# mojing1999/jmcodec

Measured on AMD Instinct MI355X. Metric: decoded frames/sec @1080p H.264 + bit-exact YUV, higher is better.
Workload: dtype u8

## Files before the change

### jmcodec_amd/csrc/deblock_device.h

```cpp
#pragma once
#include <hip/hip_runtime.h>
#include "jobs.h"
#include "kernels.h"
#include "kernel_common.h"
#include "chain_common.h"
#include "deblock_packed.h"

namespace jmamd {

struct DbRec {
    uint8_t y_bs[32];
    uint8_t y_ab[3][2];
    uint8_t y_pad[10];
    uint8_t c_bs[2][16];
    uint8_t c_ab[2][3][2];
    uint8_t c_pad[4];
};
static_assert(sizeof(DbRec) == 96, "DbRec must be 96 bytes");

__device__ __forceinline__ uint32_t perm(uint32_t hi, uint32_t lo, uint32_t sel) { return __builtin_amdgcn_perm(hi, lo, sel); }

struct Lds {
    uint8_t *base; int mb_h; int hdr;
    static constexpr int kRecStride = 80, kLT = 528, kLR = 272, kCT = 272, kCR = 144;
    __device__ uint8_t *rec(int group) const { return base + group * kRecStride; }
    __device__ uint8_t *luma_tile(int row, int par) const { return base + hdr + (size_t)row * kLT + par * 256; }
    __device__ uint8_t *luma_ring(int row, int slot) const { return base + hdr + (size_t)mb_h * kLT + (size_t)row * kLR + slot * 64; }
    __device__ uint8_t *chroma_tile(int row, int par) const { return base + hdr + (size_t)row * kCT + par * 128; }
    __device__ uint8_t *chroma_ring(int row, int slot) const { return base + hdr + (size_t)mb_h * kCT + (size_t)row * kCR + slot * 32; }
};

typedef __attribute__((address_space(1))) uint8_t gbyte;
struct DbCtx { gbyte *plane; int pitch, mb_w, mb_h; };
typedef uint32_t v4u __attribute__((ext_vector_type(4)));
typedef uint32_t v2u __attribute__((ext_vector_type(2)));
#define JM_GLOBAL __attribute__((address_space(1)))
template <typename T> __device__ __forceinline__ T gload(const gbyte *p);
template <> __device__ __forceinline__ uint4 gload<uint4>(const gbyte *p) { v4u v = *(const JM_GLOBAL v4u *)p; return make_uint4(v.x, v.y, v.z, v.w); }
template <> __device__ __forceinline__ uint32_t gload<uint32_t>(const gbyte *p) { return *(const JM_GLOBAL uint32_t *)p; }
__device__ __forceinline__ void gstore(gbyte *p, uint4 v) { v4u t = {v.x, v.y, v.z, v.w}; *(JM_GLOBAL v4u *)p = t; }
__device__ __forceinline__ void gstore(gbyte *p, uint2 v) { v2u t = {v.x, v.y}; *(JM_GLOBAL v2u *)p = t; }
__device__ __forceinline__ void gstore(gbyte *p, uint32_t v) { *(JM_GLOBAL uint32_t *)p = v; }
__device__ __forceinline__ void gstore_wt(gbyte *p, uint32_t v) { __hip_atomic_store((JM_GLOBAL uint32_t *)p, v, __ATOMIC_RELAXED, __HIP_MEMORY_SCOPE_AGENT); }
template <bool WT> __device__ __forceinline__ void fstore(gbyte *p, uint4 v) { if (WT) st_wt16((void *)p, v); else gstore(p, v); }
template <bool WT> __device__ __forceinline__ void fstore(gbyte *p, uint2 v) { if (WT) st_wt8((void *)p, v); else gstore(p, v); }
template <bool WT> __device__ __forceinline__ void fstore(gbyte *p, uint32_t v) { if (WT) gstore_wt(p, v); else gstore(p, v); }

template <bool WT, int PHASE = 0>
__device__ __forceinline__ void luma_mb(const DbCtx &pp, const Lds &lds, int x, int row, int lrow, int l, int group, uint4 own, uint32_t recdw) {
    uint8_t *tc = lds.luma_tile(lrow, x & 1), *tp = lds.luma_tile(lrow, (x - 1) & 1);
    uint8_t *ring_up = row > 0 ? lds.luma_ring(lrow - 1, x & 3) : nullptr;
    uint8_t *ring_up_l = row > 0 ? lds.luma_ring(lrow - 1, (x - 1) & 3) : nullptr;
    uint8_t *ring_dn = lds.luma_ring(lrow, x & 3), *ring_dn_l = lds.luma_ring(lrow, (x - 1) & 3);
    uint8_t *rec = lds.rec(group);
    if (PHASE != 2 && l < 12) ((uint32_t *)rec)[l] = recdw;
    int vb[4], hb[4], ab[6];
#pragma unroll
    for (int e = 0; e < 4; e++) { if (PHASE != 2) vb[e] = rec[e * 4 + (l >> 2)]; if (PHASE != 1) hb[e] = rec[16 + e * 4 + (l >> 2)]; }
#pragma unroll
    for (int i = 0; i < 6; i++) ab[i] = rec[32 + i];
    if (PHASE != 2) {
    uint32_t left = x > 0 ? *(const uint32_t *)(tp + l * 16 + 12) : 0;
    uint32_t left_after, row_after[4];
    {
        const uint32_t w[5] = {left, own.x, own.y, own.z, own.w};
        s2 A = as_s2(perm(w[1], w[0], 0x0c040c03)), B = as_s2(perm(w[1], w[0], 0x0c050c02)), C = as_s2(perm(w[1], w[0], 0x0c060c01)),
            D = as_s2(perm(w[1], w[0], 0x0c070c00));
#pragma unroll
        for (int e = 0; e < 4; e++) {
            if (e) {
                const s2 pA = A, pB = B, pC = C, pD = D;
                A = as_s2(perm(w[e + 1], as_u(pD), 0x0c040c02)); B = as_s2(perm(w[e + 1], as_u(pC), 0x0c050c02));
                C = as_s2(perm(w[e + 1], as_u(pB), 0x0c060c02)); D = as_s2(perm(w[e + 1], as_u(pA), 0x0c070c02));
            }
            const int c = e ? 1 : 0;
            flt_luma(A, B, C, D, vb[e], ab[2 * c], ab[2 * c + 1]);
            const uint32_t o = perm(as_u(C), as_u(D), 0x0c0c0400) | perm(as_u(A), as_u(B), 0x04000c0c);
            if (e == 0) left_after = o; else row_after[e - 1] = o;
        }
        row_after[3] = perm(as_u(B), as_u(A), 0x0c0c0602) | perm(as_u(D), as_u(C), 0x06020c0c);
    }
    if (x > 0) *(uint32_t *)(tp + l * 16 + 12) = left_after;
    *(uint4 *)(tc + l * 16) = make_uint4(row_after[0], row_after[1], row_after[2], row_after[3]);
    if (x > 0 && l >= 12) *(uint32_t *)(ring_dn_l + (l - 12) * 16 + 12) = left_after;
    }
    if (PHASE == 1) return;
    {
        uint32_t c[20];
        c[0] = c[1] = c[2] = c[3] = 0;
        if (ring_up) { c[0] = ring_up[l]; c[1] = ring_up[16 + l]; c[2] = ring_up[32 + l]; c[3] = ring_up[48 + l]; }
#pragma unroll
        for (int j = 0; j < 16; j++) c[4 + j] = tc[j * 16 + l];
        s2 A = as_s2(c[3] | (c[4] << 16)), B = as_s2(c[2] | (c[5] << 16)), C = as_s2(c[1] | (c[6] << 16)), D = as_s2(c[0] | (c[7] << 16));
#pragma unroll
        for (int e = 0; e < 4; e++) {
            if (e) {
                const s2 pA = A, pB = B, pC = C, pD = D;
                A = as_s2(perm(c[4 * e + 4], as_u(pD), 0x0c040c02)); B = as_s2(perm(c[4 * e + 5], as_u(pC), 0x0c040c02));
                C = as_s2(perm(c[4 * e + 6], as_u(pB), 0x0c040c02)); D = as_s2(perm(c[4 * e + 7], as_u(pA), 0x0c040c02));
            }
            const int k = e ? 1 : 2;
            flt_luma(A, B, C, D, hb[e], ab[2 * k], ab[2 * k + 1]);
            if (e == 0) { if (ring_up) { ring_up[1 * 16 + l] = (uint8_t)as_u(C); ring_up[2 * 16 + l] = (uint8_t)as_u(B);
                ring_up[3 * 16 + l] = (uint8_t)as_u(A); } }
            else { const int r = 4 * e - 4; tc[r * 16 + l] = (uint8_t)as_u(D); tc[(r + 1) * 16 + l] = (uint8_t)as_u(C);
                tc[(r + 2) * 16 + l] = (uint8_t)as_u(B); tc[(r + 3) * 16 + l] = (uint8_t)as_u(A); }
        }
        const uint8_t r12 = (uint8_t)(as_u(A) >> 16), r13 = (uint8_t)(as_u(B) >> 16), r14 = (uint8_t)(as_u(C) >> 16), r15 = (uint8_t)(as_u(D) >> 16);
        tc[12 * 16 + l] = r12; tc[13 * 16 + l] = r13; tc[14 * 16 + l] = r14; tc[15 * 16 + l] = r15;
        ring_dn[0 * 16 + l] = r12; ring_dn[1 * 16 + l] = r13; ring_dn[2 * 16 + l] = r14; ring_dn[3 * 16 + l] = r15;
    }
    gbyte *dst = pp.plane;
    int x0 = x * 16, y0 = row * 16, pitch = pp.pitch;
    bool right = x == pp.mb_w - 1, bottom = row == pp.mb_h - 1;
    {
        int R = l - 4;
        const uint8_t *src, *srcl;
        if (R < 0) { src = ring_up ? ring_up + (R + 4) * 16 : nullptr; srcl = ring_up_l ? ring_up_l + (R + 4) * 16 + 12 : nullptr; }
        else { src = tc + R * 16; srcl = tp + R * 16 + 12; }
        if (src) {
            gbyte *d = dst + (size_t)(y0 + R) * pitch + x0;
            uint4 v = *(const uint4 *)src;
            if (x > 0) { uint32_t lf = *(const uint32_t *)srcl; fstore<WT>(d - 4, make_uint4(lf, v.x, v.y, v.z)); }
            else { fstore<WT>(d, make_uint2(v.x, v.y)); fstore<WT>(d + 8, v.z); }
            if (right) fstore<WT>(d + 12, v.w);
        }
    }
    if (bottom && l < 4) {
        int R = 12 + l;
        gbyte *d = dst + (size_t)(y0 + R) * pitch + x0;
        uint4 v = *(const uint4 *)(tc + R * 16);
        if (x > 0) { uint32_t lf = *(const uint32_t *)(tp + R * 16 + 12); fstore<WT>(d - 4, make_uint4(lf, v.x, v.y, v.z)); }
        else { fstore<WT>(d, make_uint2(v.x, v.y)); fstore<WT>(d + 8, v.z); }
        if (right) fstore<WT>(d + 12, v.w);
    }
}

template <bool WT, int PHASE = 0>
__device__ __forceinline__ void chroma_mb(const DbCtx &pp, const Lds &lds, int x, int row, int lrow, int l, int group, uint4 own, uint32_t recdw) {
    uint8_t *tc = lds.chroma_tile(lrow, x & 1), *tp = lds.chroma_tile(lrow, (x - 1) & 1);
    uint8_t *ring_up = row > 0 ? lds.chroma_ring(lrow - 1, x & 3) : nullptr;
    uint8_t *ring_up_l = row > 0 ? lds.chroma_ring(lrow - 1, (x - 1) & 3) : nullptr;
    uint8_t *ring_dn = lds.chroma_ring(lrow, x & 3), *ring_dn_l = lds.chroma_ring(lrow, (x - 1) & 3);
    uint8_t *rec = lds.rec(group);
    if (PHASE != 2 && l < 12) ((uint32_t *)rec)[l] = recdw;
    if (PHASE != 2) {
        const int plane = l >> 3, r = l & 7;
        const uint32_t left = x > 0 ? *(const uint32_t *)(tp + r * 16 + 12) : 0;
        if (plane == 0) *(uint4 *)(tc + r * 16) = own;
        const int s0 = plane * 8, s1 = s0 + 16;
        const int vb[2] = { rec[plane * 16 + (r >> 1)], rec[plane * 16 + 4 + (r >> 1)] };
        const int ab[4] = { rec[32 + plane * 6], rec[32 + plane * 6 + 1], rec[32 + plane * 6 + 2], rec[32 + plane * 6 + 3] };
        {
            int p0 = (int)(left >> s1) & 255, q0 = (int)(own.x >> s0) & 255;
            flt_chroma((int)(left >> s0) & 255, p0, q0, (int)(own.x >> s1) & 255, vb[0], ab[0], ab[1]);
            if (vb[0] & 7) { tp[r * 16 + 14 + plane] = (uint8_t)p0; tc[r * 16 + plane] = (uint8_t)q0; }
        }
        {
            int p0 = (int)(own.y >> s1) & 255, q0 = (int)(own.z >> s0) & 255;
            flt_chroma((int)(own.y >> s0) & 255, p0, q0, (int)(own.z >> s1) & 255, vb[1], ab[2], ab[3]);
            if (vb[1] & 7) { tc[r * 16 + 6 + plane] = (uint8_t)p0; tc[r * 16 + 8 + plane] = (uint8_t)q0; }
        }
    }
    if (PHASE != 2 && x > 0 && l < 2) *(uint32_t *)(ring_dn_l + l * 16 + 12) = *(const uint32_t *)(tp + (6 + l) * 16 + 12);
    if (PHASE == 1) return;
    {
        int plane = l & 1;
        int hb[2] = { rec[plane * 16 + 8 + (l >> 2)], rec[plane * 16 + 12 + (l >> 2)] };
        int ab[4] = { rec[32 + plane * 6 + 4], rec[32 + plane * 6 + 5], rec[32 + plane * 6 + 2], rec[32 + plane * 6 + 3] };
        int c[10];
        c[0] = ring_up ? ring_up[l] : 0; c[1] = ring_up ? ring_up[16 + l] : 0;
#pragma unroll
        for (int j = 0; j < 8; j++) c[2 + j] = tc[j * 16 + l];
#pragma unroll
        for (int e = 0; e < 4; e += 2) {
            const int k = e ? 1 : 0;
            const int o = 2 * e;
            flt_chroma(c[o], c[o + 1], c[o + 2], c[o + 3], hb[e >> 1], ab[2 * k], ab[2 * k + 1]);
        }
        if (ring_up) ring_up[16 + l] = (uint8_t)c[1];
        tc[l] = (uint8_t)c[2]; tc[3 * 16 + l] = (uint8_t)c[5]; tc[4 * 16 + l] = (uint8_t)c[6];
        ring_dn[l] = (uint8_t)c[8]; ring_dn[16 + l] = (uint8_t)c[9];
    }
    gbyte *dst = pp.plane;
    int x0 = x * 16, y0 = row * 8, pitch = pp.pitch;
    bool right = x == pp.mb_w - 1, bottom = row == pp.mb_h - 1;
    if (l < 8) {
        int R = l - 2;
        const uint8_t *src, *srcl;
        if (R < 0) { src = ring_up ? ring_up + (R + 2) * 16 : nullptr; srcl = ring_up_l ? ring_up_l + (R + 2) * 16 + 12 : nullptr; }
        else { src = tc + R * 16; srcl = tp + R * 16 + 12; }
        if (src) {
            gbyte *d = dst + (size_t)(y0 + R) * pitch + x0;
            uint4 v = *(const uint4 *)src;
            if (x > 0) { uint32_t lf = *(const uint32_t *)srcl; fstore<WT>(d - 4, make_uint4(lf, v.x, v.y, v.z)); }
            else { fstore<WT>(d, make_uint2(v.x, v.y)); fstore<WT>(d + 8, v.z); }
            if (right) fstore<WT>(d + 12, v.w);
        }
    } else if (bottom && l < 10) {
        int R = 6 + (l - 8);
        gbyte *d = dst + (size_t)(y0 + R) * pitch + x0;
        uint4 v = *(const uint4 *)(tc + R * 16);
        if (x > 0) { uint32_t lf = *(const uint32_t *)(tp + R * 16 + 12); fstore<WT>(d - 4, make_uint4(lf, v.x, v.y, v.z)); }
        else { fstore<WT>(d, make_uint2(v.x, v.y)); fstore<WT>(d + 8, v.z); }
        if (right) fstore<WT>(d + 12, v.w);
    }
}

constexpr int kBandRows = 16;
constexpr int kDeblockSmemMain = kBandRows * Lds::kRecStride + (kBandRows + 1) * (Lds::kLT + Lds::kLR);
constexpr int kStageBytes = 1024 + 256 + 256, kDeblockMaxDepth = 4;
constexpr int kDeblockSmemBytes = kDeblockSmemMain + (kBandRows / 4) * kDeblockMaxDepth * kStageBytes;

__device__ __forceinline__ uint32_t lds_addr_of(const void *p) { return (uint32_t)(uintptr_t)(__attribute__((address_space(3))) const uint8_t *)p; }
template <bool COHERENT> __device__ __forceinline__ void glds16(const gbyte *g, uint32_t lds_byte_addr) {
    unsigned keep;
    if (COHERENT)
        asm volatile("s_mov_b32 %0, m0\n\ts_mov_b32 m0, %2\n\ts_nop 0\n\tglobal_load_lds_dwordx4 %1, off sc1\n\ts_mov_b32 m0, %0"
                     : "=&s"(keep) : "v"(g), "s"(lds_byte_addr) : "memory");
    else asm volatile("s_mov_b32 %0, m0\n\ts_mov_b32 m0, %2\n\ts_nop 0\n\tglobal_load_lds_dwordx4 %1, off\n\ts_mov_b32 m0, %0" : "=&s"(keep) : "v"(g),
        "s"(lds_byte_addr) : "memory");
}
template <bool COHERENT> __device__ __forceinline__ void glds4(const gbyte *g, uint32_t lds_byte_addr) {
    unsigned keep;
    if (COHERENT)
        asm volatile("s_mov_b32 %0, m0\n\ts_mov_b32 m0, %2\n\ts_nop 0\n\tglobal_load_lds_dword %1, off sc1\n\ts_mov_b32 m0, %0"
                     : "=&s"(keep) : "v"(g), "s"(lds_byte_addr) : "memory");
    else asm volatile("s_mov_b32 %0, m0\n\ts_mov_b32 m0, %2\n\ts_nop 0\n\tglobal_load_lds_dword %1, off\n\ts_mov_b32 m0, %0" : "=&s"(keep) : "v"(g),
        "s"(lds_byte_addr) : "memory");
}
template <int DEPTH, bool CHAIN, bool AFTER_INTRA = false>
__device__ __forceinline__ void deblock_band_body(const PicParams &pp, int band, bool is_chroma, int *prog_pic, int pub, uint8_t *smem, int *cpic,
    int *err_word) {
    const int mb_w = pp.mb_w, mb_h = pp.mb_h, pitch = pp.pitch;
    const int row0 = band * kBandRows;
    if (row0 >= mb_h) return;
    const int rows = min(kBandRows, mb_h - row0);
    int *prog = prog_pic + (is_chroma ? kDeblockMaxBands : 0);
    const gbyte *recs = (const gbyte *)pp.dbrec;
    Lds lds{smem, kBandRows + 1, kBandRows * Lds::kRecStride};
    const int group = threadIdx.x >> 4, l = threadIdx.x & 15;
    const int lrow = group + 1;
    const bool active = group < rows;
    const int row = row0 + (active ? group : 0);
    gbyte *plane = (gbyte *)(cur_plane(pp) + (is_chroma ? pp.chroma_offset : 0));
    const DbCtx cx{plane, pitch, mb_w, mb_h};
    const int rows_per_mb = is_chroma ? 8 : 16, ring_rows = is_chroma ? 2 : 4;
    const int my_row = is_chroma ? (l & 7) : l;
    const int rec_dw = (is_chroma ? 12 : 0) + (l < 12 ? l : 0);
    const bool takes_ring = band > 0 && group == 0;
    const bool gives_ring = active && group == rows - 1 && row < mb_h - 1;
    const int s_begin = kRowLag * row0, s_end = mb_w - 1 + kRowLag * (row0 + rows - 1) + (kRowLag == 1 ? 1 : 0);
    int known = 0;
    int *abort_word = CHAIN ? cpic - (size_t)pp.chain_idx * kChainStride + (size_t)kChainMaxPics * kChainStride : nullptr;
    auto wait_above = [&](int need) {
        if (band == 0 || threadIdx.x >= 64) return;
        if (known >= need) return;
        int spins = 0; WaitClock t0;
        while ((known = __hip_atomic_load(&prog[band - 1], __ATOMIC_RELAXED, __HIP_MEMORY_SCOPE_AGENT)) < need && ++spins < kSpinLimit &&
               !(CHAIN && (wait_expired(spins, t0, abort_word) || ((spins & 255) == 0 && ld_coh(abort_word))))) __builtin_amdgcn_s_sleep(8);
        if (CHAIN && l == 0) note_gaps(t0, err_word ? err_word - pp.chain_idx + kChainMaxPics : nullptr);
        if (known < need) {
            if (l == 0) { report_wait_timeout(err_word, CHAIN_ERR_RING_TIMEOUT);
                if (CHAIN) {
                    if (!ld_coh(abort_word)) { record_first_giveup(abort_word, CHAIN_ERR_RING_TIMEOUT, pp.chain_idx, band << 16 | (is_chroma ? 1 : 0), need,
                        known, 0);
                        record_giveup_evidence(abort_word, &prog[band - 1], spins, t0); }
                    st_coh(abort_word, 1);
                } }
            known = 0x7fffffff;
        }
        asm volatile("" ::: "memory");
    };
    int recon_known = (pp.stages & PS_RECON) ? 0x7fffffff : 0;
    const uint32_t *bits_row = CHAIN ? (const uint32_t *)(cpic + kChainBits) + (size_t)row * kChainRowWords : nullptr;
    constexpr bool after_intra = CHAIN && AFTER_INTRA;
    int ifin_known0 = 0, ifin_known1 = 0;
    const int *ifin0 = after_intra ? cpic + kChainIntraFin + (is_chroma ? 32 : 0) + (row >> 4) : nullptr;
    const int *ifin1 = after_intra ? cpic + kChainIntraFin + (is_chroma ? 32 : 0) + (min(row + 1, mb_h - 1) >> 4) : nullptr;
    auto wait_recon = [&](int x) {
        if (!CHAIN) return;
        const bool want = active && x >= 0 && x < mb_w;
        bool ok;
        const int tag = pp.chain_idx << 16 | (row & 0xffff);
        if (after_intra) { const int need = x + 2 * row + 4; ok = wait_counter(ifin0, ifin_known0, want, need, abort_word, tag) &&
            wait_counter(ifin1, ifin_known1, want, need, abort_word, tag); }
        else ok = wait_row_bit(bits_row, recon_known, want, x, abort_word, tag, err_word ? err_word - pp.chain_idx + kChainMaxPics : nullptr);
        if (!ok && (threadIdx.x & 63) == 0) { report_wait_timeout(err_word, after_intra ? CHAIN_ERR_IFIN_TIMEOUT : CHAIN_ERR_BITS_TIMEOUT);
            st_coh(abort_word, 1); }
    };
    const int ring_lanes = ring_rows * 4;
    const int ring_lane = l < ring_lanes ? l : 0;
    const gbyte *pix_base = plane + (size_t)(row * rows_per_mb + my_row) * pitch;
    const gbyte *rec_base = recs + (size_t)row * mb_w * sizeof(DbRec) + rec_dw * 4;
    const gbyte *ring_base = plane + (size_t)(takes_ring ? row * rows_per_mb - ring_rows + (ring_lane >> 2) : 0) * pitch + (ring_lane & 3) * 4;
    const int wave = __builtin_amdgcn_readfirstlane((int)(threadIdx.x >> 6)), wl = (int)(threadIdx.x & 63);
    uint8_t *stage = smem + kDeblockSmemMain + wave * (kDeblockMaxDepth * kStageBytes);
    const uint32_t stage_lds = lds_addr_of(stage);
    auto fetch = [&](int d, int s) {
        int xn = min(max(s - kRowLag * row, 0), mb_w - 1);
        if (CHAIN) wait_recon(s - kRowLag * row);
        const uint32_t slot = stage_lds + (uint32_t)d * kStageBytes;
        glds16<CHAIN>(pix_base + xn * 16, slot);
        glds4<false>(rec_base + (size_t)xn * sizeof(DbRec), slot + 1024);
        glds4<true>(band > 0 ? ring_base + xn * 16 : rec_base, slot + 1280);
    };
    auto give = [&](const uint8_t *ring, int xm, int lane0) {
        int k = l - lane0;
        if (k < 0 || k >= ring_lanes) return;
        uint32_t v = *(const uint32_t *)(ring + (k >> 2) * 16 + (k & 3) * 4);
        __hip_atomic_store((JM_GLOBAL uint32_t *)(plane + (size_t)((row + 1) * rows_per_mb - ring_rows + (k >> 2)) * pitch + xm * 16) + (k & 3), v,
            __ATOMIC_RELAXED, __HIP_MEMORY_SCOPE_AGENT);
    };
    auto step = [&](int s, uint4 own, uint32_t rdw, uint32_t ring) {
        if (kRowLag == 1) {
            const int xv = s - row, xh = xv - 1;
            if (active && xh >= 0 && xh < mb_w) {
                if (is_chroma) { chroma_mb<CHAIN, 2>(cx, lds, xh, row, lrow, l, group, own, rdw);
                    if (gives_ring && xh == mb_w - 1) give(lds.chroma_ring(lrow, xh & 3), xh, 8); }
                else { luma_mb<CHAIN, 2>(cx, lds, xh, row, lrow, l, group, own, rdw);
                    if (gives_ring && xh == mb_w - 1) give(lds.luma_ring(lrow, xh & 3), xh, 0); }
            }
            if (active && xv >= 0 && xv < mb_w) {
                if (is_chroma) {
                    if (takes_ring && l < ring_lanes) *(uint32_t *)(lds.chroma_ring(0, xv & 3) + (l >> 2) * 16 + (l & 3) * 4) = ring;
                    chroma_mb<CHAIN, 1>(cx, lds, xv, row, lrow, l, group, own, rdw);
                    if (gives_ring && xv > 0) give(lds.chroma_ring(lrow, (xv - 1) & 3), xv - 1, 0);
                } else {
                    if (takes_ring) *(uint32_t *)(lds.luma_ring(0, xv & 3) + (l >> 2) * 16 + (l & 3) * 4) = ring;
                    luma_mb<CHAIN, 1>(cx, lds, xv, row, lrow, l, group, own, rdw);
                    if (gives_ring && xv > 0) give(lds.luma_ring(lrow, (xv - 1) & 3), xv - 1, 0);
                }
            }
        } else {
            const int x = s - kRowLag * row;
            if (active && x >= 0 && x < mb_w) {
                if (is_chroma) {
                    if (takes_ring && l < ring_lanes) *(uint32_t *)(lds.chroma_ring(0, x & 3) + (l >> 2) * 16 + (l & 3) * 4) = ring;
                    chroma_mb<CHAIN, 0>(cx, lds, x, row, lrow, l, group, own, rdw);
                    if (gives_ring) {
                        if (x > 0) give(lds.chroma_ring(lrow, (x - 1) & 3), x - 1, 0);
                        if (x == mb_w - 1) give(lds.chroma_ring(lrow, x & 3), x, 8);
                    }
                } else {
                    if (takes_ring) *(uint32_t *)(lds.luma_ring(0, x & 3) + (l >> 2) * 16 + (l & 3) * 4) = ring;
                    luma_mb<CHAIN, 0>(cx, lds, x, row, lrow, l, group, own, rdw);
                    if (gives_ring) {
                        if (x > 0) give(lds.luma_ring(lrow, (x - 1) & 3), x - 1, 0);
                        if (x == mb_w - 1) give(lds.luma_ring(lrow, x & 3), x, 0);
                    }
                }
            }
        }
        constexpr int kPubLag = 3;
        if (gives_ring && pub > 0 && s - kPubLag >= s_begin && ((s - kPubLag + 1 - s_begin) % pub == 0)) {
            asm volatile("s_waitcnt vmcnt(%0)" :: "n"(3 * kPubLag) : "memory");
            if (l == 0) __hip_atomic_store(&prog[band], s - kPubLag + 1, __ATOMIC_RELAXED, __HIP_MEMORY_SCOPE_AGENT);
        }
        if (gives_ring && pub > 0 && s == s_end) {
            asm volatile("s_waitcnt vmcnt(0)" ::: "memory");
            if (l == 0) __hip_atomic_store(&prog[band], 0x7fffffff, __ATOMIC_RELAXED, __HIP_MEMORY_SCOPE_AGENT);
        }
        if (CHAIN) {
            asm volatile("s_waitcnt vmcnt(6) lgkmcnt(0)\n\ts_barrier" ::: "memory");
            if (threadIdx.x == 0 && s - 1 > s_begin) __hip_atomic_store(cpic + kChainFin + (is_chroma ? 32 : 0) + band, s - 1, __ATOMIC_RELAXED,
                __HIP_MEMORY_SCOPE_AGENT);
        } else
            asm volatile("s_waitcnt lgkmcnt(0)\n\ts_barrier" ::: "memory");
    };
    static_assert(DEPTH >= 2 && DEPTH <= kDeblockMaxDepth, "prefetch depth");
    constexpr int kAbove = 2 - kRowLag;
    wait_above(s_begin + DEPTH + kAbove);
#pragma unroll
    for (int d = 0; d < DEPTH; d++) fetch(d, s_begin + d);
    for (int s = s_begin; s <= s_end; s += DEPTH) {
#pragma unroll
        for (int j = 0; j < DEPTH; j++) {
            if (s + j > s_end) break;
            asm volatile("s_waitcnt vmcnt(%0)" :: "n"(3 * (DEPTH - 1)) : "memory");
            const uint8_t *sl = stage + j * kStageBytes;
            const uint4 own = *(const uint4 *)(sl + wl * 16);
            const uint32_t rdw = *(const uint32_t *)(sl + 1024 + wl * 4), ring = *(const uint32_t *)(sl + 1280 + wl * 4);
            asm volatile("s_waitcnt lgkmcnt(0)" ::: "memory");
            wait_above(s + j + DEPTH + kAbove);
            fetch(j, s + j + DEPTH);
            step(s + j, own, rdw, ring);
        }
    }
    if (CHAIN) {
        asm volatile("s_waitcnt vmcnt(0)\n\ts_barrier" ::: "memory");
        if (threadIdx.x == 0) __hip_atomic_store(cpic + kChainFin + (is_chroma ? 32 : 0) + band, 0x7fffffff, __ATOMIC_RELAXED, __HIP_MEMORY_SCOPE_AGENT);
    }
}

}
```

### jmcodec_amd/csrc/deblock_lds.hip

```cpp
#include <hip/hip_runtime.h>
#include <cstdlib>
#include <algorithm>
#include "jobs.h"
#include "kernels.h"
#include "kernel_common.h"
#include "deblock_device.h"

namespace jmamd {

__global__ __launch_bounds__(256) void k_deblock_prep(const PicParams *pics) {
    const PicParams &pp = pics[blockIdx.y];
    if (!(pp.stages & (PS_DEBLOCK_LDS | PS_CHAIN))) return;
    DbRec *out = (DbRec *)pp.dbrec;
    const int per_xcd = ((int)gridDim.x + 7) >> 3;
    const int blk = ((int)blockIdx.x & 7) * per_xcd + ((int)blockIdx.x >> 3);
    __shared__ __align__(16) uint8_t stage[8][96];
    int sub = threadIdx.x >> 5, t = threadIdx.x & 31;
    int mb = blk * 8 + sub;
    int n_mbs = pp.mb_w * pp.mb_h;
    if (mb >= n_mbs) return;
    int mbx = mb % pp.mb_w, mby = mb / pp.mb_w;
    const MbW q = load_mbw(&pp.mbs[mb]);
    const SliceRec sl = pp.slices[mbw_slice(q)];
    bool has_left = mbx > 0, has_top = mby > 0;
    MbW pl = q, pt = q;
    if (has_left) { pl = load_mbw(&pp.mbs[mb - 1]); if (sl.disable == 2 && mbw_slice(pl) != mbw_slice(q)) has_left = false; }
    if (has_top) { pt = load_mbw(&pp.mbs[mb - pp.mb_w]); if (sl.disable == 2 && mbw_slice(pt) != mbw_slice(q)) has_top = false; }
    int dir = t >> 4, e = (t >> 2) & 3, k = t & 3;
    int rq = dir == 0 ? k * 4 + e : e * 4 + k;
    int bs;
    if (sl.disable == 1) bs = 0;
    else if (e == 0) {
        bool have = dir == 0 ? has_left : has_top;
        const MbW pn = select_mbw(dir == 0, pl, pt);
        bs = have ? boundary_strength(pp, pn, dir == 0 ? k * 4 + 3 : 12 + k, q, rq, true, dir == 1) : 0;
    } else bs = boundary_strength(pp, q, dir == 0 ? rq - 1 : rq - 4, q, rq, false, dir == 1);
    if ((e & 1) && (mbw_modes(q) & MBM_T8X8)) bs = 0;
    int cls = e ? 1 : (dir ? 2 : 0);
    int qp_p = cls == 0 ? mbw_qp(pl) : (cls == 2 ? mbw_qp(pt) : mbw_qp(q)), qp_q = mbw_qp(q);
    DbRec *o = (DbRec *)stage[sub];
    {
        int qpav = (qp_p + qp_q + 1) >> 1;
        int ia = clip3(0, 51, qpav + sl.alpha_off), ib = clip3(0, 51, qpav + sl.beta_off);
        int tc0 = (bs >= 1 && bs <= 3) ? kTc0[ia][bs - 1] : 0;
        o->y_bs[t] = (uint8_t)(bs | (tc0 << 3));
        if (k == 0 && (e == 0 || (e == 1 && dir == 0))) { o->y_ab[cls][0] = kAlpha[ia]; o->y_ab[cls][1] = kBeta[ib]; }
    }
    if (!(e & 1)) {
#pragma unroll
        for (int plane = 0; plane < 2; plane++) {
            int off = plane ? pp.cr_qp_off : pp.cb_qp_off;
            int qpav = (chroma_qp(qp_p, off) + chroma_qp(qp_q, off) + 1) >> 1;
            int ia = clip3(0, 51, qpav + sl.alpha_off), ib = clip3(0, 51, qpav + sl.beta_off);
            int tc0 = (bs >= 1 && bs <= 3) ? kTc0[ia][bs - 1] : 0;
            o->c_bs[plane][dir * 8 + (e >> 1) * 4 + k] = (uint8_t)(bs | (tc0 << 3));
            if (k == 0 && (e == 0 || (e == 2 && dir == 0))) { o->c_ab[plane][cls][0] = kAlpha[ia]; o->c_ab[plane][cls][1] = kBeta[ib]; }
        }
    }
    if (t < 6) ((uint4 *)&out[mb])[t] = ((const uint4 *)stage[sub])[t];
}

template <int DEPTH>
__global__ __launch_bounds__(kBandRows * 16) void k_deblock_band(const PicParams *pics, int *ctl, int pub, int *err) {
    __shared__ __align__(16) uint8_t smem[kDeblockSmemBytes];
    const PicParams &pp = pics[blockIdx.y];
    if (!(pp.stages & PS_DEBLOCK_LDS)) return;
    deblock_band_body<DEPTH, false>(pp, blockIdx.x >> 1, blockIdx.x & 1, ctl + (size_t)blockIdx.y * kChainStride + kChainRing, pub, smem, nullptr,
        err + blockIdx.y);
}

bool deblock_lds_supported(int mb_w, int mb_h) { return mb_w > 0 && mb_h <= kBandRows * kDeblockMaxBands; }

constexpr int kDeblockDepth = 2, kDeblockPub = 2;
int deblock_depth() { return kDeblockDepth; }
int deblock_row_lag() { return kRowLag; }
int deblock_pub() { return kDeblockPub; }

void launch_deblock_prep(const PicParams *d_pics, int n, int max_mbs, hipStream_t st) {
    hipLaunchKernelGGL(k_deblock_prep, dim3(((max_mbs + 7) / 8 + 7) & ~7, n), dim3(256), 0, st, d_pics);
}
void launch_deblock_lds(const PicParams *d_pics, int n, int max_mb_h, int *ctl, int *err, bool debug_stall, hipStream_t st) {
    const int depth = deblock_depth(), pub = debug_stall ? -1 : deblock_pub();
    const int bands = (max_mb_h + kBandRows - 1) / kBandRows;
    dim3 grid(2 * bands, n), block(kBandRows * 16);
    if (depth <= 2) hipLaunchKernelGGL((k_deblock_band<2>), grid, block, 0, st, d_pics, ctl, pub, err);
    else if (depth == 3) hipLaunchKernelGGL((k_deblock_band<3>), grid, block, 0, st, d_pics, ctl, pub, err);
    else hipLaunchKernelGGL((k_deblock_band<4>), grid, block, 0, st, d_pics, ctl, pub, err);
}

}
```

### jmcodec_amd/csrc/deblock_packed.h

```cpp
#pragma once
#include <stdint.h>
#if defined(__HIPCC__)
#include <hip/hip_runtime.h>
#include "kernel_common.h"
#define JM_DB_HD __host__ __device__ __forceinline__
#else
#define JM_DB_HD static inline
#endif

namespace jmamd {

#if !defined(__HIPCC__)
JM_DB_HD int clip3(int lo, int hi, int v) { return v < lo ? lo : (v > hi ? hi : v); }
JM_DB_HD int clip1(int v) { return v < 0 ? 0 : (v > 255 ? 255 : v); }
JM_DB_HD int iabs(int v) { return v < 0 ? -v : v; }
#endif

#if defined(__HIPCC__)
typedef short s2 __attribute__((ext_vector_type(2)));
JM_DB_HD s2 pmin(s2 a, s2 b) { return __builtin_elementwise_min(a, b); }
JM_DB_HD s2 pmax(s2 a, s2 b) { return __builtin_elementwise_max(a, b); }
JM_DB_HD s2 as_s2(uint32_t v) { return __builtin_bit_cast(s2, v); }
JM_DB_HD uint32_t as_u(s2 v) { return __builtin_bit_cast(uint32_t, v); }
#else
struct s2 { int16_t x, y; };
JM_DB_HD s2 mk_s2(int x, int y) { return s2{(int16_t)(uint16_t)(x & 0xffff), (int16_t)(uint16_t)(y & 0xffff)}; }
JM_DB_HD s2 operator+(s2 a, s2 b) { return mk_s2(a.x + b.x, a.y + b.y); }
JM_DB_HD s2 operator-(s2 a, s2 b) { return mk_s2(a.x - b.x, a.y - b.y); }
JM_DB_HD s2 operator-(s2 a) { return mk_s2(-a.x, -a.y); }
JM_DB_HD s2 operator<<(s2 a, int n) { return mk_s2((int)((uint32_t)(uint16_t)a.x << n), (int)((uint32_t)(uint16_t)a.y << n)); }
JM_DB_HD s2 operator>>(s2 a, int n) { return mk_s2(a.x >> n, a.y >> n); }
JM_DB_HD s2 pmin(s2 a, s2 b) { return s2{a.x < b.x ? a.x : b.x, a.y < b.y ? a.y : b.y}; }
JM_DB_HD s2 pmax(s2 a, s2 b) { return s2{a.x > b.x ? a.x : b.x, a.y > b.y ? a.y : b.y}; }
JM_DB_HD s2 as_s2(uint32_t v) { return mk_s2((int)(v & 0xffffu), (int)(v >> 16)); }
JM_DB_HD uint32_t as_u(s2 v) { return (uint32_t)(uint16_t)v.x | ((uint32_t)(uint16_t)v.y << 16); }
#endif
#if defined(__HIP_DEVICE_COMPILE__)
JM_DB_HD uint32_t sad_u8(uint32_t a, uint32_t b, uint32_t c) { return __builtin_amdgcn_sad_u8(a, b, c); }
JM_DB_HD uint32_t alignbit(uint32_t hi, uint32_t lo, uint32_t sh) { return __builtin_amdgcn_alignbit(hi, lo, sh); }
JM_DB_HD bool any_lane(bool c) { return __builtin_amdgcn_ballot_w64(c) != 0; }
#else
JM_DB_HD uint32_t sad_u8(uint32_t a, uint32_t b, uint32_t c) {
    for (int k = 0; k < 4; k++) { const int x = (int)((a >> (8 * k)) & 255), y = (int)((b >> (8 * k)) & 255); c += (uint32_t)(x < y ? y - x : x - y); }
    return c;
}
JM_DB_HD uint32_t alignbit(uint32_t hi, uint32_t lo, uint32_t sh) { return (uint32_t)((((uint64_t)hi << 32) | lo) >> (sh & 31)); }
JM_DB_HD bool any_lane(bool c) { return c; }
#endif

JM_DB_HD int adiff(int a, int b) { return (int)sad_u8((unsigned)a, (unsigned)b, 0u); }
JM_DB_HD int sel(bool c, int a, int b) { return c ? a : b; }
JM_DB_HD s2 splat(int v) { return as_s2((uint32_t)v | ((uint32_t)v << 16)); }
JM_DB_HD s2 swp(s2 v) { const uint32_t u = as_u(v); return as_s2(alignbit(u, u, 16)); }
JM_DB_HD s2 pabs(s2 v) { return pmax(v, -v); }
JM_DB_HD s2 blend(uint32_t m, s2 a, s2 b) { return as_s2((as_u(a) & m) | (as_u(b) & ~m)); }
JM_DB_HD void flt_luma(s2 &A, s2 &B, s2 &C, const s2 D, int bsw, int alpha, int beta) {
    const int bS = bsw & 7, tc0 = bsw >> 3;
    const s2 As = swp(A), Bs = swp(B);
    const s2 beta2 = splat(beta);
    const s2 d10 = pabs(B - A), dpq = pabs(As - A);
    const s2 m10 = (d10 - beta2) >> 15, mpq = (dpq - splat(alpha)) >> 15;
    const uint32_t on = as_u(m10) & as_u(swp(m10)) & as_u(mpq) & (bS ? 0xffffffffu : 0u);
    if (!any_lane(on != 0)) return;
    const s2 m20 = (pabs(C - A) - beta2) >> 15;
    const int tc = tc0 + (int)(as_u(m20) & 1u) + (int)(as_u(m20) >> 31);
    const s2 t = ((As - A) << 2) + (B - Bs) + splat(4);
    const int dl = clip3(-tc, tc, (int)(short)(as_u(t) & 0xffffu) >> 3);
    const s2 dd = as_s2(((uint32_t)dl & 0xffffu) | ((uint32_t)(-dl) << 16));
    const s2 nA = pmin(pmax(A + dd, splat(0)), splat(255));
    const s2 avg = as_s2((as_u(A + As + splat(1)) >> 1) & 0x7fff7fffu);
    const s2 tcs = splat(tc0);
    const s2 tt = pmin(pmax((C + avg - (B << 1)) >> 1, -tcs), tcs);
    const s2 nB = B + as_s2(as_u(tt) & as_u(m20));
    const uint32_t nrm = on & (bS < 4 ? 0xffffffffu : 0u);
    s2 rA = blend(nrm, nA, A), rB = blend(nrm, nB, B), rC = C;
    const uint32_t st = on & (bS >= 4 ? 0xffffffffu : 0u);
    if (any_lane(st != 0)) {
        const s2 msg = (dpq - splat((alpha >> 2) + 2)) >> 15;
        const uint32_t sm = st & as_u(m20) & as_u(msg);
        const s2 S0 = (C + ((B + A + As) << 1) + Bs + splat(4)) >> 3;
        const s2 S1 = (C + B + A + As + splat(2)) >> 2;
        const s2 S2 = ((D << 1) + C + (C << 1) + B + A + As + splat(4)) >> 3;
        const s2 W0 = ((B << 1) + A + Bs + splat(2)) >> 2;
        rA = blend(sm, S0, blend(st, W0, rA)); rB = blend(sm, S1, rB); rC = blend(sm, S2, rC);
    }
    A = rA; B = rB; C = rC;
}
JM_DB_HD void flt_chroma(int p1, int &p0, int &q0, int q1, int bsw, int alpha, int beta) {
    const int bS = bsw & 7, tc = (bsw >> 3) + 1;
    const bool on = ((int)(bS != 0) & (int)(adiff(p0, q0) < alpha) & (int)(adiff(p1, p0) < beta) & (int)(adiff(q1, q0) < beta)) != 0;
    const int delta = clip3(-tc, tc, (((q0 - p0) << 2) + (p1 - q1) + 4) >> 3);
    const int n_p0 = clip1(p0 + delta), n_q0 = clip1(q0 - delta), w_p0 = (2 * p1 + p0 + q1 + 2) >> 2, w_q0 = (2 * q1 + q0 + p1 + 2) >> 2;
    p0 = sel(on, sel(bS < 4, n_p0, w_p0), p0); q0 = sel(on, sel(bS < 4, n_q0, w_q0), q0);
}

JM_DB_HD void filter_luma(int *s, int bS, int alpha, int beta, const uint8_t *tc0_row) {
    int p3 = s[0], p2 = s[1], p1 = s[2], p0 = s[3], q0 = s[4], q1 = s[5], q2 = s[6], q3 = s[7];
    if (!(iabs(p0 - q0) < alpha && iabs(p1 - p0) < beta && iabs(q1 - q0) < beta)) return;
    int ap = iabs(p2 - p0) < beta, aq = iabs(q2 - q0) < beta;
    if (bS < 4) {
        int tc0 = tc0_row[bS - 1], tc = tc0 + ap + aq;
        int delta = clip3(-tc, tc, (((q0 - p0) << 2) + (p1 - q1) + 4) >> 3);
        s[3] = clip1(p0 + delta); s[4] = clip1(q0 - delta);
        if (ap) s[2] = p1 + clip3(-tc0, tc0, (p2 + ((p0 + q0 + 1) >> 1) - (p1 << 1)) >> 1);
        if (aq) s[5] = q1 + clip3(-tc0, tc0, (q2 + ((p0 + q0 + 1) >> 1) - (q1 << 1)) >> 1);
    } else {
        bool strong = iabs(p0 - q0) < ((alpha >> 2) + 2);
        if (ap && strong) { s[3] = (p2 + 2 * p1 + 2 * p0 + 2 * q0 + q1 + 4) >> 3; s[2] = (p2 + p1 + p0 + q0 + 2) >> 2;
            s[1] = (2 * p3 + 3 * p2 + p1 + p0 + q0 + 4) >> 3; }
        else s[3] = (2 * p1 + p0 + q1 + 2) >> 2;
        if (aq && strong) { s[4] = (p1 + 2 * p0 + 2 * q0 + 2 * q1 + q2 + 4) >> 3; s[5] = (p0 + q0 + q1 + q2 + 2) >> 2;
            s[6] = (2 * q3 + 3 * q2 + q1 + q0 + p0 + 4) >> 3; }
        else s[4] = (2 * q1 + q0 + p1 + 2) >> 2;
    }
}
JM_DB_HD void filter_chroma(int *s, int bS, int alpha, int beta, const uint8_t *tc0_row) {
    int p1 = s[0], p0 = s[1], q0 = s[2], q1 = s[3];
    if (!(iabs(p0 - q0) < alpha && iabs(p1 - p0) < beta && iabs(q1 - q0) < beta)) return;
    if (bS < 4) {
        int tc = tc0_row[bS - 1] + 1;
        int delta = clip3(-tc, tc, (((q0 - p0) << 2) + (p1 - q1) + 4) >> 3);
        s[1] = clip1(p0 + delta); s[2] = clip1(q0 - delta);
    } else { s[1] = (2 * p1 + p0 + q1 + 2) >> 2; s[2] = (2 * q1 + q0 + p1 + 2) >> 2; }
}

}
```

### jmcodec_amd/csrc/engine.cpp

```cpp
#include "engine.h"
#include <sys/prctl.h>
#include "chain_order.h"
#include "decoder.h"
#include "kernels.h"
#include "hevc_kernels.h"
#include "numa.h"
#include <hip/hip_runtime_api.h>
#include <pthread.h>
#include <algorithm>
#include <chrono>
#include <cstdio>
#include <cstring>
#include <cstdlib>

namespace jmamd {

static long g_lane_trace = getenv("JM_AMD_DEC_LANE_TRACE") ? atol(getenv("JM_AMD_DEC_LANE_TRACE")) : 0;
static double trace_ms() { static const auto t0 = std::chrono::steady_clock::now();
    return std::chrono::duration<double, std::milli>(std::chrono::steady_clock::now() - t0).count(); }
#define LANE_TRACE(...) do { if (g_lane_trace > 0) { g_lane_trace--; fprintf(stderr, "lane-trace %9.3f " , trace_ms()); fprintf(stderr, __VA_ARGS__); } } while (0)

static std::mutex g_engines_m;
static Engine *g_engines[64] = {nullptr};

Engine *Engine::get(int device) {
    std::lock_guard<std::mutex> lk(g_engines_m);
    if (device < 0 || device >= 64) return nullptr;
    if (!g_engines[device]) {
        Engine *e = new Engine(device);
        if (!e->ok_) return nullptr;
        g_engines[device] = e;
    }
    return g_engines[device];
}

void mem_trace(const char *tag) {
    static const bool on = getenv("JM_AMD_DEC_MEMTRACE") != nullptr;
    if (!on) return;
    long pages = 0, res = 0;
    if (FILE *f = fopen("/proc/self/statm", "r")) { if (fscanf(f, "%ld %ld", &pages, &res) != 2) res = 0; fclose(f); }
    fprintf(stderr, "jm_amd_dec: memtrace %-44s %8.1f MB resident\n", tag, res * 4096.0 / 1e6);
}

Engine::Engine(int device) : device_(device) {
    (void)trace_ms();
    mem_trace("engine: start");
    if (const char *e = getenv("JM_AMD_DEC_CHAIN_DEPTH")) { chain_depth_ = std::max(1, std::min(atoi(e), 16)); chain_depth_few_ = chain_depth_.load(); }
    if (const char *e = getenv("JM_AMD_DEC_CHAIN_STREAMS")) chain_max_streams_ = std::max(0, atoi(e));
    if (const char *e = getenv("JM_AMD_DEC_CHAIN_LAG")) chain_lag_steps_ = std::max(kMinChainLag, std::min(atoi(e), 1024));
    if (const char *e = getenv("JM_AMD_DEC_CHAIN_LINGER")) chain_linger_streams_ = std::max(0, atoi(e));
    if (const char *e = getenv("JM_AMD_DEC_CROSS_LANE")) cross_lane_ = atoi(e) != 0;
    if (const char *e = getenv("JM_AMD_DEC_FILL_LINGER_US")) fill_linger_ns_ = std::max(0, atoi(e)) * 1000ll;
    if (const char *e = getenv("JM_AMD_DEC_EARLY_INTRA")) early_intra_ = atoi(e) != 0;
    if (hipSetDevice(device_) != hipSuccess) return;
    if (const char *e = getenv("JM_AMD_DEC_COPY_STREAMS")) n_copy_ = std::max(1, std::min(atoi(e), 4));
    int prio_lo = 0, prio_hi = 0, copy_prio = 0;
    hipDeviceGetStreamPriorityRange(&prio_lo, &prio_hi);
    { const char *e = getenv("JM_AMD_DEC_COPY_PRIORITY"); const int want = e ? atoi(e) : 1;
      copy_prio = want > 0 ? prio_hi : (want < 0 ? prio_lo : 0); }
    for (int k = 0; k < n_copy_; k++) if (hipStreamCreateWithPriority(&copy_streams_[k], hipStreamNonBlocking, copy_prio) != hipSuccess) {
        (void)hipGetLastError();
        if (hipStreamCreateWithFlags(&copy_streams_[k], hipStreamNonBlocking) != hipSuccess) return; }
    mem_trace("engine: copy stream");
    for (auto &ln : lanes_) {
        hipStream_t s, p, q;
        if (hipStreamCreateWithFlags(&s, hipStreamNonBlocking) != hipSuccess || hipStreamCreateWithFlags(&p, hipStreamNonBlocking) != hipSuccess ||
            hipStreamCreateWithFlags(&q, hipStreamNonBlocking) != hipSuccess) return;
        ln.stream = s; ln.pack_stream = p; ln.pre_stream = q;
        mem_trace("engine: lane streams");
        for (auto &b : ln.ring) {
            if (hipHostMalloc((void **)&b.h_pics, sizeof(PicParams) * kMaxBatch, hipHostMallocDefault) != hipSuccess) return;
            if (hipMalloc((void **)&b.d_pics, sizeof(PicParams) * kMaxBatch) != hipSuccess) return;
            if (hipHostMalloc((void **)&b.h_hpics, sizeof(HevcPicParams) * kMaxBatch, hipHostMallocDefault) != hipSuccess) return;
            if (hipMalloc((void **)&b.d_hpics, sizeof(HevcPicParams) * kMaxBatch) != hipSuccess) return;
            if (hipMalloc((void **)&b.d_progress, sizeof(int) * kMaxBatch * kHevcProgressStride) != hipSuccess) return;
            if (hipMalloc((void **)&b.d_ctl, sizeof(int) * ((size_t)kMaxBatch * chain_ctl_ints() + chain_tail_ints())) != hipSuccess) return;
            if (hipHostMalloc((void **)&b.h_err, sizeof(int) * (kMaxBatch + 4), hipHostMallocMapped) != hipSuccess) return;
            if (hipHostGetDevicePointer((void **)&b.d_err, b.h_err, 0) != hipSuccess) return;
            memset(b.h_err, 0, sizeof(int) * (kMaxBatch + 4));
            if (hipHostMalloc((void **)&b.h_groups, sizeof(uint32_t) * kMaxChainGroups, hipHostMallocDefault) != hipSuccess) return;
            if (hipMalloc((void **)&b.d_groups, sizeof(uint32_t) * kMaxChainGroups) != hipSuccess) return;
            bool tables_ok = true;
            b.out.each([&](auto &t) { const size_t bytes = sizeof(*t.host) * 2 * kOutSideCap;
                tables_ok = tables_ok && hipHostMalloc((void **)&t.host, bytes, hipHostMallocDefault) == hipSuccess &&
                            hipMalloc((void **)&t.dev, bytes) == hipSuccess; });
            if (!tables_ok) return;
            if (hipEventCreateWithFlags(&b.done, hipEventDisableTiming) != hipSuccess) return;
            if (hipEventCreateWithFlags(&b.kdone, hipEventDisableTiming) != hipSuccess) return;
            if (hipEventCreateWithFlags(&b.packed, hipEventDisableTiming) != hipSuccess) return;
            if (hipEventCreateWithFlags(&b.pre_done, hipEventDisableTiming) != hipSuccess) return;
            for (auto &e : b.pev) if (hipEventCreate(&e) != hipSuccess) return;
        }
    }
    mem_trace("engine: lane buffers");
    { const int r = chain_resident_workgroups(false), ri = chain_resident_workgroups(true);
      if (r > 0) chain_bands_max_ = std::min(kMaxChainBands, r / 2);
      if (ri > 0) chain_bands_max_intra_ = std::min(kMaxChainBandsIntra, ri / 2);
      if (getenv("JM_AMD_DEC_VERBOSE")) fprintf(stderr,
          "jm_amd_dec: device %d holds %d / %d chain workgroups (plain / with the intra role): band budget %d / %d\n", device_, r, ri, chain_bands_max_,
          chain_bands_max_intra_); }
    mem_trace("engine: occupancy queries");
    ok_ = true;
    numa_node_ = numa_node_of_device(device_, true);
    kfd_gpu_id_ = getenv("JM_AMD_DEC_IGNORE_SHARED_GPU") ? 0 : kfd_gpu_id_of_device(device_);
    th_ = std::thread([this] { pthread_setname_np(pthread_self(), "jm-engine"); numa_bind_this_thread(numa_node_); run(); });
    th_.detach();
}

unsigned long long Engine::upload(uint8_t *dev, const uint8_t *host, size_t n, ihipEvent_t *ev, bool spread) {
    std::lock_guard<std::mutex> lk(um_);
    hipSetDevice(device_);
    unsigned long long seq = ++upload_seq_;
    if (!spread) while (seq % (unsigned)n_copy_) seq = ++upload_seq_;
    hipStream_t cs = copy_streams_[seq % (unsigned)n_copy_];
    hipMemcpyAsync(dev, host, n, hipMemcpyHostToDevice, cs);
    hipEventRecord(ev, cs);
    return seq;
}

void Engine::submit(EnginePic &&p) {
    {
        std::lock_guard<std::mutex> lk(m_);
        if (p.codec == 0) {
            const long long now = std::chrono::duration_cast<std::chrono::nanoseconds>(std::chrono::steady_clock::now().time_since_epoch()).count();
            auto it = std::find_if(recent_.begin(), recent_.end(), [&](const Recent &r) { return r.dec == p.dec; });
            if (it == recent_.end()) { recent_.push_back(Recent{p.dec, now, 0}); it = recent_.end() - 1; }
            it->t = now;
            if (p.has_picture) it->mbs = p.mb_w * p.mb_h;
        }
        p.seq = p.dec->engine_state().next_seq++;
        if (p.dec->engine_state().n_pending++ == 0) decoders_pending_++;
        pending_.push_back(std::move(p));
        pending_gen_++;
    }
    cv_.notify_one();
}

bool Engine::set_knob(const std::string &key, long long v) {
    if (key.rfind("chain_", 0) == 0) { chain_block_until_ns_ = 0; shared_checked_ns_ = 0; }
    if (key == "chain_depth") { if (v <= 0) { chain_depth_ = 8; chain_depth_few_ = 16; }
        else { chain_depth_ = (int)std::min(v, 16ll); chain_depth_few_ = chain_depth_.load(); } }
    else if (key == "chain_lag") chain_lag_steps_ = (int)std::max((long long)kMinChainLag, std::min(v, 1024ll));
    else if (key == "chain_streams") chain_max_streams_ = (int)std::max(0ll, v);
    else if (key == "debug_stall") debug_stall_ = (int)v;
    else if (key == "debug_no_bi") debug_no_bi_ = (int)v;
    else if (key == "early_intra_ahead") early_intra_ahead_ = (int)std::max(1ll, std::min(v, 64ll));
    else return false;
    return true;
}

EngineStats Engine::stats() { std::lock_guard<std::mutex> lk(sm_); return st_; }

bool Engine::others_done(Decoder *d, int lane_idx, unsigned long long seq) {
    for (int li = 0; li < kLanes; li++) {
        if (li == lane_idx) continue;
        Lane &o = lanes_[li];
        for (int k = 0; k < o.inflight; k++) {
            Batch &ob = o.ring[(o.tail + k) % kBatchRing];
            bool mine = false;
            for (auto &p : ob.pics) if (p.dec == d && p.seq < seq) { mine = true; break; }
            if (mine && hipEventQuery(ob.packed) != hipSuccess) { (void)hipGetLastError(); return false; }
        }
    }
    return true;
}

void Engine::inflight_masks(Decoder *d, uint32_t &touched) {
    touched = 0;
    for (auto &o : lanes_) for (int k = 0; k < o.inflight; k++) for (auto &p : o.ring[(o.tail + k) % kBatchRing].pics) if (p.dec == d) {
        touched |= p.ref_mask | p.out_mask;
        if (p.has_picture) touched |= 1u << (p.codec == 0 ? p.pp.cur : p.hp.cur);
    }
}

bool Engine::form(Lane &ln, int lane_idx, Batch &b) {
    b.pics.clear(); b.any_chain = false; b.chain_with_intra = false; b.max_depth = 1;
    bool chaining = false;
    int depth_now = chain_depth_;
    {
        const long long now = std::chrono::duration_cast<std::chrono::nanoseconds>(std::chrono::steady_clock::now().time_since_epoch()).count();
        recent_.erase(std::remove_if(recent_.begin(), recent_.end(), [&](const Recent &r) { return now - r.t > 50ll * 1000 * 1000; }), recent_.end());
        const int n_active = (int)recent_.size();
        double load = 0;
        for (const Recent &r : recent_) load += std::max(1.0, r.mbs / 8160.0);
        chaining = chain_depth_ > 1 && n_active > 0 && load <= (double)chain_max_streams_ && now >= chain_block_until_ns_ &&
            !gpu_shared_.load(std::memory_order_relaxed);
        depth_now = n_active <= chain_linger_streams_ ? std::max(chain_depth_.load(), chain_depth_few_.load()) : chain_depth_.load();
        if (lane_idx == kOrdinaryLane && chaining && n_active <= chain_linger_streams_ && ln.inflight > 0) {
            int n = 0;
            for (const EnginePic &p : pending_) if (p.codec == 0 && p.has_picture && p.lane(true) == lane_idx) n++;
            if (n < depth_now * n_active) return false;
        }
    }
    if (lane_idx == kOrdinaryLane && !chaining && fill_linger_ns_ > 0 && (int)recent_.size() > decoders_pending_) {
        const long long now = std::chrono::duration_cast<std::chrono::nanoseconds>(std::chrono::steady_clock::now().time_since_epoch()).count();
        if (!ln.wait_since_ns) ln.wait_since_ns = now;
        if (now - ln.wait_since_ns < fill_linger_ns_) {
            bool urgent = false; size_t n_seen = 0; const size_t n_dec = (size_t)decoders_pending_;
            scan_tag_form_++;
            for (auto it = pending_.begin(); it != pending_.end() && n_seen < n_dec && !urgent; ++it) {
                EngineDecoderState &es = it->dec->engine_state();
                if (es.form_tag == scan_tag_form_) continue;
                es.form_tag = scan_tag_form_; n_seen++;
                if (it->lane(false) != lane_idx || es.inflight > es.lane_inflight[lane_idx]) continue;
                urgent = it->dec->frames_done_unfetched() < 1;
            }
            if (!urgent) { lingered_ = true; return false; }
        }
    }
    if (lane_idx == kOrdinaryLane) ln.wait_since_ns = 0;
    if (lane_idx == kIntraLane && !chaining && !deep_queues_ && fill_linger_ns_ > 0) {
        const long long now = std::chrono::duration_cast<std::chrono::nanoseconds>(std::chrono::steady_clock::now().time_since_epoch()).count();
        if (!ln.wait_since_ns || now - ln.wait_since_ns < fill_linger_ns_) {
            bool urgent = false; int n_elig = 0; size_t n_seen = 0; const size_t n_dec = (size_t)decoders_pending_;
            scan_tag_form_++;
            for (auto it = pending_.begin(); it != pending_.end() && n_seen < n_dec && !urgent && n_elig < 4; ++it) {
                EngineDecoderState &es = it->dec->engine_state();
                if (es.form_tag == scan_tag_form_) continue;
                es.form_tag = scan_tag_form_; n_seen++;
                if (it->codec != 0 || it->lane(false) != lane_idx) continue;
                if (es.inflight > es.lane_inflight[lane_idx] && !(cross_lane_ && others_done(it->dec, lane_idx, it->seq))) continue;
                n_elig++;
                urgent = it->dec->frames_done_unfetched() < 1;
            }
            if (n_elig == 0) return false;
            if (!ln.wait_since_ns) ln.wait_since_ns = now;
            if (n_elig < 4 && !urgent && now - ln.wait_since_ns < fill_linger_ns_) { lingered_ = true; return false; }
        }
        ln.wait_since_ns = 0;
    }
    std::vector<Decoder *> seen, members;
    const bool relaxed = cross_lane_ && !chaining;
    const long long now_ns = std::chrono::duration_cast<std::chrono::nanoseconds>(std::chrono::steady_clock::now().time_since_epoch()).count();
    size_t n_pre = 0, n_post = 0;
    auto account = [&](EnginePic &p, EngineDecoderState &es) {
        if (p.has_picture) es.batch_written |= 1u << (p.codec == 0 ? p.pp.cur : p.hp.cur);
        es.batch_read |= p.ref_mask | p.out_mask;
        n_pre += p.out[kBefore].frames(); n_post += p.out[kAfter].frames();
    };
    const size_t n_dec_pending = (size_t)decoders_pending_;
    auto took = [&](EngineDecoderState &es) { if (--es.n_pending == 0) decoders_pending_--; };
    for (auto it = pending_.begin(); it != pending_.end() && (int)b.pics.size() < kMaxBatch && seen.size() < n_dec_pending;) {
        Decoder *d = it->dec;
        if (std::find(seen.begin(), seen.end(), d) != seen.end()) { ++it; continue; }
        seen.push_back(d);
        EngineDecoderState &es = d->engine_state();
        int why = 0;
        if (it->lane(chaining) != lane_idx) why = 1;
        else if (es.inflight > es.lane_inflight[lane_idx] && !(relaxed && others_done(d, lane_idx, it->seq))) why = 2;
        else if (n_pre + it->out[kBefore].frames() > (size_t)kOutSideCap || n_post + it->out[kAfter].frames() > (size_t)kOutSideCap) why = 3;
        if (why) {
            if (lane_idx == kOrdinaryLane && it->codec == 0) { std::lock_guard<std::mutex> lk(sm_);
                (why == 1 ? st_.rej_other_lane : why == 2 ? st_.rej_cross_lane : st_.rej_tables)++;
                if (!es.blocked_since) { es.blocked_since = now_ns;
                    if (g_lane_trace > 0) {
                        LANE_TRACE("left-out dec %p seq %llu why %d inflight %d (lane0 %d lane1 %d)\n", (void *)d, it->seq, why, es.inflight, es.lane_inflight[0],
                            es.lane_inflight[1]);
                        for (int li = 0; li < kLanes; li++) for (int k = 0; k < lanes_[li].inflight; k++) { Batch &ob = lanes_[li].ring[(lanes_[li].tail + k) % kBatchRing];
                            for (auto &p : ob.pics) if (p.dec == d) LANE_TRACE("    in flight: lane %d batch %llu seq %llu kdone %d packed %d done %d\n", li, ob.serial, p.seq,
                                (int)hipEventQuery(ob.kdone), (int)hipEventQuery(ob.packed), (int)hipEventQuery(ob.done)); }
                        (void)hipGetLastError();
                    } } }
            ++it; continue;
        }
        if (lane_idx == kOrdinaryLane && es.blocked_since) { std::lock_guard<std::mutex> lk(sm_); st_.blocked_ns += now_ns - es.blocked_since; st_.blocked_n++;
            LANE_TRACE("rejoined dec %p seq %llu after %.3f ms\n", (void *)d, it->seq, (now_ns - es.blocked_since) * 1e-6);
            es.blocked_since = 0; }
        es.inflight++; es.lane_inflight[lane_idx]++;
        es.in_batch = 1; es.batch_written = es.batch_read = 0; es.batch_stop = false;
        account(*it, es);
        members.push_back(d);
        took(es);
        b.pics.push_back(std::move(*it));
        it = pending_.erase(it);
    }
    if (lane_idx == kIntraLane && early_intra_ && deep_queues_ && !chaining && early_scanned_gen_ != pending_gen_ && now_ns - early_scan_ns_ > 250 * 1000) {
        early_scan_ns_ = now_ns;
        const unsigned long long tag = ++early_scan_tag_;
        std::vector<std::deque<EnginePic>::iterator> cand;
        for (auto it = pending_.begin(); it != pending_.end(); ++it) {
            Decoder *d = it->dec;
            EngineDecoderState &es = d->engine_state();
            if (es.scan_tag != tag) { es.scan_tag = tag; es.scan_touched = 0; es.scan_ahead = 0;
                es.scan_closed = std::find(members.begin(), members.end(), d) != members.end(); }
            const uint32_t own = it->has_picture ? 1u << (it->codec == 0 ? it->pp.cur : it->hp.cur) : 0u;
            if (!es.scan_closed && it->codec == 0 && it->has_picture && it->lane(false) == kIntraLane && it->ref_mask == 0 && it->before_empty() &&
                !it->wait_prev_pack && !(it->out_mask & ~own)) {
                es.scan_closed = true;
                uint32_t infl; inflight_masks(d, infl);
                const bool landed = !it->uploaded || hipEventQuery(it->uploaded) == hipSuccess;
                if (!landed) (void)hipGetLastError();
                if (landed && es.scan_ahead >= early_intra_ahead_.load() && !(own & (es.scan_touched | infl))) cand.push_back(it);
            }
            es.scan_touched |= it->ref_mask | it->out_mask | own;
            es.scan_ahead++;
        }
        if (!cand.empty()) {
            std::vector<size_t> pos;
            for (auto &c : cand) pos.push_back((size_t)(c - pending_.begin()));
            for (size_t k = pos.size(); k-- > 0 && (int)b.pics.size() < kMaxBatch;) {
                auto it = pending_.begin() + (std::ptrdiff_t)pos[k];
                if (n_post + it->out[kAfter].frames() > (size_t)kOutSideCap) continue;
                EngineDecoderState &es = it->dec->engine_state();
                es.inflight++; es.lane_inflight[lane_idx]++;
                LANE_TRACE("early dec %p seq %llu\n", (void *)it->dec, it->seq);
                n_post += it->out[kAfter].frames();
                took(es);
                b.pics.push_back(std::move(*it));
                pending_.erase(it);
                { std::lock_guard<std::mutex> lk(sm_); st_.early_intra++; }
            }
        }
        early_scanned_gen_ = pending_gen_;
    }
    if (b.pics.empty()) return false;
    pending_gen_++;
    if (lane_idx == kOrdinaryLane) {
        { std::lock_guard<std::mutex> lk(sm_); st_.forms++; st_.form_decoders += (long long)seen.size(); st_.form_pending += (long long)(pending_.size() + b.pics.size()); }
        const size_t depth = (pending_.size() + b.pics.size()) / std::max<size_t>(1, seen.size());
        if (depth >= 16) deep_queues_ = true; else if (depth <= 8) deep_queues_ = false;
    }
    auto chain_cost = [&](const EnginePic &p, int &bands, int &groups) { bands = (p.chain_intra ? 4 : 2) * ((p.mb_h + 15) / 16);
        groups = p.mb_h * ((p.mb_w + 7) / 8) + 2 * ((p.mb_h + 15) / 16); };
    int tot_bands = 0, tot_groups = 0; bool any_intra = false;
    for (auto &p : b.pics) if (p.has_picture && (p.chain_ok || p.chain_intra)) { int nb, ng; chain_cost(p, nb, ng); tot_bands += nb; tot_groups += ng;
        any_intra |= p.chain_intra; }
    auto band_limit = [&](bool intra) { return intra ? chain_bands_max_intra_ : chain_bands_max_; };
    if (lane_idx == kOrdinaryLane && chaining && (int)members.size() <= chain_max_streams_ && tot_bands <= band_limit(any_intra) &&
        tot_groups <= kMaxChainGroups) {
        const int depth_cap = std::min(depth_now, std::max(1, kMaxBatch / (int)members.size()));
        for (int depth = 1; depth < depth_cap; depth++) {
            bool added = false;
            for (Decoder *d : members) {
                EngineDecoderState &es = d->engine_state();
                if (es.batch_stop || (int)b.pics.size() >= kMaxBatch) continue;
                auto it = std::find_if(pending_.begin(), pending_.end(), [&](const EnginePic &p) { return p.dec == d; });
                const bool ok = it != pending_.end() && it->lane(true) == lane_idx && it->has_picture && (it->chain_ok || it->chain_intra) &&
                                it->before_empty() && !it->wait_prev_pack &&
                                !((1u << it->pp.cur) & (es.batch_written | es.batch_read)) && n_post + it->out[kAfter].frames() <= (size_t)kOutSideCap;
                int nb = 0, ng = 0;
                if (ok) chain_cost(*it, nb, ng);
                if (!ok || tot_bands + nb > band_limit(any_intra || it->chain_intra) || tot_groups + ng > kMaxChainGroups) { es.batch_stop = true; continue; }
                tot_bands += nb; tot_groups += ng; any_intra |= it->chain_intra;
                es.inflight++; es.lane_inflight[lane_idx]++; es.in_batch++;
                account(*it, es);
                took(es);
                b.pics.push_back(std::move(*it));
                pending_.erase(it);
                b.any_chain = true; added = true;
            }
            if (!added) break;
            b.max_depth = depth + 1;
        }
    }
    if (lane_idx == kHevcLane || lane_idx == kHevcIntraLane) {
        for (Decoder *d : members) {
            EngineDecoderState &es = d->engine_state();
            while (es.in_batch < kHevcWorkSets && (int)b.pics.size() < kMaxBatch) {
                auto it = std::find_if(pending_.begin(), pending_.end(), [&](const EnginePic &p) { return p.dec == d; });
                if (it == pending_.end() || !it->has_picture || it->codec == 0 || it->lane(false) != lane_idx || !it->before_empty() ||
                    it->wait_prev_pack) break;
                if ((it->ref_mask & es.batch_written) || ((1u << it->hp.cur) & (es.batch_written | es.batch_read)) ||
                    n_post + it->out[kAfter].frames() > (size_t)kOutSideCap) break;
                es.inflight++; es.lane_inflight[lane_idx]++; es.in_batch++;
                es.batch_written |= 1u << it->hp.cur;
                account(*it, es);
                took(es);
                b.pics.push_back(std::move(*it));
                pending_.erase(it);
            }
        }
    }
    return true;
}

void Engine::launch(Lane &ln, Batch &b) {
    const int n = (int)b.pics.size(), li = (int)(&ln - lanes_);
    b.serial = ++ln.launched; b.last_ev = -1;
    b.launched_dry = false;
    if (profile_) {
        const Batch &pb = ln.ring[(ln.head + kBatchRing - 1) % kBatchRing];
        if (pb.serial + 1 == b.serial && pb.kdone) { const bool ended = hipEventQuery(pb.kdone) == hipSuccess; (void)hipGetLastError();
            b.launched_dry = ended;
            if (ended) { std::lock_guard<std::mutex> lk(sm_); st_.lane_dry[li]++; } }
    }
    LANE_TRACE("launch lane %d batch %llu pics %d\n", li, b.serial, n);
    int max_mbs = 0, max_mb_h = 0, max_mb_w = 0, stages = 0;
    bool wait_pack = false, any_hevc = false, any_jpeg = false; int max_jpeg_items = 0;
    for (auto &p : b.pics) any_jpeg |= p.codec == 2 && p.has_picture;
    if (any_jpeg && !b.h_jpics) {
        if (hipHostMalloc((void **)&b.h_jpics, sizeof(JpegPicParams) * kMaxBatch, hipHostMallocDefault) != hipSuccess ||
            hipMalloc((void **)&b.d_jpics, sizeof(JpegPicParams) * kMaxBatch) != hipSuccess) {
            (void)hipGetLastError();
            if (b.h_jpics) hipHostFree(b.h_jpics);
            b.h_jpics = nullptr; b.d_jpics = nullptr; any_jpeg = false;
            for (auto &p : b.pics) if (p.codec == 2 && p.has_picture) { p.has_picture = false; p.dec->on_engine_error("hipMalloc(MJPEG parameter table) failed"); }
        }
    }
    if (any_jpeg && profile_ && !b.jev[0]) for (auto &e : b.jev) if (hipEventCreate(&e) != hipSuccess) { (void)hipGetLastError(); e = nullptr; }
    b.any_hash = false;
    for (auto &p : b.pics) b.any_hash |= p.codec == 1 && p.has_picture && p.hp.hash_mode != 0;
    if (b.any_hash && !b.d_hash) {
        const size_t bytes = sizeof(uint32_t) * kMaxBatch * kHashStride;
        if (hipMalloc((void **)&b.d_hash, bytes) != hipSuccess || hipHostMalloc((void **)&b.h_hash, bytes, hipHostMallocDefault) != hipSuccess) {
            (void)hipGetLastError();
            if (b.d_hash) hipFree(b.d_hash);
            b.d_hash = nullptr; b.h_hash = nullptr; b.any_hash = false;
            for (auto &p : b.pics) p.hp.hash_mode = 0;
        }
    }
    if (b.any_hash && profile_ && !b.mev[0]) {
        bool any_md5 = false;
        for (auto &p : b.pics) any_md5 |= p.codec == 1 && p.has_picture && (p.hp.hash_mode & 2) != 0;
        if (any_md5) for (auto &e : b.mev) if (hipEventCreate(&e) != hipSuccess) { (void)hipGetLastError(); e = nullptr; }
    }
    HevcBatchDims hd;
    const EnginePic *last_upload[4] = {nullptr, nullptr, nullptr, nullptr};
    b.pmask = 0;
    for (int k = 0; k < kKernelClasses; k++) { b.alg[k] = 0; b.npics[k] = 0; }
    size_t d_need = 0;
    for (auto &p : b.pics) for (auto &o : p.out) d_need += OutTables::bytes_needed(o);
    if (d_need > b.deint_cap) {
        if (b.deint_scratch) hipFree(b.deint_scratch);
        b.deint_scratch = nullptr; b.deint_cap = std::max(d_need, 2 * b.deint_cap);
        if (hipMalloc((void **)&b.deint_scratch, b.deint_cap) != hipSuccess) { (void)hipGetLastError(); b.deint_scratch = nullptr; b.deint_cap = 0; }
    }
    b.out.reset(b.deint_scratch);
    for (int i = 0; i < n; i++) {
        EnginePic &p = b.pics[i];
        const bool hevc = p.codec != 0;
        if (hevc) { b.h_hpics[i] = p.hp; if (!p.has_picture) b.h_hpics[i].stages = 0; any_hevc = true; }
        if (any_jpeg) {
            if (p.codec == 2 && p.has_picture) { b.h_jpics[i] = p.jp; max_jpeg_items = std::max(max_jpeg_items, p.jp.n_items); b.alg[7] += p.jpeg_alg_bytes; b.npics[7]++; }
            else b.h_jpics[i].n_items = 0;
        }
        b.h_pics[i] = p.pp;
        if (!p.has_picture || hevc) b.h_pics[i].stages = 0;
        else if (b.any_chain && (p.chain_ok || p.chain_intra)) {
            PicParams &q = b.h_pics[i];
            q.stages = PS_CHAIN | (p.chain_intra ? PS_CHAIN_INTRA : 0); q.chain_idx = i; q.n_deps = 0;
            if (p.chain_intra) q.want_intra_resid = 1;
            for (int k = 0; k < kMaxSurfaces; k++) q.dep_pic[k] = -1;
            bool refs_in_batch = false;
            for (int j = 0; j < i; j++) {
                const EnginePic &e = b.pics[j];
                if (e.dec != p.dec || !e.has_picture || e.codec != 0) continue;
                if (p.ref_mask & (1u << e.pp.cur)) refs_in_batch = true;
                if (e.chain_ok || e.chain_intra) { q.dep_pic[e.pp.cur] = (int8_t)j; if (p.ref_mask & (1u << e.pp.cur)) q.n_deps++; }
            }
            if (!refs_in_batch) q.stages |= PS_RECON;
        }
        stages |= b.h_pics[i].stages;
        if (p.has_picture && !hevc) max_mb_w = std::max(max_mb_w, p.mb_w);
        if (p.has_picture && ((1u << (hevc ? p.hp.cur : p.pp.cur)) & p.dec->engine_state().displayed[li])) wait_pack = true;
        if (hevc && p.has_picture) {
            const HevcPicParams &h = p.hp;
            hd.max_pus = std::max(hd.max_pus, h.n_pus); hd.max_tbs = std::max(hd.max_tbs, h.n_tbs); hd.max_itbs = std::max(hd.max_itbs, h.n_itbs);
            hd.max_ctb_w = std::max(hd.max_ctb_w, h.ctb_w); hd.max_ctb_h = std::max(hd.max_ctb_h, h.ctb_h);
            hd.max_w = std::max(hd.max_w, h.w); hd.max_h = std::max(hd.max_h, h.h); hd.any_intra |= (h.stages & HPS_INTRA) != 0;
            hd.any_deblock |= (h.stages & HPS_DEBLOCK) != 0; hd.any_sao |= (h.stages & HPS_SAO) != 0;
            if (h.hash_mode & 1) { hd.any_hash = true; b.alg[8] += (long long)h.w * h.h * 3 / 2; b.npics[8]++; }
            if (h.hash_mode & 2) { hd.any_md5 = true; b.alg[9] += (long long)h.w * h.h * 3 / 2; b.npics[9]++; }
        }
        if (p.has_picture) {
            max_mbs = std::max(max_mbs, p.mb_w * p.mb_h); max_mb_h = std::max(max_mb_h, p.mb_h);
            if (p.uploaded) { const EnginePic *&lu = last_upload[p.upload_seq % (unsigned)n_copy_]; if (!lu || p.upload_seq > lu->upload_seq) lu = &p; }
        }
        if (p.wait_prev_pack) wait_pack = true;
        for (int side : {kBefore, kAfter}) if (!b.out.add(p.out[side], side, p.disp_w, p.disp_h, p.alg_bytes[3], p.alg_bytes[4]))
            p.dec->on_engine_error("hipMalloc(deinterlace scratch) failed");
        int st = b.h_pics[i].stages;
        if (hevc && p.has_picture) { const int hs = p.hp.stages; if (hs & (HPS_MC | HPS_RESID)) { b.alg[0] += p.alg_bytes[0]; b.npics[0]++; }
            if (hs & HPS_INTRA) { b.alg[1] += p.alg_bytes[1]; b.npics[1]++; } if (hs & (HPS_DEBLOCK | HPS_SAO)) { b.alg[2] += p.alg_bytes[2]; b.npics[2]++; } }
        if (st & PS_RECON) { b.alg[0] += p.alg_bytes[0]; b.npics[0]++; }
        if (st & (PS_INTRA_LDS | PS_INTRA_V1)) { b.alg[1] += p.alg_bytes[1]; b.npics[1]++; }
        if (st & (PS_DEBLOCK_LDS | PS_DEBLOCK_V1)) { b.alg[2] += p.alg_bytes[2]; b.npics[2]++; }
        if (st & PS_CHAIN) { b.alg[4] += ((st & PS_RECON) ? 0 : p.alg_bytes[0]) + ((st & PS_CHAIN_INTRA) ? p.alg_bytes[1] : 0) + p.alg_bytes[2]; b.npics[4]++; }
    }
    b.alg[3] = b.out.alg_pack; b.npics[3] = b.out.n_frames; b.alg[5] = b.out.alg_rgb; b.npics[5] = b.out.n_rgb;
    b.alg[10] = b.out.alg_rgb444; b.npics[10] = b.out.n_chroma[0] + b.out.n_chroma[1];
    b.alg[6] = b.out.alg_deint; b.npics[6] = b.out.n_deint;
    for (auto &p : b.pics) p.dec->engine_state().displayed[li] = 0;
    for (auto &p : b.pics) p.dec->engine_state().displayed[li] |= p.out_mask;
    b.max_mbs = max_mbs; b.max_mb_h = max_mb_h; b.redo = false;
    hipStream_t st = ln.stream, pst = ln.pack_stream;
    hipStream_t ps = any_hevc ? st : ln.pre_stream;
    if (!any_hevc && (stages & (PS_INTRA_LDS | PS_DEBLOCK_LDS | PS_CHAIN))) { hipMemsetAsync(b.d_ctl, 0, sizeof(int) * (size_t)n * chain_ctl_ints(), ps);
        hipMemsetAsync(b.d_ctl + (size_t)kMaxBatch * chain_ctl_ints(), 0, chain_tail_ints() * sizeof(int), ps);
        if (stages & PS_CHAIN) {
            const double launch_ms = 0.25 * b.max_depth * std::max(1.0, max_mbs / 8160.0) + 0.8;
            const unsigned ticks = (unsigned)(std::min(100.0, std::max(10.0, 10.0 * launch_ms)) * 100000.0);
            static const unsigned forced = getenv("JM_AMD_DEC_CHAIN_WAIT_MS") ? (unsigned)(atof(getenv("JM_AMD_DEC_CHAIN_WAIT_MS")) * 100000.0) : 0u;
            hipMemsetD32Async((hipDeviceptr_t)(b.d_ctl + (size_t)kMaxBatch * chain_ctl_ints() + chain_tail_wait_limit()), (int)(forced ? forced : ticks), 1, ps);
        } }
    if (any_hevc) hipMemcpyAsync(b.d_hpics, b.h_hpics, sizeof(HevcPicParams) * n, hipMemcpyHostToDevice, ps);
    else hipMemcpyAsync(b.d_pics, b.h_pics, sizeof(PicParams) * n, hipMemcpyHostToDevice, ps);
    if (any_jpeg) hipMemcpyAsync(b.d_jpics, b.h_jpics, sizeof(JpegPicParams) * n, hipMemcpyHostToDevice, ps);
    b.out.each([&](auto &t) { for (int side : {kBefore, kAfter}) if (t.n[side])
        hipMemcpyAsync(t.dev + side * kOutSideCap, t.h(side), sizeof(*t.host) * t.n[side], hipMemcpyHostToDevice, ps); });
    for (const EnginePic *lu : last_upload) if (lu) hipStreamWaitEvent(ps, lu->uploaded, 0);
    if (profile_ && !any_hevc) hipEventRecord(b.pev[8], ps);
    bool prep_early = false;
    if (!any_hevc) {
        if (stages & (PS_DEBLOCK_LDS | PS_CHAIN)) { launch_deblock_prep(b.d_pics, n, max_mbs, ps); prep_early = true; }
        if (profile_) hipEventRecord(b.pev[9], ps);
        hipEventRecord(b.pre_done, ps);
        hipStreamWaitEvent(st, b.pre_done, 0);
    }
    if (ln.pack_hist[1]) hipStreamWaitEvent(st, ln.pack_hist[1], 0);
    if ((wait_pack || b.out.any(kBefore)) && ln.pack_hist[0]) hipStreamWaitEvent(st, ln.pack_hist[0], 0);
    auto mark = [&](int i, hipStream_t s) { if (profile_) hipEventRecord(b.pev[i], s); };
    run_side(b, kBefore, st, true);
    if (any_hevc && (hd.max_pus || hd.max_tbs || hd.any_intra || hd.any_deblock || hd.any_sao)) {
        hipEvent_t ev[5] = {b.pev[1], b.pev[2], b.pev[3], b.pev[4], b.pev[18]};
        launch_hevc_picture_batch(b.d_hpics, n, hd, b.d_progress, st, profile_ ? ev : nullptr, b.d_hash);
        if (hd.max_pus || hd.max_tbs) b.pmask |= 2;
        if (hd.any_intra) b.pmask |= 4;
        if (hd.any_deblock || hd.any_sao) b.pmask |= 8;
        b.last_ev = 4;
        if (hd.any_md5 && b.d_hash) {
            const bool timed = profile_ && b.mev[0] && b.mev[1];
            if (timed) hipEventRecord(b.mev[0], st);
            launch_hevc_md5(b.d_hpics, n, b.d_hash, st);
            if (timed) { hipEventRecord(b.mev[1], st); b.pmask |= 4096; }
        }
        if (hd.any_hash || (hd.any_md5 && b.d_hash)) hipMemcpyAsync(b.h_hash, b.d_hash, sizeof(uint32_t) * (size_t)n * kHashStride, hipMemcpyDeviceToHost, st);
        if (hd.any_hash) { b.pmask |= 2048; b.last_ev = 18; }
    }
    if (any_jpeg && max_jpeg_items > 0) {
        const bool timed = profile_ && b.jev[0] && b.jev[1];
        if (timed) hipEventRecord(b.jev[0], st);
        launch_jpeg_recon(b.d_jpics, n, max_jpeg_items, st);
        if (timed) { hipEventRecord(b.jev[1], st); b.pmask |= 1024; }
    }
    b.any_bipred = b.any_field = false;
    for (auto &p : b.pics) { b.any_bipred |= p.has_picture && p.codec == 0 && p.bipred; b.any_field |= p.has_picture && p.codec == 0 && p.pp.field != 0; }
    if (stages & PS_RECON) { launch_recon_inter(b.d_pics, n, max_mbs, b.any_bipred && !debug_no_bi_, b.any_field, b.d_err, st); b.pmask |= 2; }
    if (!any_hevc) mark(2, st);
    if (stages & PS_INTRA_LDS) { launch_intra_lds(b.d_pics, n, max_mb_h, b.d_ctl, b.d_err, st); b.pmask |= 4; }
    if (stages & PS_INTRA_V1) { launch_recon_intra(b.d_pics, n, st); b.pmask |= 4; }
    if (!any_hevc) mark(3, st);
    if ((stages & (PS_DEBLOCK_LDS | PS_CHAIN)) && !prep_early) launch_deblock_prep(b.d_pics, n, max_mbs, st);
    if (stages & PS_DEBLOCK_LDS) { launch_deblock_lds(b.d_pics, n, max_mb_h, b.d_ctl, b.d_err, debug_stall_ == 1, st); b.pmask |= 8; }
    if (stages & PS_DEBLOCK_V1) { launch_deblock(b.d_pics, n, st); b.pmask |= 8; }
    if (!any_hevc) { mark(4, st); b.last_ev = 4; }
    if (stages & PS_CHAIN) {
        const int band_rows = chain_band_rows(), L = deblock_row_lag();
        constexpr int kBandLag = 8, kKeySlack = 2, kIntraExtra = 24;
        std::vector<int> base_of(n, 0), slope_of(n, L);
        size_t n_keys = 0;
        for (int i = 0; i < n; i++) {
            if (!(b.h_pics[i].stages & PS_CHAIN)) continue;
            slope_of[i] = (b.h_pics[i].stages & PS_CHAIN_INTRA) ? 2 : L;
            for (int j = i - 1; j >= 0; j--) if (b.pics[j].dec == b.pics[i].dec && (b.h_pics[j].stages & PS_CHAIN)) {
                base_of[i] = base_of[j] + chain_lag_steps_ + kKeySlack + slope_of[i] * b.pics[i].reach_rows + b.pics[i].reach_cols +
                             kBandLag * ((b.pics[i].reach_rows + 1) / band_rows);
                if (b.h_pics[j].stages & PS_CHAIN_INTRA) base_of[i] += b.h_pics[j].mb_h + kIntraExtra;
                break; }
            n_keys = std::max(n_keys,
                (size_t)(base_of[i] + slope_of[i] * b.h_pics[i].mb_h + b.h_pics[i].mb_w + kBandLag * (b.h_pics[i].mb_h / band_rows + 1) + 2));
        }
        if (group_buckets_.size() < n_keys) group_buckets_.resize(n_keys);
        for (size_t k = 0; k < n_keys; k++) group_buckets_[k].clear();
        for (int i = 0; i < n; i++) {
            if (!(b.h_pics[i].stages & PS_CHAIN) || (b.h_pics[i].stages & PS_RECON)) continue;
            const int mb_h = b.h_pics[i].mb_h, segs = (b.h_pics[i].mb_w + 7) / 8, base = base_of[i];
            for (int r = 0; r < mb_h; r++) {
                const int kr = base + slope_of[i] * r + kBandLag * (r / band_rows);
                for (int c = 0; c < segs; c++) group_buckets_[kr + 8 * c].push_back((uint32_t)i << 16 | (uint32_t)(r * 32 + c));
            }
        }
        int n_groups = 0;
        bool with_intra = false;
        for (int i = 0; i < n; i++) if (b.h_pics[i].stages & PS_CHAIN) for (int bnd = 0; bnd * band_rows < b.h_pics[i].mb_h; bnd++) {
            if (b.h_pics[i].stages & PS_CHAIN_INTRA) { b.h_groups[n_groups++] = (uint32_t)i << 16 | 0xC000u | (uint32_t)bnd; with_intra = true; }
            b.h_groups[n_groups++] = (uint32_t)i << 16 | 0x8000u | (uint32_t)bnd;
        }
        for (size_t k = 0; k < n_keys; k++) append_bucket_by_xcd(group_buckets_[k].data(), group_buckets_[k].size(), b.h_groups, n_groups, bucket_tmp_);
        hipMemcpyAsync(b.d_groups, b.h_groups, sizeof(uint32_t) * (size_t)n_groups, hipMemcpyHostToDevice, st);
        launch_chain(b.d_pics, b.d_groups, n_groups, with_intra, b.d_ctl, b.d_err, debug_stall_ != 0, st);
        b.chain_with_intra = with_intra;
        b.pmask |= 32; mark(7, st); b.last_ev = 7;
    }
    hipEventRecord(b.kdone, st);
    hipStreamWaitEvent(pst, b.kdone, 0);
    run_side(b, kAfter, pst, true);
    hipError_t le = hipGetLastError();
    if (le != hipSuccess) fprintf(stderr, "jm_amd_dec: kernel launch failed: %s\n", hipGetErrorString(le));
    hipEventRecord(b.done, pst);
    ln.pack_hist[1] = ln.pack_hist[0]; ln.pack_hist[0] = b.packed;
}

void Engine::run_side(Batch &b, int side, hipStream_t s, bool in_launch) {
    const OutTables &t = b.out;
    auto mark = [&](int i) { if (in_launch && profile_) hipEventRecord(b.pev[i], s); };
    mark(side ? 5 : 0);
    if (t.deint.n[side]) { mark(14 + 2 * side); (t.pairs[side] ? launch_deint2 : launch_deint)(t.deint.d(side), t.deint.n[side], t.d_items, s); mark(15 + 2 * side); b.pmask |= side ? 512 : 256; }
    if (t.plain.n[side]) launch_packout(t.plain.d(side), t.plain.n[side], t.max_w, t.max_h, s);
    if (t.scale.n[side]) launch_scale_pack(t.scale.d(side), t.scale.n[side], t.s_tiles, s);
    if (t.rgb.n[side]) { mark(10 + 2 * side); launch_rgb_pack(t.rgb.d(side), t.rgb.n[side], t.r_tiles[0], t.r_tiles[1], 0, s);
        if (t.n_chroma[side]) { mark(19 + 2 * side); launch_rgb_pack(t.rgb.d(side), t.rgb.n[side], 0, 0, t.r_tiles[2], s); mark(20 + 2 * side);
            b.pmask |= side ? 16384 : 8192; }
        mark(11 + 2 * side); b.pmask |= side ? 128 : 64; }
    if (t.any(side)) b.pmask |= side ? 16 : 1;
    if (in_launch && side) { mark(6); hipEventRecord(b.packed, s); }
    if (t.any(side)) for (auto &p : b.pics) for (OutSlot *o : p.out[side].slots) if (o->dev && o->host && !o->fetch)
        hipMemcpyAsync(o->host, o->dev, o->bytes, hipMemcpyDeviceToHost, s);
    if (in_launch && !side) mark(1);
}

void Engine::recover(Lane &ln, Batch &b, const std::vector<std::pair<Decoder *, uint32_t>> &later) {
    const int n = (int)b.pics.size();
    hipStream_t st = ln.stream;
    hipStreamSynchronize(ln.pack_stream); hipStreamSynchronize(st);
    auto is_tainted = [&](Decoder *d) { return std::find(ln.tainted.begin(), ln.tainted.end(), d) != ln.tainted.end(); };
    auto taint = [&](Decoder *d) { if (!is_tainted(d)) ln.tainted.push_back(d); };
    for (int i = 0; i < n; i++) {
        Decoder *d = b.pics[i].dec;
        bool first = true;
        for (int j = 0; j < i; j++) first &= b.pics[j].dec != d;
        if (!first) continue;
        uint32_t written = 0, ext_refs = 0, shown = 0, shown_before = 0, lw = 0;
        for (int j = i; j < n; j++) {
            const EnginePic &p = b.pics[j];
            if (p.dec != d) continue;
            ext_refs |= p.ref_mask & ~written;
            shown |= p.out_mask;
            if (!p.before_empty()) shown_before |= p.out_mask;
            if (p.has_picture && p.codec == 0) written |= 1u << p.pp.cur;
        }
        for (auto &e : later) if (e.first == d) lw |= e.second;
        if ((lw & (ext_refs | shown)) || (b.redo && (written & shown_before))) taint(d);
    }
    if (b.redo && b.out.any(kBefore)) { run_side(b, kBefore, st, false); hipStreamSynchronize(st); }
    std::vector<int> depth(n, 0); int max_depth = 0;
    for (int i = 0; i < n; i++) { for (int j = 0; j < i; j++) if (b.pics[j].dec == b.pics[i].dec && b.pics[j].has_picture) depth[i]++;
        max_depth = std::max(max_depth, depth[i]); }
    for (int d = 0; d <= max_depth; d++) {
        int stages = 0;
        for (int i = 0; i < n; i++) {
            const EnginePic &p = b.pics[i];
            b.h_pics[i] = p.pp;
            b.h_pics[i].stages = (p.has_picture && p.codec == 0 && depth[i] == d) ? p.classic_stages : 0;
            stages |= b.h_pics[i].stages;
            b.h_err[i] = 0;
        }
        if (!stages) continue;
        hipMemsetAsync(b.d_ctl, 0, sizeof(int) * (size_t)n * chain_ctl_ints(), st);
        hipMemcpyAsync(b.d_pics, b.h_pics, sizeof(PicParams) * n, hipMemcpyHostToDevice, st);
        if (stages & PS_RECON) launch_recon_inter(b.d_pics, n, b.max_mbs, b.any_bipred, b.any_field, b.d_err, st);
        if (stages & PS_INTRA_LDS) launch_intra_lds(b.d_pics, n, b.max_mb_h, b.d_ctl, b.d_err, st);
        if (stages & PS_INTRA_V1) launch_recon_intra(b.d_pics, n, st);
        if (stages & PS_DEBLOCK_LDS) { launch_deblock_prep(b.d_pics, n, b.max_mbs, st);
            launch_deblock_lds(b.d_pics, n, b.max_mb_h, b.d_ctl, b.d_err, false, st); }
        if (stages & PS_DEBLOCK_V1) launch_deblock(b.d_pics, n, st);
        hipStreamSynchronize(st);
    }
    if (b.out.any(kAfter)) { run_side(b, kAfter, st, false); hipStreamSynchronize(st); }
    for (int i = 0; i < n; i++) if (is_tainted(b.pics[i].dec) && !b.h_err[i]) b.h_err[i] = kErrNotRecovered;
    { std::lock_guard<std::mutex> lk(sm_); st_.chain_recoveries++; }
    const auto since_epoch = std::chrono::steady_clock::now().time_since_epoch();
    chain_block_until_ns_ = std::chrono::duration_cast<std::chrono::nanoseconds>(since_epoch).count() + 30ll * 1000 * 1000 * 1000;
    static bool said = false;
    if (!said) { said = true;
        fprintf(stderr, "jm_amd_dec: device %d: a chain launch ran out of time waiting for workgroups (is the GPU shared?) -- its pictures were decoded "
                "again by the stage kernels; chain launches pause for 30 s\n", device_);
    }
}

void Engine::dump_chain_state(Batch &b) {
    const int n = (int)b.pics.size(), stride = chain_ctl_ints();
    std::vector<int> ctl((size_t)kMaxBatch * stride + chain_tail_ints());
    if (hipMemcpy(ctl.data(), b.d_ctl, ctl.size() * sizeof(int), hipMemcpyDeviceToHost) != hipSuccess) { (void)hipGetLastError(); return; }
    const int *lw = ctl.data() + (size_t)kMaxBatch * stride;
    int n_band_wgs = 0, n_recon_groups = 0;
    for (int i = 0; i < n; i++) if (b.h_pics[i].stages & PS_CHAIN) { const int bands = (b.h_pics[i].mb_h + 15) / 16;
        n_band_wgs += ((b.h_pics[i].stages & PS_CHAIN_INTRA) ? 4 : 2) * bands;
        if (!(b.h_pics[i].stages & PS_RECON)) n_recon_groups += b.h_pics[i].mb_h * ((b.h_pics[i].mb_w + 7) / 8); }
    fprintf(stderr, "  census: abort %d | reconstruction workgroups started %d done %d (work list: %d groups x 2, some empty) | "
        "band workgroups started %d done %d of %d | highest work-list index started %d | band budget %d / %d\n",
        lw[0], lw[1], lw[2], n_recon_groups, lw[3], lw[4], n_band_wgs, lw[5], chain_bands_max_, chain_bands_max_intra_);
    if (lw[2] > 0) fprintf(stderr, "  reconstruction workgroups: %.2f us each on average, of which %.2f us in wait_final (wave 0)\n",
        0.01 * (double)(unsigned)lw[7] / lw[2], 0.01 * (double)(unsigned)lw[6] / lw[2]);
    if (lw[8]) fprintf(stderr,
        "  FIRST give-up (of %d): code %d (1 fin: reconstruction waits for the deblocking of picture `pic`; 2 bits: a deblocking band of `pic` waits "
        "for its reconstruction; 4 ring; 8 intra ring; 16 ifin) pic %d where 0x%x (fin: band << 16 | macroblock column; bits: row << 16 | column, bit 31 of "
        "the row = intra band; ring: band << 16 | chroma) needed %d saw %d / %d\n", lw[8], lw[9], lw[10], (unsigned)lw[11], lw[12], lw[13], lw[14]);
    if (lw[8]) fprintf(stderr,
        "  ... the same counter read by an atomic read-modify-write when the wait gave up: %d (equal to what the polls saw = the producer stood there; larger = "
        "published and not seen) | waiter: XCC %d, HW_ID1 0x%08x (wave %d SIMD %d CU %d SA %d SE %d), %d looks | its timer skipped %d clock gap(s), the longest "
        "%.2f ms | wait limit of the launch %.1f ms\n", lw[16], lw[17] & 15, (unsigned)lw[18], lw[18] & 31, (lw[18] >> 8) & 3, (lw[18] >> 10) & 15,
        (lw[18] >> 16) & 1, (lw[18] >> 18) & 7, lw[19], lw[20], lw[21] * 1e-5, lw[15] * 1e-5);
    for (int i = 0; i < n; i++) {
        const PicParams &q = b.h_pics[i];
        if (!(q.stages & PS_CHAIN)) continue;
        const int *c = ctl.data() + (size_t)i * stride;
        const int bands = (q.mb_h + 15) / 16;
        fprintf(stderr, "  picture %2d dec %p %dx%d stages 0x%x%s deps %d err %d reach %d/%d |", i, (void *)b.pics[i].dec, q.mb_w, q.mb_h, q.stages,
            (q.stages & PS_RECON) ? " (reconstructed before the launch)" : "", q.n_deps, b.h_err[i], b.pics[i].reach_rows, b.pics[i].reach_cols);
        for (int k = 0; k < bands; k++) fprintf(stderr, " b%d ring %d/%d fin %d/%d", k, c[0 + k], c[32 + k], c[64 + k], c[64 + 32 + k]);
        if (q.stages & PS_CHAIN_INTRA) for (int k = 0; k < bands; k++) fprintf(stderr, " i%d ring %d/%d ifin %d/%d", k, c[128 + k], c[128 + 32 + k], c[192 + k],
            c[192 + 32 + k]);
        int full = 0, first_open = -1, first_open_bits = 0;
        for (int r = 0; r < q.mb_h; r++) { int cnt = 0; for (int w = 0; w < 8; w++) cnt += __builtin_popcount((unsigned)c[256 + r * 8 + w]);
            if (cnt >= q.mb_w) full++; else if (first_open < 0) { first_open = r; first_open_bits = cnt; } }
        fprintf(stderr, " | bitmap: %d of %d rows complete, first open row %d has %d of %d\n", full, q.mb_h, first_open, first_open_bits, q.mb_w);
    }
    const int *ts = lw + chain_tail_head_ints();
    int t0 = 0x7fffffff;
    for (int i = 0; i < n; i++) for (int k = 0; k < 4; k += 2) if (ts[4 * i + k]) t0 = std::min(t0, 0x40000000 - ts[4 * i + k]);
    if (t0 != 0x7fffffff) for (int i = 0; i < n; i++) {
        if (!(b.h_pics[i].stages & PS_CHAIN)) continue;
        auto us = [&](int k) { const int v = ts[4 * i + k]; return v ? ((k & 1) ? v - t0 : 0x40000000 - v - t0) * 0.01 : -1.0; };
        fprintf(stderr, "  time line picture %2d dec %p: reconstruction %.1f .. %.1f us, bands %.1f .. %.1f us\n", i, (void *)b.pics[i].dec, us(0), us(1),
            us(2), us(3));
    }
}

void Engine::complete(Lane &ln, Batch &b, bool failed) {
    LANE_TRACE("retire lane %d batch %llu pics %zu\n", (int)(&ln - lanes_), b.serial, b.pics.size());
    if (!failed && (b.redo || b.any_chain)) {
        bool wait_err = b.redo;
        for (size_t i = 0; i < b.pics.size(); i++) wait_err |= b.h_err[i] != 0 && b.any_chain;
        if (wait_err) {
            static std::atomic<int> dumped{0};
            if (getenv("JM_AMD_DEC_VERBOSE") || (!b.redo && dumped.fetch_add(1) < 4)) {
                fprintf(stderr, "jm_amd_dec: chain launch of %zu pictures gave up%s; codes:", b.pics.size(), b.redo ? " (redo of the batch behind one that did)" : "");
                for (size_t i = 0; i < b.pics.size(); i++) fprintf(stderr, " %d", b.h_err[i]); fprintf(stderr, "\n");
                dump_chain_state(b); }
            std::vector<std::pair<Decoder *, uint32_t>> later;
            if (!b.redo) ln.tainted.clear();
            if (ln.inflight > 1) {
                Batch &nx = ln.ring[(ln.tail + 1) % kBatchRing]; hipEventSynchronize(nx.done); nx.redo = true;
                for (auto &p : nx.pics) if (p.has_picture && p.codec == 0) later.emplace_back(p.dec, 1u << p.pp.cur);
            }
            recover(ln, b, later);
        }
    }
    if (profile_ && !failed) {
        std::lock_guard<std::mutex> lk(sm_);
        auto add = [&](int cls, int e0, int e1, bool ran) {
            if (!ran) return;
            float ms = 0;
            if (hipEventElapsedTime(&ms, b.pev[e0], b.pev[e1]) == hipSuccess) { st_.ns[cls] += ms * 1e6; st_.launches[cls]++; }
        };
        add(3, 0, 1, b.pmask & 1); add(0, 1, 2, b.pmask & 2); add(1, 2, 3, b.pmask & 4); add(2, 3, 4, b.pmask & 8); add(3, 5, 6, b.pmask & 16);
        add(4, 4, 7, b.pmask & 32); add(5, 10, 11, b.pmask & 64); add(5, 12, 13, b.pmask & 128);
        add(6, 14, 15, b.pmask & 256); add(6, 16, 17, b.pmask & 512); add(8, 4, 18, b.pmask & 2048);
        add(10, 19, 20, b.pmask & 8192); add(10, 21, 22, b.pmask & 16384);
        if (b.pmask & 1024) { float ms = 0; if (hipEventElapsedTime(&ms, b.jev[0], b.jev[1]) == hipSuccess) { st_.ns[7] += ms * 1e6; st_.launches[7]++; } }
        if (b.pmask & 4096) { float ms = 0; if (hipEventElapsedTime(&ms, b.mev[0], b.mev[1]) == hipSuccess) { st_.ns[9] += ms * 1e6; st_.launches[9]++; } }
        for (int k = 0; k < kKernelClasses; k++) { st_.pics[k] += b.npics[k]; st_.alg_bytes[k] += b.alg[k]; }
        st_.batches++; st_.batch_pics += (long long)b.pics.size();
        const int li = (int)(&ln - lanes_);
        st_.lane_batches[li]++; st_.lane_pics[li] += (long long)b.pics.size();
        if (b.last_ev >= 0) {
            float ms = 0;
            if (hipEventElapsedTime(&ms, b.pev[0], b.pev[b.last_ev]) == hipSuccess) st_.lane_busy_ns[li] += ms * 1e6;
            const Batch &pb = ln.ring[(ln.tail + kBatchRing - 1) % kBatchRing];
            if (pb.serial + 1 == b.serial && pb.last_ev >= 0 && hipEventElapsedTime(&ms, pb.pev[pb.last_ev], b.pev[0]) == hipSuccess && ms > 0) {
                st_.lane_gap_ns[li] += ms * 1e6;
                float mu = 0, mp = 0;
                const bool h264 = !b.pics.empty() && b.pics[0].codec == 0;
                if (h264 && !b.launched_dry && hipEventElapsedTime(&mu, pb.pev[pb.last_ev], b.pev[8]) == hipSuccess && mu > 0) st_.lane_upwait_ns[li] += std::min(mu, ms) * 1e6;
                if (h264 && !b.launched_dry && hipEventElapsedTime(&mp, pb.pev[pb.last_ev], b.pev[9]) == hipSuccess && mp > 0) st_.lane_prewait_ns[li] += std::min(mp, ms) * 1e6;
            }
        }
        (void)hipGetLastError();
    }
    if (b.any_chain && !failed) { static const bool timeline = getenv("JM_AMD_DEC_CHAIN_TIMELINE") != nullptr;
        if (timeline) { fprintf(stderr, "jm_amd_dec: chain launch of %zu pictures\n", b.pics.size()); dump_chain_state(b); } }
    if (b.h_err[kMaxBatch]) { std::lock_guard<std::mutex> lk(sm_); st_.wait_gap_launches++; st_.wait_gap_max_ticks = std::max(st_.wait_gap_max_ticks,
        (long long)(unsigned)b.h_err[kMaxBatch + 1]);
        if (getenv("JM_AMD_DEC_VERBOSE")) fprintf(stderr, "jm_amd_dec: a chain launch's waits saw %d clock gap(s), the longest %.2f ms: its waves were not run meanwhile "
            "(chain launch %lld of this process, batch %llu of its lane, %.1f ms after the engine's first trace point, CLOCK_MONOTONIC %.3f s when it retired)\n",
            b.h_err[kMaxBatch], (unsigned)b.h_err[kMaxBatch + 1] * 1e-5, st_.chain_batches + 1, b.serial, trace_ms(),
            std::chrono::duration<double>(std::chrono::steady_clock::now().time_since_epoch()).count());
        b.h_err[kMaxBatch] = b.h_err[kMaxBatch + 1] = 0; }
    if (b.any_chain && !failed) { static const bool census = getenv("JM_AMD_DEC_CENSUS") != nullptr;
        if (census) { int tail[32];
            if (hipMemcpy(tail, b.d_ctl + (size_t)kMaxBatch * chain_ctl_ints(), sizeof tail, hipMemcpyDeviceToHost) == hipSuccess) {
                std::lock_guard<std::mutex> lk(sm_); st_.quad_windows += tail[22]; st_.private_windows += tail[23]; }
            else (void)hipGetLastError(); } }
    if (b.any_chain && !failed) { std::lock_guard<std::mutex> lk(sm_); st_.chain_batches++; st_.chain_i_batches += b.chain_with_intra;
        for (auto &p : b.pics) st_.chain_pics += p.has_picture && (p.chain_ok || p.chain_intra); }
    { std::lock_guard<std::mutex> lk(m_); const int li = (int)(&ln - lanes_);
      for (auto &p : b.pics) { p.dec->engine_state().inflight--; p.dec->engine_state().lane_inflight[li]--; } pending_gen_++; }
    for (size_t i = 0; i < b.pics.size(); i++) if (b.h_err[i]) { b.pics[i].dec->on_device_wait_error(b.h_err[i]); b.h_err[i] = 0;
        std::lock_guard<std::mutex> lk(sm_); st_.wait_errors++; }
    for (size_t i = 0; i < b.pics.size(); i++) {
        const EnginePic &p = b.pics[i];
        if (p.codec != 1 || (p.hash_type <= 0 && !p.hash_md5)) continue;
        if (failed || b.redo || !p.has_picture || !p.hp.hash_mode || !b.h_hash) { p.dec->on_picture_hash(p, nullptr, -1); continue; }
        if (p.hash_md5) {
            const uint8_t *digests = (const uint8_t *)(b.h_hash + i * kHashStride + kMd5Word);
            int bad = -1;
            for (int c = 2; c >= 0; c--) if (memcmp(digests + 16 * c, p.md5_want[c], 16) != 0) bad = c;
            p.dec->on_picture_md5(p, digests, bad);
            continue;
        }
        const uint32_t *words = b.h_hash + i * kHashStride, *got = words + (p.hash_type == 1 ? 0 : 3);
        int bad = -1;
        for (int c = 2; c >= 0; c--) if (got[c] != p.hash_want[c]) bad = c;
        p.dec->on_picture_hash(p, words, bad);
    }
    for (auto &p : b.pics) p.dec->on_engine_done(p, failed);
    b.pics.clear();
}

void Engine::look_for_other_users() {
    if (!kfd_gpu_id_) return;
    const long long now = std::chrono::duration_cast<std::chrono::nanoseconds>(std::chrono::steady_clock::now().time_since_epoch()).count();
    const bool was = gpu_shared_.load(std::memory_order_relaxed);
    if (now - shared_checked_ns_.load() <= (was ? 200ll : 1000ll) * 1000 * 1000) return;
    shared_checked_ns_ = now;
    const bool sh = kfd_gpu_has_other_users(kfd_gpu_id_);
    if (sh != was) fprintf(stderr, "jm_amd_dec: device %d: %s -- chain launches %s\n", device_,
        sh ? "another process has compute queues on this GPU" : "the GPU is no longer shared", sh ? "off" : "on again");
    gpu_shared_.store(sh, std::memory_order_relaxed);
}

void Engine::run() {
    hipSetDevice(device_);
    { const char *e = getenv("JM_AMD_DEC_TIMER_SLACK_NS"); const unsigned long ns = e ? strtoul(e, nullptr, 10) : 0ul; if (ns) prctl(PR_SET_TIMERSLACK, ns, 0, 0, 0); }
    for (;;) {
        bool progressed = false;
        for (auto &ln : lanes_) {
            while (ln.inflight > 0) {
                const hipError_t q = hipEventQuery(ln.ring[ln.tail].done);
                if (q == hipErrorNotReady) break;
                if (q != hipSuccess && !device_failed_) { device_failed_ = true;
                    fprintf(stderr, "jm_amd_dec: device %d failed: %s -- every handle on it now returns errors\n", device_, hipGetErrorString(q)); }
                { auto t0 = std::chrono::steady_clock::now(); complete(ln, ln.ring[ln.tail], q != hipSuccess);
                    long long ns = std::chrono::duration_cast<std::chrono::nanoseconds>(std::chrono::steady_clock::now() - t0).count();
                    std::lock_guard<std::mutex> lk(sm_); st_.complete_ns += ns; }
                ln.tail = (ln.tail + 1) % kBatchRing; ln.inflight--;
                progressed = true;
            }
        }
        lingered_ = false;
        for (int li = 0; li < kLanes; li++) {
            Lane &ln = lanes_[li];
            static const int max_inflight = getenv("JM_AMD_DEC_INFLIGHT") ? atoi(getenv("JM_AMD_DEC_INFLIGHT")) : 2;
            if (ln.inflight >= (li == kIntraLane && early_intra_ && deep_queues_ ? 1 : max_inflight)) continue;
            Batch &b = ln.ring[ln.head];
            bool have;
            if (li == kOrdinaryLane) { bool any; { std::lock_guard<std::mutex> lk(m_); any = !pending_.empty(); } if (any) look_for_other_users(); }
            { std::lock_guard<std::mutex> lk(m_); have = !pending_.empty() && form(ln, li, b); }
            if (!have) continue;
            if (device_failed_) { complete(ln, b, true); progressed = true; continue; }
            { auto t0 = std::chrono::steady_clock::now(); launch(ln, b);
                long long ns = std::chrono::duration_cast<std::chrono::nanoseconds>(std::chrono::steady_clock::now() - t0).count();
                std::lock_guard<std::mutex> lk(sm_); st_.launch_ns += ns; }
            ln.head = (ln.head + 1) % kBatchRing; ln.inflight++;
            progressed = true;
        }
        if (progressed) continue;
        bool busy = false;
        for (auto &ln : lanes_) busy |= ln.inflight > 0;
        if (busy || lingered_) std::this_thread::sleep_for(std::chrono::microseconds(20));
        else { std::unique_lock<std::mutex> lk(m_); cv_.wait_for(lk, std::chrono::milliseconds(2), [&] { return !pending_.empty(); }); }
    }
}

}
```

### jmcodec_amd/csrc/engine.h

```cpp
#pragma once
#include "jobs.h"
#include "out_tables.h"
#include "hevc_jobs.h"
#include "jpeg_jobs.h"
#include <atomic>
#include <condition_variable>
#include <deque>
#include <mutex>
#include <string>
#include <thread>
#include <vector>

struct ihipStream_t; struct ihipEvent_t;

namespace jmamd {

class Decoder;

constexpr int kBatchRing = 4;
constexpr int kMaxChainGroups = 128 * 1024;
constexpr int kMaxChainBands = 384;
constexpr int kMaxChainBandsIntra = 256;
constexpr int kMinChainLag = 24;
constexpr int kOrdinaryLane = 0;
constexpr int kIntraLane = 1;
constexpr int kErrNotRecovered = 32;
constexpr int kLanes = 4;
constexpr int kHevcLane = 2;
constexpr int kHevcIntraLane = 3;
constexpr int kEarlyIntraAhead = 10;

struct EnginePic {
    Decoder *dec = nullptr;
    bool has_picture = false;
    PicParams pp;
    int codec = 0;
    HevcPicParams hp;
    JpegPicParams jp; long long jpeg_alg_bytes = 0;
    int job_slot = -1;
    ihipEvent_t *uploaded = nullptr; unsigned long long upload_seq = 0;
    OutSide out[2];
    bool before_empty() const { return out[kBefore].frames() == 0; }
    int mb_w = 0, mb_h = 0, disp_w = 0, disp_h = 0;
    bool wait_prev_pack = false;
    bool chain_ok = false;
    bool chain_intra = false;
    int classic_stages = 0;
    uint32_t ref_mask = 0, out_mask = 0;
    bool bipred = false;
    int reach_rows = 0;
    int reach_cols = 0;
    long long alg_bytes[5] = {0, 0, 0, 0, 0};
    unsigned long long seq = 0;
    int hash_type = 0, hash_poc = 0; uint32_t hash_want[3] = {0, 0, 0};
    bool hash_md5 = false; uint8_t md5_want[3][16] = {};
    int lane(bool chaining = false) const {
        if (codec == 2) return kHevcLane;
        if (codec == 1) return (has_picture && hp.n_pus == 0 && hp.n_itbs > 0) ? kHevcIntraLane : kHevcLane;
        return (has_picture && (pp.stages & PS_INTRA_LDS) && !(chaining && chain_intra)) ? kIntraLane : kOrdinaryLane;
    }
};

constexpr int kKernelClasses = 11;
struct EngineStats {
    double ns[kKernelClasses] = {}; long long launches[kKernelClasses] = {}, pics[kKernelClasses] = {}, alg_bytes[kKernelClasses] = {};
    long long batches = 0, batch_pics = 0, chain_batches = 0, chain_pics = 0, wait_errors = 0, chain_recoveries = 0;
    long long chain_i_batches = 0;
    long long forms = 0, form_decoders = 0, form_pending = 0;
    long long launch_ns = 0, complete_ns = 0;
    long long rej_other_lane = 0, rej_cross_lane = 0, rej_tables = 0;
    long long wait_gap_launches = 0, wait_gap_max_ticks = 0;
    long long quad_windows = 0, private_windows = 0;
    long long early_intra = 0;
    long long blocked_ns = 0, blocked_n = 0;
    double lane_upwait_ns[4] = {0, 0, 0, 0}, lane_prewait_ns[4] = {0, 0, 0, 0}; long long lane_dry[4] = {0, 0, 0, 0};
    double lane_busy_ns[4] = {0, 0, 0, 0}, lane_gap_ns[4] = {0, 0, 0, 0}; long long lane_batches[4] = {0, 0, 0, 0}, lane_pics[4] = {0, 0, 0, 0};
};

struct EngineDecoderState {
    int inflight = 0;
    int lane_inflight[4] = {0, 0, 0, 0};
    uint32_t displayed[4] = {0, 0, 0, 0};
    unsigned long long next_seq = 0;
    int n_pending = 0;
    unsigned long long form_tag = 0;
    unsigned long long scan_tag = 0; uint32_t scan_touched = 0; int scan_ahead = 0; bool scan_closed = false;
    long long blocked_since = 0;
    int in_batch = 0; uint32_t batch_written = 0, batch_read = 0; bool batch_stop = false;
};

void mem_trace(const char *tag);

class Engine {
public:
    static Engine *get(int device);
    void submit(EnginePic &&p);
    unsigned long long upload(uint8_t *dev, const uint8_t *host, size_t n, ihipEvent_t *ev, bool spread = true);
    void set_profile(bool on) { profile_ = on; }
    int  fetchers() const { return fetchers_.load(std::memory_order_relaxed); }
    void fetch_begin() { fetchers_.fetch_add(1, std::memory_order_relaxed); }
    void fetch_end() { fetchers_.fetch_sub(1, std::memory_order_relaxed); }
    bool set_knob(const std::string &key, long long v);
    EngineStats stats();
    int device() const { return device_; }
    bool gpu_shared() const { return gpu_shared_.load(std::memory_order_relaxed); }

private:
    explicit Engine(int device);
    void run();
    struct Batch {
        PicParams *h_pics = nullptr, *d_pics = nullptr;
        HevcPicParams *h_hpics = nullptr, *d_hpics = nullptr;
        JpegPicParams *h_jpics = nullptr, *d_jpics = nullptr; ihipEvent_t *jev[2] = {nullptr, nullptr};
        int *d_progress = nullptr;
        int *d_ctl = nullptr;
        int *h_err = nullptr, *d_err = nullptr;
        uint32_t *d_hash = nullptr, *h_hash = nullptr; bool any_hash = false;
        ihipEvent_t *mev[2] = {nullptr, nullptr};
        bool any_chain = false, chain_with_intra = false, redo = false; int max_depth = 1;
        int max_mbs = 0, max_mb_h = 0; bool any_bipred = false, any_field = false;
        uint32_t *h_groups = nullptr, *d_groups = nullptr;
        OutTables out;
        uint8_t *deint_scratch = nullptr; size_t deint_cap = 0;
        ihipEvent_t *done = nullptr, *kdone = nullptr, *packed = nullptr, *pre_done = nullptr, *pev[23] = {nullptr};
        std::vector<EnginePic> pics;
        unsigned pmask = 0;
        long long alg[kKernelClasses] = {}; int npics[kKernelClasses] = {};
        int last_ev = -1;
        bool launched_dry = false;
        unsigned long long serial = 0;
    };
    struct Lane {
        ihipStream_t *stream = nullptr, *pack_stream = nullptr, *pre_stream = nullptr;
        ihipEvent_t *pack_hist[2] = {nullptr, nullptr};
        Batch ring[kBatchRing];
        int head = 0, tail = 0, inflight = 0;
        unsigned long long launched = 0;
        long long wait_since_ns = 0;
        std::vector<Decoder *> tainted;
    };
    bool form(Lane &ln, int lane_idx, Batch &b);
    bool cross_lane_ = true, early_intra_ = true;
    long long fill_linger_ns_ = 4000 * 1000;
    unsigned long long scan_tag_form_ = 0;
    bool lingered_ = false;
    int decoders_pending_ = 0;
    bool deep_queues_ = false;
    std::atomic<int> early_intra_ahead_{kEarlyIntraAhead};
    long long early_scan_ns_ = 0; unsigned long long early_scan_tag_ = 0;
    unsigned long long pending_gen_ = 0, early_scanned_gen_ = ~0ull;
    bool others_done(Decoder *d, int lane_idx, unsigned long long seq);
    void inflight_masks(Decoder *d, uint32_t &touched);
    std::atomic<int> chain_max_streams_{16};
    int chain_bands_max_ = kMaxChainBands, chain_bands_max_intra_ = kMaxChainBandsIntra;
    std::atomic<int> chain_depth_{8}, chain_lag_steps_{24};
    std::atomic<int> chain_depth_few_{16};
    struct Recent { Decoder *dec; long long t; int mbs; };
    std::vector<Recent> recent_;
    std::vector<std::vector<uint32_t>> group_buckets_;
    std::vector<uint32_t> bucket_tmp_;
    void launch(Lane &ln, Batch &b);
    void run_side(Batch &b, int side, ihipStream_t *s, bool in_launch);
    void complete(Lane &ln, Batch &b, bool failed);
    void dump_chain_state(Batch &b);
    void recover(Lane &ln, Batch &b, const std::vector<std::pair<Decoder *, uint32_t>> &later);

    int device_, numa_node_ = -1;
    unsigned kfd_gpu_id_ = 0; std::atomic<bool> gpu_shared_{false}; std::atomic<long long> shared_checked_ns_{0};
    void look_for_other_users();
    ihipStream_t *copy_streams_[4] = {nullptr, nullptr, nullptr, nullptr}; int n_copy_ = 2;
    std::mutex um_; unsigned long long upload_seq_ = 0;
    Lane lanes_[kLanes];
    std::mutex m_; std::condition_variable cv_;
    std::deque<EnginePic> pending_;
    bool profile_ = false, ok_ = false, device_failed_ = false;
    std::atomic<int> debug_stall_{0};
    std::atomic<int> debug_no_bi_{0};
    std::atomic<int> fetchers_{0};
    std::atomic<long long> chain_block_until_ns_{0};
    int chain_linger_streams_ = 2;
    std::mutex sm_; EngineStats st_;
    std::thread th_;
};

}
```

### jmcodec_amd/csrc/kernel_common.h

```cpp
#pragma once
#include <hip/hip_runtime.h>
#include "jobs.h"

namespace jmamd {

__device__ __forceinline__ const uint8_t *ref_plane(const PicParams &pp, int slot) { return pp.surf[slot & 31] + ((slot & 32) ? (pp.pitch >> 1) : 0); }
__device__ __forceinline__ uint8_t *cur_plane(const PicParams &pp) { return pp.surf[pp.cur] + (pp.field == 2 ? (pp.pitch >> 1) : 0); }
__device__ __forceinline__ int chroma_mvy_offset(const PicParams &pp, int slot) {
    return pp.field == 0 || ((slot >> 5) & 1) == pp.field - 1 ? 0 : (pp.field == 2 ? 2 : -2);
}

__device__ __forceinline__ int clip3(int lo, int hi, int v) { return v < lo ? lo : (v > hi ? hi : v); }
__device__ __forceinline__ int clip1(int v) { return v < 0 ? 0 : (v > 255 ? 255 : v); }
__device__ __forceinline__ int iabs(int v) { return v < 0 ? -v : v; }
__device__ __forceinline__ int tap6(int a, int b, int c, int d, int e, int f) { return a - 5 * b + 20 * c + 20 * d - 5 * e + f; }

__device__ __forceinline__ int norm4(int qp_rem, int cls) {
    unsigned long long t = cls == 0 ? 0x12100E0D0B0AULL : (cls == 1 ? 0x1D1917141210ULL : 0x171412100E0DULL);
    return (int)((t >> (8 * qp_rem)) & 0xff);
}
__device__ __forceinline__ int qpc_from_qpi(int qpi) {
    if (qpi < 30) return qpi;
    int k = qpi - 30;
    unsigned long long lo = 0x9888776655433210ULL;
    unsigned int hi = 0xAAAA99u;
    int v = k < 16 ? (int)((lo >> (4 * k)) & 15) : (int)((hi >> (4 * (k - 16))) & 15);
    return 29 + v;
}
static __device__ const uint8_t kAlpha[52] = { 0,0,0,0,0,0,0,0,0,0,0,0,0,0,0,0,4,4,5,6,7,8,9,10,12,13,15,17,20,22,25,28,
    32,36,40,45,50,56,63,71,80,90,101,113,127,144,162,182,203,226,255,255 };
static __device__ const uint8_t kBeta[52] = { 0,0,0,0,0,0,0,0,0,0,0,0,0,0,0,0,2,2,2,3,3,3,3,4,4,4,6,6,7,7,8,8,
    9,9,10,10,11,11,12,12,13,13,14,14,15,15,16,16,17,17,18,18 };
static __device__ const uint8_t kTc0[52][3] = {
 {0,0,0},{0,0,0},{0,0,0},{0,0,0},{0,0,0},{0,0,0},{0,0,0},{0,0,0},{0,0,0},{0,0,0},{0,0,0},{0,0,0},{0,0,0},{0,0,0},{0,0,0},{0,0,0},{0,0,0},
 {0,0,1},{0,0,1},{0,0,1},{0,0,1},{0,1,1},{0,1,1},{1,1,1},{1,1,1},{1,1,1},{1,1,1},{1,1,2},{1,1,2},{1,1,2},{1,1,2},{1,2,3},{1,2,3},
 {2,2,3},{2,2,4},{2,3,4},{2,3,4},{3,3,5},{3,4,6},{3,4,6},{4,5,7},{4,5,8},{4,6,9},{5,7,10},{6,8,11},{6,8,13},{7,10,14},{8,11,16},
 {9,12,18},{10,13,20},{11,15,23},{13,17,25} };

__device__ __forceinline__ int chroma_qp(int qpy, int off) {
    return qpc_from_qpi(clip3(0, 51, qpy + off));
}
__device__ __forceinline__ int level_scale4(int qp_rem, int pos) {
    int i = pos >> 2, j = pos & 3;
    int cls = (!(i & 1) && !(j & 1)) ? 0 : (((i & 1) && (j & 1)) ? 1 : 2);
    return 16 * norm4(qp_rem, cls);
}
__device__ __forceinline__ int dequant4w(int c, int qp, int pos, int w) {
    int i = pos >> 2, j = pos & 3;
    int cls = (!(i & 1) && !(j & 1)) ? 0 : (((i & 1) && (j & 1)) ? 1 : 2);
    int ls = w * norm4(qp % 6, cls), s = qp / 6;
    return s >= 4 ? (c * ls) << (s - 4) : (c * ls + (1 << (3 - s))) >> (4 - s);
}
__device__ __forceinline__ int dequant4(int c, int qp, int pos) {
    int ls = level_scale4(qp % 6, pos), s = qp / 6;
    return s >= 4 ? (c * ls) << (s - 4) : (c * ls + (1 << (3 - s))) >> (4 - s);
}
__device__ __forceinline__ void idct4x4(int *d) {
#pragma unroll
    for (int i = 0; i < 4; i++) {
        int a = d[4 * i], b = d[4 * i + 1], c = d[4 * i + 2], e = d[4 * i + 3];
        int e0 = a + c, e1 = a - c, e2 = (b >> 1) - e, e3 = b + (e >> 1);
        d[4 * i] = e0 + e3; d[4 * i + 1] = e1 + e2; d[4 * i + 2] = e1 - e2; d[4 * i + 3] = e0 - e3;
    }
#pragma unroll
    for (int j = 0; j < 4; j++) {
        int a = d[j], b = d[4 + j], c = d[8 + j], e = d[12 + j];
        int g0 = a + c, g1 = a - c, g2 = (b >> 1) - e, g3 = b + (e >> 1);
        d[j] = (g0 + g3 + 32) >> 6; d[4 + j] = (g1 + g2 + 32) >> 6; d[8 + j] = (g1 - g2 + 32) >> 6; d[12 + j] = (g0 - g3 + 32) >> 6;
    }
}
__device__ __forceinline__ int blk_to_raster(int blk) { return ((((blk >> 1) & 1) + 2 * (blk >> 3)) << 2) | ((blk & 1) + 2 * ((blk >> 2) & 1)); }
__device__ __forceinline__ int raster_to_blk(int r) { int bx = r & 3, by = r >> 2; return (by >> 1) * 8 + (bx >> 1) * 4 + (by & 1) * 2 + (bx & 1); }

typedef uint32_t jm_g2u __attribute__((ext_vector_type(2)));
typedef uint32_t jm_g4u __attribute__((ext_vector_type(4)));
__device__ __forceinline__ uint2 gld_u2(const void *p) { const jm_g2u v = *(const __attribute__((address_space(1))) jm_g2u *)p; return make_uint2(v.x, v.y); }
__device__ __forceinline__ void gst_u4(void *p, uint4 v) { const jm_g4u t = {v.x, v.y, v.z, v.w}; *(__attribute__((address_space(1))) jm_g4u *)p = t; }

struct MbWords { uint32_t w[8]; };
__device__ __forceinline__ MbWords load_mbrec_uniform(const MbRec *p) {
    typedef uint32_t v8u __attribute__((ext_vector_type(8)));
    const v8u v = *(const __attribute__((address_space(4))) v8u *)(uintptr_t)p;
    return __builtin_bit_cast(MbWords, v);
}

struct MbW { uint32_t w[8]; };
__device__ __forceinline__ MbW load_mbw(const MbRec *p) {
    const uint4 *q = (const uint4 *)p;
    uint4 a = q[0], b = q[1];
    MbW m; m.w[0] = a.x; m.w[1] = a.y; m.w[2] = a.z; m.w[3] = a.w; m.w[4] = b.x; m.w[5] = b.y; m.w[6] = b.z; m.w[7] = b.w;
    return m;
}
__device__ __forceinline__ MbW select_mbw(bool c, const MbW &a, const MbW &b) {
    MbW m;
#pragma unroll
    for (int i = 0; i < 8; i++) m.w[i] = c ? a.w[i] : b.w[i];
    return m;
}
__device__ __forceinline__ int mbw_kind(const MbW &m) { return m.w[0] & 255; }
__device__ __forceinline__ int mbw_qp(const MbW &m) { return (m.w[0] >> 8) & 255; }
__device__ __forceinline__ int mbw_modes(const MbW &m) { return (m.w[0] >> 16) & 255; }
__device__ __forceinline__ int mbw_flags(const MbW &m) { return m.w[0] >> 24; }
__device__ __forceinline__ int mbw_cbp_blk(const MbW &m) { return m.w[1] & 0xffff; }
__device__ __forceinline__ int mbw_slice(const MbW &m) { return m.w[1] >> 24; }
__device__ __forceinline__ int mbw_ref(const MbW &m, int b8) { return (int)(int8_t)(m.w[3] >> (8 * b8)); }
__device__ __forceinline__ void mbw_mv(const PicParams &pp, const MbW &m, int rpos, int &mx, int &my) {
    if (mbw_flags(m) & MBF_MV_EXT) { const short *v = pp.mv_ext + ((size_t)m.w[4] + rpos) * 2; mx = v[0]; my = v[1]; }
    else {
        int b8 = (rpos >> 3) * 2 + ((rpos & 3) >> 1);
        uint32_t w = b8 == 0 ? m.w[4] : (b8 == 1 ? m.w[5] : (b8 == 2 ? m.w[6] : m.w[7]));
        mx = (int)(int16_t)(w & 0xffff); my = (int)(int16_t)(w >> 16);
    }
}
__device__ __forceinline__ void mbw_motion(const PicParams &pp, const MbW &m, int rpos, int &s0, int &s1, int &x0, int &y0, int &x1, int &y1) {
    int b8 = (rpos >> 3) * 2 + ((rpos & 3) >> 1);
    s0 = mbw_ref(m, b8); s1 = -1; x1 = y1 = 0;
    if (mbw_modes(m) & MBM_BIPRED) {
        const short *rec = pp.mv_ext + (size_t)m.w[4] * 2;
        x0 = rec[rpos * 2]; y0 = rec[rpos * 2 + 1]; x1 = rec[32 + rpos * 2]; y1 = rec[32 + rpos * 2 + 1];
        s1 = ((const int8_t *)(rec + 64))[b8];
    } else mbw_mv(pp, m, rpos, x0, y0);
}
__device__ __forceinline__ int boundary_strength(const PicParams &pp, const MbW &p, int rp, const MbW &q, int rq, bool mb_edge, bool horizontal) {
    if (mbw_kind(p) != MB_INTER || mbw_kind(q) != MB_INTER) return mb_edge && !(pp.field && horizontal) ? 4 : 3;
    const int vlim = pp.field ? 2 : 4;
    if (((mbw_cbp_blk(p) >> raster_to_blk(rp)) & 1) || ((mbw_cbp_blk(q) >> raster_to_blk(rq)) & 1)) return 2;
    if (!((mbw_modes(p) | mbw_modes(q)) & MBM_BIPRED)) {
        if (mbw_ref(p, (rp >> 3) * 2 + ((rp & 3) >> 1)) != mbw_ref(q, (rq >> 3) * 2 + ((rq & 3) >> 1))) return 1;
        int px, py, qx, qy; mbw_mv(pp, p, rp, px, py); mbw_mv(pp, q, rq, qx, qy);
        return (iabs(px - qx) >= 4 || iabs(py - qy) >= vlim) ? 1 : 0;
    }
    int p0, p1, q0, q1, px0, py0, px1, py1, qx0, qy0, qx1, qy1;
    mbw_motion(pp, p, rp, p0, p1, px0, py0, px1, py1); mbw_motion(pp, q, rq, q0, q1, qx0, qy0, qx1, qy1);
    int np = (p0 >= 0) + (p1 >= 0), nq = (q0 >= 0) + (q1 >= 0);
    if (np != nq) return 1;
    auto far = [vlim](int ax, int ay, int bx, int by) { return iabs(ax - bx) >= 4 || iabs(ay - by) >= vlim; };
    if (np == 1) {
        bool pl1 = p0 < 0, ql1 = q0 < 0;
        if ((pl1 ? p1 : p0) != (ql1 ? q1 : q0)) return 1;
        return far(pl1 ? px1 : px0, pl1 ? py1 : py0, ql1 ? qx1 : qx0, ql1 ? qy1 : qy0) ? 1 : 0;
    }
    if (!((p0 == q0 && p1 == q1) || (p0 == q1 && p1 == q0))) return 1;
    bool straight = far(px0, py0, qx0, qy0) || far(px1, py1, qx1, qy1), crossed = far(px0, py0, qx1, qy1) || far(px1, py1, qx0, qy0);
    if (p0 != p1) return (p0 == q0 ? straight : crossed) ? 1 : 0;
    return (straight && crossed) ? 1 : 0;
}

}
```

### jmcodec_amd/csrc/kernels.h

```cpp
#pragma once
#include <hip/hip_runtime_api.h>
#include "jobs.h"

namespace jmamd {
void launch_recon_inter(const PicParams *d_pics, int n, int max_mbs, bool any_bipred, bool any_field, int *d_err, hipStream_t st);
void launch_recon_intra(const PicParams *d_pics, int n, hipStream_t st);
void launch_deblock(const PicParams *d_pics, int n, hipStream_t st);
constexpr int kMaxMbRows = 1056;
bool intra_lds_supported(int mb_w, int mb_h);
void launch_intra_lds(const PicParams *d_pics, int n, int max_mb_h, int *ctl, int *err, hipStream_t st);
bool deblock_lds_supported(int mb_w, int mb_h);
constexpr int kDeblockMaxBands = 32, kDeblockProgressStride = 2 * kDeblockMaxBands;
void launch_deblock_prep(const PicParams *d_pics, int n, int max_mbs, hipStream_t st);
void launch_deblock_lds(const PicParams *d_pics, int n, int max_mb_h, int *ctl, int *err, bool debug_stall, hipStream_t st);
bool chain_supported(int mb_w, int mb_h);
void launch_chain(const PicParams *d_pics, const uint32_t *d_groups, int n_groups, bool with_intra, int *ctl, int *err, bool debug_stall, hipStream_t st);
int  chain_band_rows();
int  deblock_row_lag();
int  chain_resident_workgroups(bool intra);
int  chain_ctl_ints();
int  chain_tail_head_ints(); int chain_tail_wait_limit();
int  chain_tail_ints();
void launch_packout(const PackJob *d_jobs, int n, int max_width, int max_height, hipStream_t st);
int  scale_tiles(int tw, int th);
void launch_scale_pack(const ScaleJob *d_jobs, int n, int max_tiles, hipStream_t st);
int  rgb_tiles(int tw, int th);
void launch_rgb_pack(const RgbJob *d_jobs, int n, int identity_tiles, int scaled_tiles, int chroma_tiles, hipStream_t st);
int  deint_items(int w, int h);
void launch_deint(const DeintJob *d_jobs, int n, int max_items, hipStream_t st);
int  deint2_items(int w, int h);
void launch_deint2(const DeintJob *d_jobs, int n, int max_items, hipStream_t st);
void launch_frame_to_argb(const uint8_t *d_src, int w, int h, int fmt, uint8_t *d_dst, int dst_pitch, hipStream_t st);
void launch_frame_to_nv12_pitch(const uint8_t *d_src, int w, int h, int fmt, uint8_t *d_dst, int pitch, hipStream_t st);
}
```

### jmcodec_amd/csrc/kernels.hip

```cpp
#include <hip/hip_runtime.h>
#include <cstdlib>
#include "jobs.h"
#include "kernels.h"
#include "kernel_common.h"
#include "deblock_packed.h"
#include "recon_device.h"

namespace jmamd {

template <bool HAS_BI, bool FIELD>
__global__ __launch_bounds__(256) void k_recon_inter(const PicParams *pics, int *err) {
    const PicParams &pp = pics[blockIdx.y];
    const int per_xcd = ((int)gridDim.x + 7) >> 3;
    const int blk = ((int)blockIdx.x & 7) * per_xcd + ((int)blockIdx.x >> 3);
    if (!(pp.stages & PS_RECON) || blk * 4 >= pp.mb_w * pp.mb_h) return;
    __shared__ ReconLds sm;
    const int n_mbs = pp.mb_w * pp.mb_h;
    const int mb = blk * 4 + __builtin_amdgcn_readfirstlane((int)(threadIdx.x >> 6));
    recon_inter_wave<false, false, HAS_BI, FIELD>(pp, mb, mb < n_mbs, sm, ChainView{nullptr, err});
}

constexpr int kWaves = 16;
constexpr int kIntraWaves = 8;
constexpr int kMaxRows = kMaxMbRows;
static_assert(kMaxRows == kMaxMbRows && kMaxRows * sizeof(int) <= 8192, "progress[] must hold every row activate() lets through");

__device__ __forceinline__ void wait_row(volatile int *progress, int row, int need) {
    if (row < 0) return;
    while (progress[row] < need) __builtin_amdgcn_s_sleep(1);
    __builtin_amdgcn_fence(__ATOMIC_ACQUIRE, "workgroup");
}
__device__ __forceinline__ void publish_row(volatile int *progress, int row, int done, int lane) {
    __builtin_amdgcn_fence(__ATOMIC_RELEASE, "workgroup");
    if (lane == 0) progress[row] = done;
}

struct IntraTile {
    uint8_t y[17][28];
    uint8_t e8[2][32];
    uint8_t c[2][9][12];
};

__device__ void intra4x4_block(IntraTile &t, const ResTile &rt, int blk, int mode, bool availA, bool availB, bool availC, bool availD, int lane) {
    if (lane >= 16) return;
    int rpos = blk_to_raster(blk), bx = rpos & 3, by = rpos >> 2;
    int px = lane & 3, py = lane >> 2;
    int ox = 1 + bx * 4, oy = 1 + by * 4;
    int T[9], L[5];
#pragma unroll
    for (int k = 0; k < 4; k++) { T[k + 1] = availB ? t.y[oy - 1][ox + k] : 128; L[k + 1] = availA ? t.y[oy + k][ox - 1] : 128; }
#pragma unroll
    for (int k = 4; k < 8; k++) T[k + 1] = (availB && availC) ? t.y[oy - 1][ox + k] : T[4];
    T[0] = L[0] = availD ? t.y[oy - 1][ox - 1] : 128;
#define TT(k) T[(k) + 1]
#define LL(k) L[(k) + 1]
    int p;
    switch (mode) {
    case 0: p = TT(px); break;
    case 1: p = LL(py); break;
    case 2:
        if (availA && availB) p = (TT(0) + TT(1) + TT(2) + TT(3) + LL(0) + LL(1) + LL(2) + LL(3) + 4) >> 3;
        else if (availA) p = (LL(0) + LL(1) + LL(2) + LL(3) + 2) >> 2;
        else if (availB) p = (TT(0) + TT(1) + TT(2) + TT(3) + 2) >> 2;
        else p = 128;
        break;
    case 3: p = (px == 3 && py == 3) ? (TT(6) + 3 * TT(7) + 2) >> 2 : (TT(px + py) + 2 * TT(px + py + 1) + TT(px + py + 2) + 2) >> 2; break;
    case 4:
        if (px > py) p = (TT(px - py - 2) + 2 * TT(px - py - 1) + TT(px - py) + 2) >> 2;
        else if (px < py) p = (LL(py - px - 2) + 2 * LL(py - px - 1) + LL(py - px) + 2) >> 2;
        else p = (TT(0) + 2 * TT(-1) + LL(0) + 2) >> 2;
        break;
    case 5: { int z = 2 * px - py, i = px - (py >> 1);
        if (z >= 0) p = (z & 1) ? (TT(i - 2) + 2 * TT(i - 1) + TT(i) + 2) >> 2 : (TT(i - 1) + TT(i) + 1) >> 1;
        else if (z == -1) p = (LL(0) + 2 * TT(-1) + TT(0) + 2) >> 2;
        else p = (LL(py - 1) + 2 * LL(py - 2) + LL(py - 3) + 2) >> 2;
        break; }
    case 6: { int z = 2 * py - px, i = py - (px >> 1);
        if (z >= 0) p = (z & 1) ? (LL(i - 2) + 2 * LL(i - 1) + LL(i) + 2) >> 2 : (LL(i - 1) + LL(i) + 1) >> 1;
        else if (z == -1) p = (LL(0) + 2 * TT(-1) + TT(0) + 2) >> 2;
        else p = (TT(px - 1) + 2 * TT(px - 2) + TT(px - 3) + 2) >> 2;
        break; }
    case 7: { int i = px + (py >> 1); p = (py & 1) ? (TT(i) + 2 * TT(i + 1) + TT(i + 2) + 2) >> 2 : (TT(i) + TT(i + 1) + 1) >> 1; break; }
    default: { int z = px + 2 * py, i = py + (px >> 1);
        if (z > 5) p = LL(3);
        else if (z == 5) p = (LL(2) + 3 * LL(3) + 2) >> 2;
        else p = (z & 1) ? (LL(i) + 2 * LL(i + 1) + LL(i + 2) + 2) >> 2 : (LL(i) + LL(i + 1) + 1) >> 1;
        break; }
    }
#undef TT
#undef LL
    p = clip1(p + rt.y[(by * 4 + py) * 16 + bx * 4 + px]);
    t.y[oy + py][ox + px] = (uint8_t)p;
}

__device__ void intra8x8_block(IntraTile &t, const ResTile &rt, int b8, int mode, bool availA, bool availB, bool availC, bool availD, int lane) {
    int ox = 1 + (b8 & 1) * 8, oy = 1 + (b8 >> 1) * 8;
    uint8_t *raw = t.e8[0], *fe = t.e8[1];
    if (lane == 0) raw[0] = availD ? t.y[oy - 1][ox - 1] : 128;
    else if (lane <= 16) { int k = lane - 1; raw[lane] = availB ? t.y[oy - 1][ox + ((k >= 8 && !availC) ? 7 : k)] : 128; }
    else if (lane <= 24) raw[lane] = availA ? t.y[oy + lane - 17][ox - 1] : 128;
    if (lane == 0) {
        int c = raw[0], t0 = raw[1], l0 = raw[17];
        fe[0] = (uint8_t)(!availD ? 128 : ((availA &&
            availB) ? (t0 + 2 * c + l0 + 2) >> 2 : (availB ? (3 * c + t0 + 2) >> 2 : (availA ? (3 * c + l0 + 2) >> 2 : c))));
    } else if (lane <= 16) {
        int k = lane - 1, c = raw[lane];
        int lo = k == 0 ? (availD ? raw[0] : c) : raw[lane - 1], hi = k == 15 ? c : raw[lane + 1];
        fe[lane] = (uint8_t)((lo + 2 * c + hi + 2) >> 2);
    } else if (lane <= 24) {
        int k = lane - 17, c = raw[lane];
        int lo = k == 0 ? (availD ? raw[0] : c) : raw[lane - 1], hi = k == 7 ? c : raw[lane + 1];
        fe[lane] = (uint8_t)((lo + 2 * c + hi + 2) >> 2);
    }
    int x = lane & 7, y = lane >> 3;
#define TT(i) ((i) < 0 ? fe[0] : fe[1 + (i)])
#define LL(i) ((i) < 0 ? fe[0] : fe[17 + (i)])
    int p;
    switch (mode) {
    case 0: p = TT(x); break;
    case 1: p = LL(y); break;
    case 2: {
        int st = 0, sl = 0;
        for (int i = 0; i < 8; i++) { st += TT(i); sl += LL(i); }
        p = (availA && availB) ? (st + sl + 8) >> 4 : (availA ? (sl + 4) >> 3 : (availB ? (st + 4) >> 3 : 128));
        break; }
    case 3: p = (x == 7 && y == 7) ? (TT(14) + 3 * TT(15) + 2) >> 2 : (TT(x + y) + 2 * TT(x + y + 1) + TT(x + y + 2) + 2) >> 2; break;
    case 4:
        if (x > y) p = (TT(x - y - 2) + 2 * TT(x - y - 1) + TT(x - y) + 2) >> 2;
        else if (x < y) p = (LL(y - x - 2) + 2 * LL(y - x - 1) + LL(y - x) + 2) >> 2;
        else p = (TT(0) + 2 * TT(-1) + LL(0) + 2) >> 2;
        break;
    case 5: { int z = 2 * x - y, i = x - (y >> 1);
        if (z >= 0) p = (z & 1) ? (TT(i - 2) + 2 * TT(i - 1) + TT(i) + 2) >> 2 : (TT(i - 1) + TT(i) + 1) >> 1;
        else if (z == -1) p = (LL(0) + 2 * TT(-1) + TT(0) + 2) >> 2;
        else p = (LL(y - 2 * x - 1) + 2 * LL(y - 2 * x - 2) + LL(y - 2 * x - 3) + 2) >> 2;
        break; }
    case 6: { int z = 2 * y - x, i = y - (x >> 1);
        if (z >= 0) p = (z & 1) ? (LL(i - 2) + 2 * LL(i - 1) + LL(i) + 2) >> 2 : (LL(i - 1) + LL(i) + 1) >> 1;
        else if (z == -1) p = (LL(0) + 2 * TT(-1) + TT(0) + 2) >> 2;
        else p = (TT(x - 2 * y - 1) + 2 * TT(x - 2 * y - 2) + TT(x - 2 * y - 3) + 2) >> 2;
        break; }
    case 7: { int i = x + (y >> 1); p = (y & 1) ? (TT(i) + 2 * TT(i + 1) + TT(i + 2) + 2) >> 2 : (TT(i) + TT(i + 1) + 1) >> 1; break; }
    default: { int z = x + 2 * y, i = y + (x >> 1);
        if (z > 13) p = LL(7);
        else if (z == 13) p = (LL(6) + 3 * LL(7) + 2) >> 2;
        else p = (z & 1) ? (LL(i) + 2 * LL(i + 1) + LL(i + 2) + 2) >> 2 : (LL(i) + LL(i + 1) + 1) >> 1;
        break; }
    }
#undef TT
#undef LL
    p = clip1(p + rt.y[((b8 >> 1) * 8 + y) * 16 + (b8 & 1) * 8 + x]);
    t.y[oy + y][ox + x] = (uint8_t)p;
}

__device__ __forceinline__ int plane_pred(const uint8_t *tile, int stride, int n, int x, int y) {
    int h2 = n >> 1, Hs = 0, Vs = 0;
    for (int k = 0; k < h2; k++) {
        Hs += (k + 1) * (tile[-stride + h2 + k] - tile[-stride + h2 - 2 - k]);
        Vs += (k + 1) * (tile[(h2 + k) * stride - 1] - tile[(h2 - 2 - k) * stride - 1]);
    }
    int a = 16 * (tile[(n - 1) * stride - 1] + tile[-stride + n - 1]);
    int b = n == 16 ? (5 * Hs + 32) >> 6 : (34 * Hs + 32) >> 6;
    int c = n == 16 ? (5 * Vs + 32) >> 6 : (34 * Vs + 32) >> 6;
    return clip1((a + b * (x - (h2 - 1)) + c * (y - (h2 - 1)) + 16) >> 5);
}

__device__ void intra_mb(const PicParams &pp, const MbRec &r, int mbx, int mby, IntraTile &t, ResTile &rt, int lane) {
    int pitch = pp.pitch, W = pp.mb_w * 16, H = pp.mb_h * 16;
    uint8_t *dst = cur_plane(pp);
    uint8_t *dst_c = dst + pp.chroma_offset;
    bool availA = r.flags & MBF_AVAIL_A, availB = r.flags & MBF_AVAIL_B, availC = r.flags & MBF_AVAIL_C, availD = r.flags & MBF_AVAIL_D;
    if (mb_has_residual(r)) mb_residual_to_lds(pp, r, rt, lane);
    else { for (int k = lane; k < 256; k += 64) rt.y[k] = 0; for (int k = lane; k < 128; k += 64) (&rt.c[0][0])[k] = 0; }
    {
        int x0 = mbx * 16, y0 = mby * 16;
        if (lane < 25) { int x = clip3(0, W - 1, x0 - 1 + lane), y = clip3(0, H - 1, y0 - 1); t.y[0][lane] = dst[(size_t)y * pitch + x]; }
        else if (lane >= 32 && lane < 48) { int i = lane - 32; int x = clip3(0, W - 1, x0 - 1); t.y[1 + i][0] = dst[(size_t)(y0 + i) * pitch + x]; }
        int cx0 = mbx * 8, cy0 = mby * 8, CW = W >> 1, CH = H >> 1;
        if (lane < 18) { int pl = lane / 9, i = lane % 9; int x = clip3(0, CW - 1, cx0 - 1 + i), y = clip3(0, CH - 1, cy0 - 1);
            t.c[pl][0][i] = dst_c[(size_t)y * pitch + 2 * x + pl]; }
        else if (lane >= 32 && lane < 48) { int pl = (lane - 32) >> 3, i = (lane - 32) & 7; int x = clip3(0, CW - 1, cx0 - 1);
            t.c[pl][1 + i][0] = dst_c[(size_t)(cy0 + i) * pitch + 2 * x + pl]; }
    }
    if (r.kind == MB_I4 && (r.modes & MBM_T8X8)) {
        for (int b8 = 0; b8 < 4; b8++) {
            int bx = b8 & 1, by = b8 >> 1;
            int mode = (r.u.i4[b8 >> 1] >> ((b8 & 1) * 4)) & 15;
            bool a = bx > 0 || availA, b = by > 0 || availB, d = (bx > 0 && by > 0) ? true : (bx > 0 ? availB : (by > 0 ? availA : availD));
            bool c = b8 == 0 ? availB : (b8 == 1 ? availC : b8 == 2);
            intra8x8_block(t, rt, b8, mode, a, b, c, d, lane);
        }
    } else if (r.kind == MB_I4) {
        for (int blk = 0; blk < 16; blk++) {
            int rpos = blk_to_raster(blk), bx = rpos & 3, by = rpos >> 2;
            int mode = (r.u.i4[rpos >> 1] >> ((rpos & 1) * 4)) & 15;
            bool a = bx > 0 || availA, b = by > 0 || availB, d = (bx > 0 && by > 0) ? true : (bx > 0 ? availB : (by > 0 ? availA : availD));
            bool c;
            if (by == 0) c = bx < 3 ? availB : availC;
            else c = !(bx == 3 || blk == 3 || blk == 11 || blk == 7 || blk == 13 || blk == 15);
            intra4x4_block(t, rt, blk, mode, a, b, c, d, lane);
        }
    } else {
        int mode = (r.modes >> 2) & 3;
        int rb = lane >> 2, row = lane & 3, bx = rb & 3, by = rb >> 2, y = by * 4 + row;
        int dc = 128;
        if (mode == 2) {
            int st = 0, sl = 0;
            for (int i = 0; i < 16; i++) { st += t.y[0][1 + i]; sl += t.y[1 + i][0]; }
            dc = (availA && availB) ? (st + sl + 16) >> 5 : (availA ? (sl + 8) >> 4 : (availB ? (st + 8) >> 4 : 128));
        }
        int v[4];
#pragma unroll
        for (int k = 0; k < 4; k++) {
            int x = bx * 4 + k, p;
            if (mode == 0) p = t.y[0][1 + x];
            else if (mode == 1) p = t.y[1 + y][0];
            else if (mode == 2) p = dc;
            else p = plane_pred(&t.y[1][1], 28, 16, x, y);
            v[k] = clip1(p + rt.y[y * 16 + x]);
        }
#pragma unroll
        for (int k = 0; k < 4; k++) t.y[1 + y][1 + bx * 4 + k] = (uint8_t)v[k];
    }
    {
        int cmode = r.modes & 3, cx = lane & 7, cy = lane >> 3;
        int out[2];
#pragma unroll
        for (int pl = 0; pl < 2; pl++) {
            int p;
            if (cmode == 0) {
                int bx = cx >> 2, by = cy >> 2, st = 0, sl = 0;
                for (int i = 0; i < 4; i++) { st += t.c[pl][0][1 + bx * 4 + i]; sl += t.c[pl][1 + by * 4 + i][0]; }
                if (bx == by) p = (availA && availB) ? (st + sl + 4) >> 3 : (availA ? (sl + 2) >> 2 : (availB ? (st + 2) >> 2 : 128));
                else if (bx == 1) p = availB ? (st + 2) >> 2 : (availA ? (sl + 2) >> 2 : 128);
                else p = availA ? (sl + 2) >> 2 : (availB ? (st + 2) >> 2 : 128);
            } else if (cmode == 1) p = t.c[pl][1 + cy][0];
            else if (cmode == 2) p = t.c[pl][0][1 + cx];
            else p = plane_pred(&t.c[pl][1][1], 12, 8, cx, cy);
            out[pl] = clip1(p + rt.c[pl][cy * 8 + cx]);
        }
        *(uint16_t *)(dst_c + (size_t)(mby * 8 + cy) * pitch + mbx * 16 + cx * 2) = (uint16_t)(out[0] | (out[1] << 8));
    }
    {
        int row = lane >> 2, xq = lane & 3;
        const uint8_t *s = &t.y[1 + row][1 + xq * 4];
        *(uint32_t *)(dst + (size_t)(mby * 16 + row) * pitch + mbx * 16 + xq * 4) = s[0] | (s[1] << 8) | (s[2] << 16) | (s[3] << 24);
    }
}

__global__ __launch_bounds__(kIntraWaves * 64) void k_recon_intra(const PicParams *pics) {
    const PicParams &pp = pics[blockIdx.y];
    if (!(pp.stages & PS_INTRA_V1)) return;
    __shared__ volatile int progress[kMaxRows];
    __shared__ IntraTile tiles[kIntraWaves];
    __shared__ ResTile res[kIntraWaves];
    int wave = threadIdx.x >> 6, lane = threadIdx.x & 63;
    for (int i = threadIdx.x; i < kMaxRows; i += blockDim.x) progress[i] = 0;
    __syncthreads();
    for (int row = wave; row < pp.mb_h; row += kIntraWaves) {
        const MbRec *recs = pp.mbs + (size_t)row * pp.mb_w;
        for (int c0 = 0; c0 < pp.mb_w; c0 += 64) {
            int x = c0 + lane;
            int kind = x < pp.mb_w ? recs[x].kind : MB_INTER;
            unsigned long long m = __ballot(kind == MB_I4 || kind == MB_I16);
            while (m) {
                int xi = c0 + __builtin_ctzll(m);
                m &= m - 1;
                publish_row(progress, row, xi, lane);
                int need = xi + 2 < pp.mb_w ? xi + 2 : pp.mb_w;
                wait_row(progress, row - 1, need);
                MbRec r = recs[xi];
                intra_mb(pp, r, xi, row, tiles[wave], res[wave], lane);
            }
        }
        publish_row(progress, row, pp.mb_w, lane);
    }
}

struct DbTables { uint8_t alpha[52], beta[52], tc0[52][3]; };
struct DbTile {
    uint8_t y[20][24];
    uint8_t c[10][24];
    uint8_t bs[2][4][4];
};

__device__ void deblock_mb(const PicParams &pp, int mbx, int mby, DbTile &t, const DbTables &tb, int lane) {
    int pitch = pp.pitch, mbw = pp.mb_w;
    uint8_t *dst = cur_plane(pp);
    uint8_t *dst_c = dst + pp.chroma_offset;
    const MbW q = load_mbw(&pp.mbs[mby * mbw + mbx]);
    const SliceRec sl = pp.slices[mbw_slice(q)];
    if (sl.disable == 1) return;
    bool has_left = mbx > 0, has_top = mby > 0;
    MbW pl_ = q, pt_ = q;
    if (has_left) { pl_ = load_mbw(&pp.mbs[mby * mbw + mbx - 1]); if (sl.disable == 2 && mbw_slice(pl_) != mbw_slice(q)) has_left = false; }
    if (has_top) { pt_ = load_mbw(&pp.mbs[(mby - 1) * mbw + mbx]); if (sl.disable == 2 && mbw_slice(pt_) != mbw_slice(q)) has_top = false; }
    if (lane < 32) {
        int dir = lane >> 4, e = (lane >> 2) & 3, k = lane & 3;
        int rq = dir == 0 ? k * 4 + e : e * 4 + k;
        int bs;
        if (e == 0) {
            bool have = dir == 0 ? has_left : has_top;
            if (!have) bs = 0;
            else { int rp = dir == 0 ? k * 4 + 3 : 12 + k; bs = boundary_strength(pp, select_mbw(dir == 0, pl_, pt_), rp, q, rq, true, dir == 1); }
        } else bs = boundary_strength(pp, q, dir == 0 ? rq - 1 : rq - 4, q, rq, false, dir == 1);
        if ((e & 1) && (mbw_modes(q) & MBM_T8X8)) bs = 0;
        t.bs[dir][e][k] = (uint8_t)bs;
    }
    int x0 = mbx * 16, y0 = mby * 16;
    {
        for (int i = lane; i < 100; i += 64) {
            int row = i / 5, dw = i % 5;
            int y = y0 - 4 + row, x = x0 - 4 + dw * 4;
            uint32_t v = 0;
            if (y >= 0 && x >= 0) v = *(const uint32_t *)(dst + (size_t)y * pitch + x);
            *(uint32_t *)&t.y[row][dw * 4] = v;
        }
        for (int i = lane; i < 50; i += 64) {
            int row = i / 5, dw = i % 5;
            int y = mby * 8 - 2 + row, x = x0 - 4 + dw * 4;
            uint32_t v = 0;
            if (y >= 0 && x >= 0) v = *(const uint32_t *)(dst_c + (size_t)y * pitch + x);
            *(uint32_t *)&t.c[row][dw * 4] = v;
        }
    }
    int qp_q = mbw_qp(q);
    if (lane < 16) {
        for (int e = 0; e < 4; e++) {
            int bs = t.bs[0][e][lane >> 2];
            if (!bs) continue;
            int qp_p = e == 0 ? mbw_qp(pl_) : qp_q;
            int qpav = (qp_p + qp_q + 1) >> 1;
            int ia = clip3(0, 51, qpav + sl.alpha_off), ib = clip3(0, 51, qpav + sl.beta_off);
            int s[8];
            uint8_t *px = &t.y[4 + lane][e * 4];
#pragma unroll
            for (int k = 0; k < 8; k++) s[k] = px[k];
            filter_luma(s, bs, tb.alpha[ia], tb.beta[ib], tb.tc0[ia]);
#pragma unroll
            for (int k = 1; k < 7; k++) px[k] = (uint8_t)s[k];
        }
    }
    if (lane < 16) {
        for (int e = 0; e < 4; e++) {
            int bs = t.bs[1][e][lane >> 2];
            if (!bs) continue;
            int qp_p = e == 0 ? mbw_qp(pt_) : qp_q;
            int qpav = (qp_p + qp_q + 1) >> 1;
            int ia = clip3(0, 51, qpav + sl.alpha_off), ib = clip3(0, 51, qpav + sl.beta_off);
            int s[8];
#pragma unroll
            for (int k = 0; k < 8; k++) s[k] = t.y[e * 4 + k][4 + lane];
            filter_luma(s, bs, tb.alpha[ia], tb.beta[ib], tb.tc0[ia]);
#pragma unroll
            for (int k = 1; k < 7; k++) t.y[e * 4 + k][4 + lane] = (uint8_t)s[k];
        }
    }
    if (lane < 16) {
        int plane = lane >> 3, row = lane & 7;
        int qc_q = chroma_qp(qp_q, plane ? pp.cr_qp_off : pp.cb_qp_off);
        for (int e = 0; e < 4; e += 2) {
            int bs = t.bs[0][e][row >> 1];
            if (!bs) continue;
            int qc_p = e == 0 ? chroma_qp(mbw_qp(pl_), plane ? pp.cr_qp_off : pp.cb_qp_off) : qc_q;
            int qpav = (qc_p + qc_q + 1) >> 1;
            int ia = clip3(0, 51, qpav + sl.alpha_off), ib = clip3(0, 51, qpav + sl.beta_off);
            int s[4];
            uint8_t *px = &t.c[2 + row][4 + (e * 2) * 2 + plane];
#pragma unroll
            for (int k = 0; k < 4; k++) s[k] = px[(k - 2) * 2];
            filter_chroma(s, bs, tb.alpha[ia], tb.beta[ib], tb.tc0[ia]);
            px[-2] = (uint8_t)s[1]; px[0] = (uint8_t)s[2];
        }
    }
    if (lane < 16) {
        int plane = lane & 1, ccol = lane >> 1;
        int qc_q = chroma_qp(qp_q, plane ? pp.cr_qp_off : pp.cb_qp_off);
        for (int e = 0; e < 4; e += 2) {
            int bs = t.bs[1][e][ccol >> 1];
            if (!bs) continue;
            int qc_p = e == 0 ? chroma_qp(mbw_qp(pt_), plane ? pp.cr_qp_off : pp.cb_qp_off) : qc_q;
            int qpav = (qc_p + qc_q + 1) >> 1;
            int ia = clip3(0, 51, qpav + sl.alpha_off), ib = clip3(0, 51, qpav + sl.beta_off);
            int s[4];
#pragma unroll
            for (int k = 0; k < 4; k++) s[k] = t.c[e * 2 + k][4 + lane];
            filter_chroma(s, bs, tb.alpha[ia], tb.beta[ib], tb.tc0[ia]);
            t.c[e * 2 + 1][4 + lane] = (uint8_t)s[1]; t.c[e * 2 + 2][4 + lane] = (uint8_t)s[2];
        }
    }
    for (int i = lane; i < 100; i += 64) {
        int row = i / 5, dw = i % 5;
        int y = y0 - 4 + row, x = x0 - 4 + dw * 4;
        if (row >= 1 && y >= 0 && x >= 0) *(uint32_t *)(dst + (size_t)y * pitch + x) = *(const uint32_t *)&t.y[row][dw * 4];
    }
    for (int i = lane; i < 50; i += 64) {
        int row = i / 5, dw = i % 5;
        int y = mby * 8 - 2 + row, x = x0 - 4 + dw * 4;
        if (row >= 1 && y >= 0 && x >= 0) *(uint32_t *)(dst_c + (size_t)y * pitch + x) = *(const uint32_t *)&t.c[row][dw * 4];
    }
}

__global__ __launch_bounds__(kWaves * 64) void k_deblock(const PicParams *pics) {
    const PicParams &pp = pics[blockIdx.y];
    if (!(pp.stages & PS_DEBLOCK_V1)) return;
    __shared__ volatile int progress[kMaxRows];
    __shared__ DbTile tiles[kWaves];
    __shared__ DbTables tb;
    int wave = threadIdx.x >> 6, lane = threadIdx.x & 63;
    for (int i = threadIdx.x; i < kMaxRows; i += blockDim.x) progress[i] = 0;
    if (threadIdx.x < 52) { tb.alpha[threadIdx.x] = kAlpha[threadIdx.x]; tb.beta[threadIdx.x] = kBeta[threadIdx.x]; }
    if (threadIdx.x < 156) (&tb.tc0[0][0])[threadIdx.x] = (&kTc0[0][0])[threadIdx.x];
    __syncthreads();
    for (int row = wave; row < pp.mb_h; row += kWaves) {
        for (int x = 0; x < pp.mb_w; x++) {
            int need = x + 2 < pp.mb_w ? x + 2 : pp.mb_w;
            wait_row(progress, row - 1, need);
            deblock_mb(pp, x, row, tiles[wave], tb, lane);
            publish_row(progress, row, x + 1, lane);
        }
    }
}

void launch_recon_inter(const PicParams *d_pics, int n, int max_mbs, bool any_bipred, bool any_field, int *d_err, hipStream_t st) {
    int nblk = ((max_mbs + 3) / 4 + 7) & ~7;
    if (any_field) { if (any_bipred) hipLaunchKernelGGL((k_recon_inter<true, true>), dim3(nblk, n), dim3(256), 0, st, d_pics, d_err);
        else hipLaunchKernelGGL((k_recon_inter<false, true>), dim3(nblk, n), dim3(256), 0, st, d_pics, d_err); }
    else if (any_bipred) hipLaunchKernelGGL((k_recon_inter<true, false>), dim3(nblk, n), dim3(256), 0, st, d_pics, d_err);
    else hipLaunchKernelGGL((k_recon_inter<false, false>), dim3(nblk, n), dim3(256), 0, st, d_pics, d_err);
}
void launch_recon_intra(const PicParams *d_pics, int n, hipStream_t st) { hipLaunchKernelGGL(k_recon_intra, dim3(1, n), dim3(kIntraWaves * 64), 0, st, d_pics);
    }
void launch_deblock(const PicParams *d_pics, int n, hipStream_t st) { hipLaunchKernelGGL(k_deblock, dim3(1, n), dim3(kWaves * 64), 0, st, d_pics); }

}
```

Baseline: 15220.

## Fuse deblock prep into recon and replace setup memsets/copies with one kernel

Per-macroblock deblock strength records are now computed at the end of the inter recon kernel when recon runs, so the separate prep kernel launches only for pictures without recon. The per-batch memsets and host-to-device parameter copies are merged into one batch-setup kernel that reads pinned host memory directly through mapped pointers. The separate pre-stream and its event handoff are removed, and lane streams are created lazily. This cuts launch and API overhead but puts PCIe reads of mapped memory inside a kernel and lengthens the recon kernel.

After: 14860. 0.976x the previous value.

```diff
diff --git a/jmcodec_amd/csrc/bs_packed.h b/jmcodec_amd/csrc/bs_packed.h
--- /dev/null
+++ b/jmcodec_amd/csrc/bs_packed.h
@@ -0,0 +1,53 @@
+#pragma once
+#include "kernel_common.h"
+
+namespace jmamd {
+
+struct DbRec {
+    uint8_t y_bs[32];
+    uint8_t y_ab[3][2];
+    uint8_t y_pad[10];
+    uint8_t c_bs[2][16];
+    uint8_t c_ab[2][3][2];
+    uint8_t c_pad[4];
+};
+static_assert(sizeof(DbRec) == 96, "DbRec must be 96 bytes");
+
+JM_KD void dbrec_lane(const PicParams &pp, const SliceRec sl, const MbW &q, const MbW &pl, const MbW &pt, bool in_left, bool in_top, int t, DbRec *o) {
+    const bool has_left = in_left && !(sl.disable == 2 && mbw_slice(pl) != mbw_slice(q));
+    const bool has_top = in_top && !(sl.disable == 2 && mbw_slice(pt) != mbw_slice(q));
+    const int dir = t >> 4, e = (t >> 2) & 3, k = t & 3;
+    const int rq = dir == 0 ? k * 4 + e : e * 4 + k;
+    int bs;
+    if (sl.disable == 1) bs = 0;
+    else if (e == 0) {
+        const bool have = dir == 0 ? has_left : has_top;
+        const MbW pn = select_mbw(dir == 0, pl, pt);
+        bs = have ? boundary_strength(pp, pn, dir == 0 ? k * 4 + 3 : 12 + k, q, rq, true, dir == 1) : 0;
+    } else bs = boundary_strength(pp, q, dir == 0 ? rq - 1 : rq - 4, q, rq, false, dir == 1);
+    if ((e & 1) && (mbw_modes(q) & MBM_T8X8)) bs = 0;
+    const int cls = e ? 1 : (dir ? 2 : 0);
+    const int qp_p = cls == 0 ? mbw_qp(in_left ? pl : q) : (cls == 2 ? mbw_qp(in_top ? pt : q) : mbw_qp(q)), qp_q = mbw_qp(q);
+    {
+        const int qpav = (qp_p + qp_q + 1) >> 1;
+        const int ia = clip3(0, 51, qpav + sl.alpha_off), ib = clip3(0, 51, qpav + sl.beta_off);
+        const int tc0 = (bs >= 1 && bs <= 3) ? kTc0[ia][bs - 1] : 0;
+        o->y_bs[t] = (uint8_t)(bs | (tc0 << 3));
+        if (k == 0 && (e == 0 || (e == 1 && dir == 0))) { o->y_ab[cls][0] = kAlpha[ia]; o->y_ab[cls][1] = kBeta[ib]; }
+    }
+    if (!(e & 1)) {
+#if defined(__HIPCC__)
+#pragma unroll
+#endif
+        for (int plane = 0; plane < 2; plane++) {
+            const int off = plane ? pp.cr_qp_off : pp.cb_qp_off;
+            const int qpav = (chroma_qp(qp_p, off) + chroma_qp(qp_q, off) + 1) >> 1;
+            const int ia = clip3(0, 51, qpav + sl.alpha_off), ib = clip3(0, 51, qpav + sl.beta_off);
+            const int tc0 = (bs >= 1 && bs <= 3) ? kTc0[ia][bs - 1] : 0;
+            o->c_bs[plane][dir * 8 + (e >> 1) * 4 + k] = (uint8_t)(bs | (tc0 << 3));
+            if (k == 0 && (e == 0 || (e == 2 && dir == 0))) { o->c_ab[plane][cls][0] = kAlpha[ia]; o->c_ab[plane][cls][1] = kBeta[ib]; }
+        }
+    }
+}
+
+}
diff --git a/jmcodec_amd/csrc/deblock_device.h b/jmcodec_amd/csrc/deblock_device.h
--- a/jmcodec_amd/csrc/deblock_device.h
+++ b/jmcodec_amd/csrc/deblock_device.h
@@ -5,18 +5,9 @@
 #include "kernel_common.h"
 #include "chain_common.h"
 #include "deblock_packed.h"
+#include "bs_packed.h"
 
 namespace jmamd {
-
-struct DbRec {
-    uint8_t y_bs[32];
-    uint8_t y_ab[3][2];
-    uint8_t y_pad[10];
-    uint8_t c_bs[2][16];
-    uint8_t c_ab[2][3][2];
-    uint8_t c_pad[4];
-};
-static_assert(sizeof(DbRec) == 96, "DbRec must be 96 bytes");
 
 __device__ __forceinline__ uint32_t perm(uint32_t hi, uint32_t lo, uint32_t sel) { return __builtin_amdgcn_perm(hi, lo, sel); }
 
diff --git a/jmcodec_amd/csrc/deblock_lds.hip b/jmcodec_amd/csrc/deblock_lds.hip
--- a/jmcodec_amd/csrc/deblock_lds.hip
+++ b/jmcodec_amd/csrc/deblock_lds.hip
@@ -10,7 +10,7 @@
 
 __global__ __launch_bounds__(256) void k_deblock_prep(const PicParams *pics) {
     const PicParams &pp = pics[blockIdx.y];
-    if (!(pp.stages & (PS_DEBLOCK_LDS | PS_CHAIN))) return;
+    if (!(pp.stages & (PS_DEBLOCK_LDS | PS_CHAIN)) || (pp.stages & PS_RECON)) return;
     DbRec *out = (DbRec *)pp.dbrec;
     const int per_xcd = ((int)gridDim.x + 7) >> 3;
     const int blk = ((int)blockIdx.x & 7) * per_xcd + ((int)blockIdx.x >> 3);
@@ -22,41 +22,9 @@
     int mbx = mb % pp.mb_w, mby = mb / pp.mb_w;
     const MbW q = load_mbw(&pp.mbs[mb]);
     const SliceRec sl = pp.slices[mbw_slice(q)];
-    bool has_left = mbx > 0, has_top = mby > 0;
-    MbW pl = q, pt = q;
-    if (has_left) { pl = load_mbw(&pp.mbs[mb - 1]); if (sl.disable == 2 && mbw_slice(pl) != mbw_slice(q)) has_left = false; }
-    if (has_top) { pt = load_mbw(&pp.mbs[mb - pp.mb_w]); if (sl.disable == 2 && mbw_slice(pt) != mbw_slice(q)) has_top = false; }
-    int dir = t >> 4, e = (t >> 2) & 3, k = t & 3;
-    int rq = dir == 0 ? k * 4 + e : e * 4 + k;
-    int bs;
-    if (sl.disable == 1) bs = 0;
-    else if (e == 0) {
-        bool have = dir == 0 ? has_left : has_top;
-        const MbW pn = select_mbw(dir == 0, pl, pt);
-        bs = have ? boundary_strength(pp, pn, dir == 0 ? k * 4 + 3 : 12 + k, q, rq, true, dir == 1) : 0;
-    } else bs = boundary_strength(pp, q, dir == 0 ? rq - 1 : rq - 4, q, rq, false, dir == 1);
-    if ((e & 1) && (mbw_modes(q) & MBM_T8X8)) bs = 0;
-    int cls = e ? 1 : (dir ? 2 : 0);
-    int qp_p = cls == 0 ? mbw_qp(pl) : (cls == 2 ? mbw_qp(pt) : mbw_qp(q)), qp_q = mbw_qp(q);
-    DbRec *o = (DbRec *)stage[sub];
-    {
-        int qpav = (qp_p + qp_q + 1) >> 1;
-        int ia = clip3(0, 51, qpav + sl.alpha_off), ib = clip3(0, 51, qpav + sl.beta_off);
-        int tc0 = (bs >= 1 && bs <= 3) ? kTc0[ia][bs - 1] : 0;
-        o->y_bs[t] = (uint8_t)(bs | (tc0 << 3));
-        if (k == 0 && (e == 0 || (e == 1 && dir == 0))) { o->y_ab[cls][0] = kAlpha[ia]; o->y_ab[cls][1] = kBeta[ib]; }
-    }
-    if (!(e & 1)) {
-#pragma unroll
-        for (int plane = 0; plane < 2; plane++) {
-            int off = plane ? pp.cr_qp_off : pp.cb_qp_off;
-            int qpav = (chroma_qp(qp_p, off) + chroma_qp(qp_q, off) + 1) >> 1;
-            int ia = clip3(0, 51, qpav + sl.alpha_off), ib = clip3(0, 51, qpav + sl.beta_off);
-            int tc0 = (bs >= 1 && bs <= 3) ? kTc0[ia][bs - 1] : 0;
-            o->c_bs[plane][dir * 8 + (e >> 1) * 4 + k] = (uint8_t)(bs | (tc0 << 3));
-            if (k == 0 && (e == 0 || (e == 2 && dir == 0))) { o->c_ab[plane][cls][0] = kAlpha[ia]; o->c_ab[plane][cls][1] = kBeta[ib]; }
-        }
-    }
+    const bool in_left = mbx > 0, in_top = mby > 0;
+    const MbW pl = in_left ? load_mbw(&pp.mbs[mb - 1]) : q, pt = in_top ? load_mbw(&pp.mbs[mb - pp.mb_w]) : q;
+    dbrec_lane(pp, sl, q, pl, pt, in_left, in_top, t, (DbRec *)stage[sub]);
     if (t < 6) ((uint4 *)&out[mb])[t] = ((const uint4 *)stage[sub])[t];
 }
 
diff --git a/jmcodec_amd/csrc/deblock_packed.h b/jmcodec_amd/csrc/deblock_packed.h
--- a/jmcodec_amd/csrc/deblock_packed.h
+++ b/jmcodec_amd/csrc/deblock_packed.h
@@ -10,7 +10,8 @@
 
 namespace jmamd {
 
-#if !defined(__HIPCC__)
+#if !defined(__HIPCC__) && !defined(JM_HOST_CLIP_HELPERS)
+#define JM_HOST_CLIP_HELPERS
 JM_DB_HD int clip3(int lo, int hi, int v) { return v < lo ? lo : (v > hi ? hi : v); }
 JM_DB_HD int clip1(int v) { return v < 0 ? 0 : (v > 255 ? 255 : v); }
 JM_DB_HD int iabs(int v) { return v < 0 ? -v : v; }
diff --git a/jmcodec_amd/csrc/engine.cpp b/jmcodec_amd/csrc/engine.cpp
--- a/jmcodec_amd/csrc/engine.cpp
+++ b/jmcodec_amd/csrc/engine.cpp
@@ -63,13 +63,9 @@
         if (hipStreamCreateWithFlags(&copy_streams_[k], hipStreamNonBlocking) != hipSuccess) return; }
     mem_trace("engine: copy stream");
     for (auto &ln : lanes_) {
-        hipStream_t s, p, q;
-        if (hipStreamCreateWithFlags(&s, hipStreamNonBlocking) != hipSuccess || hipStreamCreateWithFlags(&p, hipStreamNonBlocking) != hipSuccess ||
-            hipStreamCreateWithFlags(&q, hipStreamNonBlocking) != hipSuccess) return;
-        ln.stream = s; ln.pack_stream = p; ln.pre_stream = q;
-        mem_trace("engine: lane streams");
         for (auto &b : ln.ring) {
             if (hipHostMalloc((void **)&b.h_pics, sizeof(PicParams) * kMaxBatch, hipHostMallocDefault) != hipSuccess) return;
+            if (hipHostGetDevicePointer((void **)&b.hd_pics, b.h_pics, 0) != hipSuccess) return;
             if (hipMalloc((void **)&b.d_pics, sizeof(PicParams) * kMaxBatch) != hipSuccess) return;
             if (hipHostMalloc((void **)&b.h_hpics, sizeof(HevcPicParams) * kMaxBatch, hipHostMallocDefault) != hipSuccess) return;
             if (hipMalloc((void **)&b.d_hpics, sizeof(HevcPicParams) * kMaxBatch) != hipSuccess) return;
@@ -81,14 +77,16 @@
             if (hipHostMalloc((void **)&b.h_groups, sizeof(uint32_t) * kMaxChainGroups, hipHostMallocDefault) != hipSuccess) return;
             if (hipMalloc((void **)&b.d_groups, sizeof(uint32_t) * kMaxChainGroups) != hipSuccess) return;
             bool tables_ok = true;
+            int k_tab = 0;
             b.out.each([&](auto &t) { const size_t bytes = sizeof(*t.host) * 2 * kOutSideCap;
                 tables_ok = tables_ok && hipHostMalloc((void **)&t.host, bytes, hipHostMallocDefault) == hipSuccess &&
-                            hipMalloc((void **)&t.dev, bytes) == hipSuccess; });
+                            hipHostGetDevicePointer((void **)&b.out_hd[k_tab], t.host, 0) == hipSuccess &&
+                            hipMalloc((void **)&t.dev, bytes) == hipSuccess;
+                k_tab++; });
             if (!tables_ok) return;
             if (hipEventCreateWithFlags(&b.done, hipEventDisableTiming) != hipSuccess) return;
             if (hipEventCreateWithFlags(&b.kdone, hipEventDisableTiming) != hipSuccess) return;
             if (hipEventCreateWithFlags(&b.packed, hipEventDisableTiming) != hipSuccess) return;
-            if (hipEventCreateWithFlags(&b.pre_done, hipEventDisableTiming) != hipSuccess) return;
             for (auto &e : b.pev) if (hipEventCreate(&e) != hipSuccess) return;
         }
     }
@@ -105,6 +103,19 @@
     kfd_gpu_id_ = getenv("JM_AMD_DEC_IGNORE_SHARED_GPU") ? 0 : kfd_gpu_id_of_device(device_);
     th_ = std::thread([this] { pthread_setname_np(pthread_self(), "jm-engine"); numa_bind_this_thread(numa_node_); run(); });
     th_.detach();
+}
+
+bool Engine::lane_streams(Lane &ln) {
+    if (ln.stream) return true;
+    const int first = (int)(&ln - lanes_) & ~1;
+    static_assert(kOrdinaryLane == 0 && kIntraLane == 1 && kHevcLane == 2 && kHevcIntraLane == 3 && kLanes == 4, "lanes pair up by codec");
+    hipStream_t s[4] = {nullptr, nullptr, nullptr, nullptr};
+    for (auto &q : s) if (hipStreamCreateWithFlags(&q, hipStreamNonBlocking) != hipSuccess) { (void)hipGetLastError();
+        for (auto &d : s) if (d) hipStreamDestroy(d);
+        return false; }
+    lanes_[first].stream = s[0]; lanes_[first + 1].stream = s[1]; lanes_[first].pack_stream = s[2]; lanes_[first + 1].pack_stream = s[3];
+    mem_trace("engine: lane streams");
+    return true;
 }
 
 unsigned long long Engine::upload(uint8_t *dev, const uint8_t *host, size_t n, ihipEvent_t *ev, bool spread) {
@@ -386,7 +397,7 @@
     }
     LANE_TRACE("launch lane %d batch %llu pics %d\n", li, b.serial, n);
     int max_mbs = 0, max_mb_h = 0, max_mb_w = 0, stages = 0;
-    bool wait_pack = false, any_hevc = false, any_jpeg = false; int max_jpeg_items = 0;
+    bool wait_pack = false, any_hevc = false, any_jpeg = false, need_prep = false; int max_jpeg_items = 0;
     for (auto &p : b.pics) any_jpeg |= p.codec == 2 && p.has_picture;
     if (any_jpeg && !b.h_jpics) {
         if (hipHostMalloc((void **)&b.h_jpics, sizeof(JpegPicParams) * kMaxBatch, hipHostMallocDefault) != hipSuccess ||
@@ -451,6 +462,7 @@
             if (!refs_in_batch) q.stages |= PS_RECON;
         }
         stages |= b.h_pics[i].stages;
+        need_prep |= (b.h_pics[i].stages & (PS_DEBLOCK_LDS | PS_CHAIN)) && !(b.h_pics[i].stages & PS_RECON);
         if (p.has_picture && !hevc) max_mb_w = std::max(max_mb_w, p.mb_w);
         if (p.has_picture && ((1u << (hevc ? p.hp.cur : p.pp.cur)) & p.dec->engine_state().displayed[li])) wait_pack = true;
         if (hevc && p.has_picture) {
@@ -483,30 +495,36 @@
     for (auto &p : b.pics) p.dec->engine_state().displayed[li] = 0;
     for (auto &p : b.pics) p.dec->engine_state().displayed[li] |= p.out_mask;
     b.max_mbs = max_mbs; b.max_mb_h = max_mb_h; b.redo = false;
+    if (!lane_streams(ln)) { static bool said = false;
+        if (!said) { said = true; fprintf(stderr, "jm_amd_dec: hipStreamCreate failed for lane %d: its batches run on the default stream\n", li); } }
     hipStream_t st = ln.stream, pst = ln.pack_stream;
-    hipStream_t ps = any_hevc ? st : ln.pre_stream;
-    if (!any_hevc && (stages & (PS_INTRA_LDS | PS_DEBLOCK_LDS | PS_CHAIN))) { hipMemsetAsync(b.d_ctl, 0, sizeof(int) * (size_t)n * chain_ctl_ints(), ps);
-        hipMemsetAsync(b.d_ctl + (size_t)kMaxBatch * chain_ctl_ints(), 0, chain_tail_ints() * sizeof(int), ps);
-        if (stages & PS_CHAIN) {
-            const double launch_ms = 0.25 * b.max_depth * std::max(1.0, max_mbs / 8160.0) + 0.8;
-            const unsigned ticks = (unsigned)(std::min(100.0, std::max(10.0, 10.0 * launch_ms)) * 100000.0);
-            static const unsigned forced = getenv("JM_AMD_DEC_CHAIN_WAIT_MS") ? (unsigned)(atof(getenv("JM_AMD_DEC_CHAIN_WAIT_MS")) * 100000.0) : 0u;
-            hipMemsetD32Async((hipDeviceptr_t)(b.d_ctl + (size_t)kMaxBatch * chain_ctl_ints() + chain_tail_wait_limit()), (int)(forced ? forced : ticks), 1, ps);
-        } }
-    if (any_hevc) hipMemcpyAsync(b.d_hpics, b.h_hpics, sizeof(HevcPicParams) * n, hipMemcpyHostToDevice, ps);
-    else hipMemcpyAsync(b.d_pics, b.h_pics, sizeof(PicParams) * n, hipMemcpyHostToDevice, ps);
-    if (any_jpeg) hipMemcpyAsync(b.d_jpics, b.h_jpics, sizeof(JpegPicParams) * n, hipMemcpyHostToDevice, ps);
-    b.out.each([&](auto &t) { for (int side : {kBefore, kAfter}) if (t.n[side])
-        hipMemcpyAsync(t.dev + side * kOutSideCap, t.h(side), sizeof(*t.host) * t.n[side], hipMemcpyHostToDevice, ps); });
-    for (const EnginePic *lu : last_upload) if (lu) hipStreamWaitEvent(ps, lu->uploaded, 0);
-    if (profile_ && !any_hevc) hipEventRecord(b.pev[8], ps);
-    bool prep_early = false;
+    for (const EnginePic *lu : last_upload) if (lu) hipStreamWaitEvent(st, lu->uploaded, 0);
+    if (profile_ && !any_hevc) hipEventRecord(b.pev[8], st);
+    BatchSetup setup;
     if (!any_hevc) {
-        if (stages & (PS_DEBLOCK_LDS | PS_CHAIN)) { launch_deblock_prep(b.d_pics, n, max_mbs, ps); prep_early = true; }
-        if (profile_) hipEventRecord(b.pev[9], ps);
-        hipEventRecord(b.pre_done, ps);
-        hipStreamWaitEvent(st, b.pre_done, 0);
-    }
+        static_assert(sizeof(PicParams) % 4 == 0 && sizeof(PackJob) % 4 == 0 && sizeof(ScaleJob) % 4 == 0 && sizeof(RgbJob) % 4 == 0 && sizeof(DeintJob) % 4 == 0,
+            "k_batch_setup moves dwords");
+        setup.add(b.d_pics, b.hd_pics, sizeof(PicParams) * (size_t)n);
+        if (stages & (PS_INTRA_LDS | PS_DEBLOCK_LDS | PS_CHAIN)) {
+            int *tail = b.d_ctl + (size_t)kMaxBatch * chain_ctl_ints();
+            setup.add(b.d_ctl, nullptr, sizeof(int) * (size_t)n * chain_ctl_ints());
+            setup.add(tail, nullptr, chain_tail_ints() * sizeof(int));
+            if (stages & PS_CHAIN) {
+                const double launch_ms = 0.25 * b.max_depth * std::max(1.0, max_mbs / 8160.0) + 0.8;
+                const unsigned ticks = (unsigned)(std::min(100.0, std::max(10.0, 10.0 * launch_ms)) * 100000.0);
+                static const unsigned forced = getenv("JM_AMD_DEC_CHAIN_WAIT_MS") ? (unsigned)(atof(getenv("JM_AMD_DEC_CHAIN_WAIT_MS")) * 100000.0) : 0u;
+                setup.wait_word = tail + chain_tail_wait_limit(); setup.wait_ticks = (int)(forced ? forced : ticks);
+            }
+        }
+    }
+    if (any_hevc) hipMemcpyAsync(b.d_hpics, b.h_hpics, sizeof(HevcPicParams) * n, hipMemcpyHostToDevice, st);
+    if (any_jpeg) hipMemcpyAsync(b.d_jpics, b.h_jpics, sizeof(JpegPicParams) * n, hipMemcpyHostToDevice, st);
+    { int k_tab = 0;
+      b.out.each([&](auto &t) { for (int side : {kBefore, kAfter})
+          setup.add(t.dev + side * kOutSideCap, (const uint8_t *)b.out_hd[k_tab] + sizeof(*t.host) * (size_t)(side * kOutSideCap), sizeof(*t.host) * (size_t)t.n[side]);
+          k_tab++; }); }
+    launch_batch_setup(setup, st);
+    if (profile_ && !any_hevc) hipEventRecord(b.pev[9], st);
     if (ln.pack_hist[1]) hipStreamWaitEvent(st, ln.pack_hist[1], 0);
     if ((wait_pack || b.out.any(kBefore)) && ln.pack_hist[0]) hipStreamWaitEvent(st, ln.pack_hist[0], 0);
     auto mark = [&](int i, hipStream_t s) { if (profile_) hipEventRecord(b.pev[i], s); };
@@ -540,7 +558,7 @@
     if (stages & PS_INTRA_LDS) { launch_intra_lds(b.d_pics, n, max_mb_h, b.d_ctl, b.d_err, st); b.pmask |= 4; }
     if (stages & PS_INTRA_V1) { launch_recon_intra(b.d_pics, n, st); b.pmask |= 4; }
     if (!any_hevc) mark(3, st);
-    if ((stages & (PS_DEBLOCK_LDS | PS_CHAIN)) && !prep_early) launch_deblock_prep(b.d_pics, n, max_mbs, st);
+    if (need_prep) launch_deblock_prep(b.d_pics, n, max_mbs, st);
     if (stages & PS_DEBLOCK_LDS) { launch_deblock_lds(b.d_pics, n, max_mb_h, b.d_ctl, b.d_err, debug_stall_ == 1, st); b.pmask |= 8; }
     if (stages & PS_DEBLOCK_V1) { launch_deblock(b.d_pics, n, st); b.pmask |= 8; }
     if (!any_hevc) { mark(4, st); b.last_ev = 4; }
diff --git a/jmcodec_amd/csrc/engine.h b/jmcodec_amd/csrc/engine.h
--- a/jmcodec_amd/csrc/engine.h
+++ b/jmcodec_amd/csrc/engine.h
@@ -110,6 +110,7 @@
     void run();
     struct Batch {
         PicParams *h_pics = nullptr, *d_pics = nullptr;
+        const PicParams *hd_pics = nullptr; const void *out_hd[4] = {nullptr, nullptr, nullptr, nullptr};
         HevcPicParams *h_hpics = nullptr, *d_hpics = nullptr;
         JpegPicParams *h_jpics = nullptr, *d_jpics = nullptr; ihipEvent_t *jev[2] = {nullptr, nullptr};
         int *d_progress = nullptr;
@@ -122,7 +123,7 @@
         uint32_t *h_groups = nullptr, *d_groups = nullptr;
         OutTables out;
         uint8_t *deint_scratch = nullptr; size_t deint_cap = 0;
-        ihipEvent_t *done = nullptr, *kdone = nullptr, *packed = nullptr, *pre_done = nullptr, *pev[23] = {nullptr};
+        ihipEvent_t *done = nullptr, *kdone = nullptr, *packed = nullptr, *pev[23] = {nullptr};
         std::vector<EnginePic> pics;
         unsigned pmask = 0;
         long long alg[kKernelClasses] = {}; int npics[kKernelClasses] = {};
@@ -131,7 +132,7 @@
         unsigned long long serial = 0;
     };
     struct Lane {
-        ihipStream_t *stream = nullptr, *pack_stream = nullptr, *pre_stream = nullptr;
+        ihipStream_t *stream = nullptr, *pack_stream = nullptr;
         ihipEvent_t *pack_hist[2] = {nullptr, nullptr};
         Batch ring[kBatchRing];
         int head = 0, tail = 0, inflight = 0;
@@ -159,6 +160,7 @@
     std::vector<Recent> recent_;
     std::vector<std::vector<uint32_t>> group_buckets_;
     std::vector<uint32_t> bucket_tmp_;
+    bool lane_streams(Lane &ln);
     void launch(Lane &ln, Batch &b);
     void run_side(Batch &b, int side, ihipStream_t *s, bool in_launch);
     void complete(Lane &ln, Batch &b, bool failed);
diff --git a/jmcodec_amd/csrc/kernel_common.h b/jmcodec_amd/csrc/kernel_common.h
--- a/jmcodec_amd/csrc/kernel_common.h
+++ b/jmcodec_amd/csrc/kernel_common.h
@@ -1,25 +1,37 @@
 #pragma once
+#include <stdint.h>
+#include <string.h>
+#if defined(__HIPCC__)
 #include <hip/hip_runtime.h>
+#define JM_KD __device__ __forceinline__
+#define JM_KTAB static __device__ const
+#else
+#define JM_KD static inline
+#define JM_KTAB static const
+#endif
 #include "jobs.h"
 
 namespace jmamd {
 
-__device__ __forceinline__ const uint8_t *ref_plane(const PicParams &pp, int slot) { return pp.surf[slot & 31] + ((slot & 32) ? (pp.pitch >> 1) : 0); }
-__device__ __forceinline__ uint8_t *cur_plane(const PicParams &pp) { return pp.surf[pp.cur] + (pp.field == 2 ? (pp.pitch >> 1) : 0); }
-__device__ __forceinline__ int chroma_mvy_offset(const PicParams &pp, int slot) {
+JM_KD const uint8_t *ref_plane(const PicParams &pp, int slot) { return pp.surf[slot & 31] + ((slot & 32) ? (pp.pitch >> 1) : 0); }
+JM_KD uint8_t *cur_plane(const PicParams &pp) { return pp.surf[pp.cur] + (pp.field == 2 ? (pp.pitch >> 1) : 0); }
+JM_KD int chroma_mvy_offset(const PicParams &pp, int slot) {
     return pp.field == 0 || ((slot >> 5) & 1) == pp.field - 1 ? 0 : (pp.field == 2 ? 2 : -2);
 }
 
-__device__ __forceinline__ int clip3(int lo, int hi, int v) { return v < lo ? lo : (v > hi ? hi : v); }
-__device__ __forceinline__ int clip1(int v) { return v < 0 ? 0 : (v > 255 ? 255 : v); }
-__device__ __forceinline__ int iabs(int v) { return v < 0 ? -v : v; }
-__device__ __forceinline__ int tap6(int a, int b, int c, int d, int e, int f) { return a - 5 * b + 20 * c + 20 * d - 5 * e + f; }
+#if defined(__HIPCC__) || !defined(JM_HOST_CLIP_HELPERS)
+#define JM_HOST_CLIP_HELPERS
+JM_KD int clip3(int lo, int hi, int v) { return v < lo ? lo : (v > hi ? hi : v); }
+JM_KD int clip1(int v) { return v < 0 ? 0 : (v > 255 ? 255 : v); }
+JM_KD int iabs(int v) { return v < 0 ? -v : v; }
+#endif
+JM_KD int tap6(int a, int b, int c, int d, int e, int f) { return a - 5 * b + 20 * c + 20 * d - 5 * e + f; }
 
-__device__ __forceinline__ int norm4(int qp_rem, int cls) {
+JM_KD int norm4(int qp_rem, int cls) {
     unsigned long long t = cls == 0 ? 0x12100E0D0B0AULL : (cls == 1 ? 0x1D1917141210ULL : 0x171412100E0DULL);
     return (int)((t >> (8 * qp_rem)) & 0xff);
 }
-__device__ __forceinline__ int qpc_from_qpi(int qpi) {
+JM_KD int qpc_from_qpi(int qpi) {
     if (qpi < 30) return qpi;
     int k = qpi - 30;
     unsigned long long lo = 0x9888776655433210ULL;
@@ -27,35 +39,35 @@
     int v = k < 16 ? (int)((lo >> (4 * k)) & 15) : (int)((hi >> (4 * (k - 16))) & 15);
     return 29 + v;
 }
-static __device__ const uint8_t kAlpha[52] = { 0,0,0,0,0,0,0,0,0,0,0,0,0,0,0,0,4,4,5,6,7,8,9,10,12,13,15,17,20,22,25,28,
+JM_KTAB uint8_t kAlpha[52] = { 0,0,0,0,0,0,0,0,0,0,0,0,0,0,0,0,4,4,5,6,7,8,9,10,12,13,15,17,20,22,25,28,
     32,36,40,45,50,56,63,71,80,90,101,113,127,144,162,182,203,226,255,255 };
-static __device__ const uint8_t kBeta[52] = { 0,0,0,0,0,0,0,0,0,0,0,0,0,0,0,0,2,2,2,3,3,3,3,4,4,4,6,6,7,7,8,8,
+JM_KTAB uint8_t kBeta[52] = { 0,0,0,0,0,0,0,0,0,0,0,0,0,0,0,0,2,2,2,3,3,3,3,4,4,4,6,6,7,7,8,8,
     9,9,10,10,11,11,12,12,13,13,14,14,15,15,16,16,17,17,18,18 };
-static __device__ const uint8_t kTc0[52][3] = {
+JM_KTAB uint8_t kTc0[52][3] = {
  {0,0,0},{0,0,0},{0,0,0},{0,0,0},{0,0,0},{0,0,0},{0,0,0},{0,0,0},{0,0,0},{0,0,0},{0,0,0},{0,0,0},{0,0,0},{0,0,0},{0,0,0},{0,0,0},{0,0,0},
  {0,0,1},{0,0,1},{0,0,1},{0,0,1},{0,1,1},{0,1,1},{1,1,1},{1,1,1},{1,1,1},{1,1,1},{1,1,2},{1,1,2},{1,1,2},{1,1,2},{1,2,3},{1,2,3},
  {2,2,3},{2,2,4},{2,3,4},{2,3,4},{3,3,5},{3,4,6},{3,4,6},{4,5,7},{4,5,8},{4,6,9},{5,7,10},{6,8,11},{6,8,13},{7,10,14},{8,11,16},
  {9,12,18},{10,13,20},{11,15,23},{13,17,25} };
 
-__device__ __forceinline__ int chroma_qp(int qpy, int off) {
+JM_KD int chroma_qp(int qpy, int off) {
     return qpc_from_qpi(clip3(0, 51, qpy + off));
 }
-__device__ __forceinline__ int level_scale4(int qp_rem, int pos) {
+JM_KD int level_scale4(int qp_rem, int pos) {
     int i = pos >> 2, j = pos & 3;
     int cls = (!(i & 1) && !(j & 1)) ? 0 : (((i & 1) && (j & 1)) ? 1 : 2);
     return 16 * norm4(qp_rem, cls);
 }
-__device__ __forceinline__ int dequant4w(int c, int qp, int pos, int w) {
+JM_KD int dequant4w(int c, int qp, int pos, int w) {
     int i = pos >> 2, j = pos & 3;
     int cls = (!(i & 1) && !(j & 1)) ? 0 : (((i & 1) && (j & 1)) ? 1 : 2);
     int ls = w * norm4(qp % 6, cls), s = qp / 6;
     return s >= 4 ? (c * ls) << (s - 4) : (c * ls + (1 << (3 - s))) >> (4 - s);
 }
-__device__ __forceinline__ int dequant4(int c, int qp, int pos) {
+JM_KD int dequant4(int c, int qp, int pos) {
     int ls = level_scale4(qp % 6, pos), s = qp / 6;
     return s >= 4 ? (c * ls) << (s - 4) : (c * ls + (1 << (3 - s))) >> (4 - s);
 }
-__device__ __forceinline__ void idct4x4(int *d) {
+JM_KD void idct4x4(int *d) {
 #pragma unroll
     for (int i = 0; i < 4; i++) {
         int a = d[4 * i], b = d[4 * i + 1], c = d[4 * i + 2], e = d[4 * i + 3];
@@ -69,42 +81,48 @@
         d[j] = (g0 + g3 + 32) >> 6; d[4 + j] = (g1 + g2 + 32) >> 6; d[8 + j] = (g1 - g2 + 32) >> 6; d[12 + j] = (g0 - g3 + 32) >> 6;
     }
 }
-__device__ __forceinline__ int blk_to_raster(int blk) { return ((((blk >> 1) & 1) + 2 * (blk >> 3)) << 2) | ((blk & 1) + 2 * ((blk >> 2) & 1)); }
-__device__ __forceinline__ int raster_to_blk(int r) { int bx = r & 3, by = r >> 2; return (by >> 1) * 8 + (bx >> 1) * 4 + (by & 1) * 2 + (bx & 1); }
+JM_KD int blk_to_raster(int blk) { return ((((blk >> 1) & 1) + 2 * (blk >> 3)) << 2) | ((blk & 1) + 2 * ((blk >> 2) & 1)); }
+JM_KD int raster_to_blk(int r) { int bx = r & 3, by = r >> 2; return (by >> 1) * 8 + (bx >> 1) * 4 + (by & 1) * 2 + (bx & 1); }
 
+#if defined(__HIPCC__)
 typedef uint32_t jm_g2u __attribute__((ext_vector_type(2)));
 typedef uint32_t jm_g4u __attribute__((ext_vector_type(4)));
-__device__ __forceinline__ uint2 gld_u2(const void *p) { const jm_g2u v = *(const __attribute__((address_space(1))) jm_g2u *)p; return make_uint2(v.x, v.y); }
-__device__ __forceinline__ void gst_u4(void *p, uint4 v) { const jm_g4u t = {v.x, v.y, v.z, v.w}; *(__attribute__((address_space(1))) jm_g4u *)p = t; }
+JM_KD uint2 gld_u2(const void *p) { const jm_g2u v = *(const __attribute__((address_space(1))) jm_g2u *)p; return make_uint2(v.x, v.y); }
+JM_KD void gst_u4(void *p, uint4 v) { const jm_g4u t = {v.x, v.y, v.z, v.w}; *(__attribute__((address_space(1))) jm_g4u *)p = t; }
 
 struct MbWords { uint32_t w[8]; };
-__device__ __forceinline__ MbWords load_mbrec_uniform(const MbRec *p) {
+JM_KD MbWords load_mbrec_uniform(const MbRec *p) {
     typedef uint32_t v8u __attribute__((ext_vector_type(8)));
     const v8u v = *(const __attribute__((address_space(4))) v8u *)(uintptr_t)p;
     return __builtin_bit_cast(MbWords, v);
 }
+#endif
 
 struct MbW { uint32_t w[8]; };
-__device__ __forceinline__ MbW load_mbw(const MbRec *p) {
+#if defined(__HIPCC__)
+JM_KD MbW load_mbw(const MbRec *p) {
     const uint4 *q = (const uint4 *)p;
     uint4 a = q[0], b = q[1];
     MbW m; m.w[0] = a.x; m.w[1] = a.y; m.w[2] = a.z; m.w[3] = a.w; m.w[4] = b.x; m.w[5] = b.y; m.w[6] = b.z; m.w[7] = b.w;
     return m;
 }
-__device__ __forceinline__ MbW select_mbw(bool c, const MbW &a, const MbW &b) {
+#else
+JM_KD MbW load_mbw(const MbRec *p) { MbW m; memcpy(m.w, p, 32); return m; }
+#endif
+JM_KD MbW select_mbw(bool c, const MbW &a, const MbW &b) {
     MbW m;
 #pragma unroll
     for (int i = 0; i < 8; i++) m.w[i] = c ? a.w[i] : b.w[i];
     return m;
 }
-__device__ __forceinline__ int mbw_kind(const MbW &m) { return m.w[0] & 255; }
-__device__ __forceinline__ int mbw_qp(const MbW &m) { return (m.w[0] >> 8) & 255; }
-__device__ __forceinline__ int mbw_modes(const MbW &m) { return (m.w[0] >> 16) & 255; }
-__device__ __forceinline__ int mbw_flags(const MbW &m) { return m.w[0] >> 24; }
-__device__ __forceinline__ int mbw_cbp_blk(const MbW &m) { return m.w[1] & 0xffff; }
-__device__ __forceinline__ int mbw_slice(const MbW &m) { return m.w[1] >> 24; }
-__device__ __forceinline__ int mbw_ref(const MbW &m, int b8) { return (int)(int8_t)(m.w[3] >> (8 * b8)); }
-__device__ __forceinline__ void mbw_mv(const PicParams &pp, const MbW &m, int rpos, int &mx, int &my) {
+JM_KD int mbw_kind(const MbW &m) { return m.w[0] & 255; }
+JM_KD int mbw_qp(const MbW &m) { return (m.w[0] >> 8) & 255; }
+JM_KD int mbw_modes(const MbW &m) { return (m.w[0] >> 16) & 255; }
+JM_KD int mbw_flags(const MbW &m) { return m.w[0] >> 24; }
+JM_KD int mbw_cbp_blk(const MbW &m) { return m.w[1] & 0xffff; }
+JM_KD int mbw_slice(const MbW &m) { return m.w[1] >> 24; }
+JM_KD int mbw_ref(const MbW &m, int b8) { return (int)(int8_t)(m.w[3] >> (8 * b8)); }
+JM_KD void mbw_mv(const PicParams &pp, const MbW &m, int rpos, int &mx, int &my) {
     if (mbw_flags(m) & MBF_MV_EXT) { const short *v = pp.mv_ext + ((size_t)m.w[4] + rpos) * 2; mx = v[0]; my = v[1]; }
     else {
         int b8 = (rpos >> 3) * 2 + ((rpos & 3) >> 1);
@@ -112,7 +130,7 @@
         mx = (int)(int16_t)(w & 0xffff); my = (int)(int16_t)(w >> 16);
     }
 }
-__device__ __forceinline__ void mbw_motion(const PicParams &pp, const MbW &m, int rpos, int &s0, int &s1, int &x0, int &y0, int &x1, int &y1) {
+JM_KD void mbw_motion(const PicParams &pp, const MbW &m, int rpos, int &s0, int &s1, int &x0, int &y0, int &x1, int &y1) {
     int b8 = (rpos >> 3) * 2 + ((rpos & 3) >> 1);
     s0 = mbw_ref(m, b8); s1 = -1; x1 = y1 = 0;
     if (mbw_modes(m) & MBM_BIPRED) {
@@ -121,7 +139,7 @@
         s1 = ((const int8_t *)(rec + 64))[b8];
     } else mbw_mv(pp, m, rpos, x0, y0);
 }
-__device__ __forceinline__ int boundary_strength(const PicParams &pp, const MbW &p, int rp, const MbW &q, int rq, bool mb_edge, bool horizontal) {
+JM_KD int boundary_strength(const PicParams &pp, const MbW &p, int rp, const MbW &q, int rq, bool mb_edge, bool horizontal) {
     if (mbw_kind(p) != MB_INTER || mbw_kind(q) != MB_INTER) return mb_edge && !(pp.field && horizontal) ? 4 : 3;
     const int vlim = pp.field ? 2 : 4;
     if (((mbw_cbp_blk(p) >> raster_to_blk(rp)) & 1) || ((mbw_cbp_blk(q) >> raster_to_blk(rq)) & 1)) return 2;
diff --git a/jmcodec_amd/csrc/kernels.h b/jmcodec_amd/csrc/kernels.h
--- a/jmcodec_amd/csrc/kernels.h
+++ b/jmcodec_amd/csrc/kernels.h
@@ -11,6 +11,13 @@
 void launch_intra_lds(const PicParams *d_pics, int n, int max_mb_h, int *ctl, int *err, hipStream_t st);
 bool deblock_lds_supported(int mb_w, int mb_h);
 constexpr int kDeblockMaxBands = 32, kDeblockProgressStride = 2 * kDeblockMaxBands;
+constexpr int kSetupJobs = 12;
+struct BatchSetup {
+    struct Job { void *dst; const void *src; uint32_t n4; } job[kSetupJobs];
+    int n = 0; const int *wait_word = nullptr; int wait_ticks = 0;
+    void add(void *dst, const void *src, size_t bytes) { if (bytes && n < kSetupJobs) job[n++] = Job{dst, src, (uint32_t)(bytes / 4)}; }
+};
+void launch_batch_setup(const BatchSetup &s, hipStream_t st);
 void launch_deblock_prep(const PicParams *d_pics, int n, int max_mbs, hipStream_t st);
 void launch_deblock_lds(const PicParams *d_pics, int n, int max_mb_h, int *ctl, int *err, bool debug_stall, hipStream_t st);
 bool chain_supported(int mb_w, int mb_h);
diff --git a/jmcodec_amd/csrc/kernels.hip b/jmcodec_amd/csrc/kernels.hip
--- a/jmcodec_amd/csrc/kernels.hip
+++ b/jmcodec_amd/csrc/kernels.hip
@@ -4,9 +4,24 @@
 #include "kernels.h"
 #include "kernel_common.h"
 #include "deblock_packed.h"
+#include "bs_packed.h"
 #include "recon_device.h"
 
 namespace jmamd {
+
+__device__ __forceinline__ void recon_dbrec_wave(const PicParams &pp, int mb, uint32_t *stage) {
+    const int lane = threadIdx.x & 63;
+    const int mby = pp.mb_w_magic ? (int)__umulhi((uint32_t)mb, pp.mb_w_magic) : mb, mbx = mb - mby * pp.mb_w;
+    const bool in_left = mbx > 0, in_top = mby > 0;
+    const MbW q = __builtin_bit_cast(MbW, load_mbrec_uniform(pp.mbs + mb));
+    const MbW pl = __builtin_bit_cast(MbW, load_mbrec_uniform(pp.mbs + (in_left ? mb - 1 : mb)));
+    const MbW pt = __builtin_bit_cast(MbW, load_mbrec_uniform(pp.mbs + (in_top ? mb - pp.mb_w : mb)));
+    const uint32_t slw = *(const __attribute__((address_space(4))) uint32_t *)(uintptr_t)(pp.slices + mbw_slice(q));
+    const SliceRec sl = __builtin_bit_cast(SliceRec, slw);
+    if (lane < 32) dbrec_lane(pp, sl, q, pl, pt, in_left, in_top, lane, (DbRec *)stage);
+    __builtin_amdgcn_wave_barrier();
+    if (lane < 6) gst_u4((uint4 *)((DbRec *)pp.dbrec + mb) + lane, ((const uint4 *)stage)[lane]);
+}
 
 template <bool HAS_BI, bool FIELD>
 __global__ __launch_bounds__(256) void k_recon_inter(const PicParams *pics, int *err) {
@@ -18,6 +33,7 @@
     const int n_mbs = pp.mb_w * pp.mb_h;
     const int mb = blk * 4 + __builtin_amdgcn_readfirstlane((int)(threadIdx.x >> 6));
     recon_inter_wave<false, false, HAS_BI, FIELD>(pp, mb, mb < n_mbs, sm, ChainView{nullptr, err});
+    if (mb < n_mbs && (pp.stages & (PS_DEBLOCK_LDS | PS_CHAIN))) recon_dbrec_wave(pp, mb, sm.outt[threadIdx.x >> 6]);
 }
 
 constexpr int kWaves = 16;
@@ -422,6 +438,18 @@
     }
 }
 
+constexpr int kSetupBlocks = 64;
+__global__ __launch_bounds__(256) void k_batch_setup(BatchSetup s) {
+    const uint32_t t = blockIdx.x * 256u + threadIdx.x, step = kSetupBlocks * 256u;
+    for (int j = 0; j < s.n; j++) {
+        uint32_t *dst = (uint32_t *)s.job[j].dst;
+        const uint32_t *src = (const uint32_t *)s.job[j].src;
+        const uint32_t n4 = s.job[j].n4;
+        for (uint32_t i = t; i < n4; i += step) dst[i] = src ? src[i] : ((const int *)(dst + i) == s.wait_word ? (uint32_t)s.wait_ticks : 0u);
+    }
+}
+
+void launch_batch_setup(const BatchSetup &s, hipStream_t st) { if (s.n > 0) hipLaunchKernelGGL(k_batch_setup, dim3(kSetupBlocks), dim3(256), 0, st, s); }
 void launch_recon_inter(const PicParams *d_pics, int n, int max_mbs, bool any_bipred, bool any_field, int *d_err, hipStream_t st) {
     int nblk = ((max_mbs + 3) / 4 + 7) & ~7;
     if (any_field) { if (any_bipred) hipLaunchKernelGGL((k_recon_inter<true, true>), dim3(nblk, n), dim3(256), 0, st, d_pics, d_err);
```
